# Hongje/OTVM

Hardware: AMD Instinct MI355X
Metric: frames_per_sec (higher is better)
Workload: dtype f16x3 (fp32 operands split into fp16 hi+lo, fp32 accumulate); 1 GPU; synthetic 1920x1080 clip, T=140 frames (untimed lead-in 0 + warmup 5 + timed: the last 135), memory every 5, max 5 slots, trimap propagation + alpha + memorize per frame, one sequence per GPU; weights=synthetic (otvm_amd.synth_weights seed 0), parallelism=sequence-per-gpu x1, batch=1

## Files before the change

include/otvm_hip.h:

```cpp
#ifndef OTVM_HIP_H
#define OTVM_HIP_H

#include <stdint.h>

#ifdef __cplusplus
extern "C" {
#endif

#define OTVM_ACT_NONE 0
#define OTVM_ACT_RELU 1
#define OTVM_ACT_LEAKY 2

#define OTVM_PREC_F32 0
#define OTVM_PREC_F16X3 1
#define OTVM_PREC_F16 2

const char* otvm_last_error(void);
#define OTVM_ABI_VERSION 21
int otvm_abi_version(void);

int otvm_pack_conv_weight(const float* w_oihw, int O, int I, int kh, int kw, int ws, const float* scale,
                          float* w_packed, int O_pad, int I_pad, int K_pad, void* stream);

int64_t otvm_patch_weight_bytes_f16x3(int O, int I_pad);
int otvm_pack_patch_weight_f16x3(const float* w_packed, int O, int K_pad, int I_pad, void* w_frag, float* w_scale,
                                 void* stream);

int64_t otvm_stem_weight_bytes_f16x3(int I_pad);
int otvm_pack_stem_weight_f16x3(const float* w_packed, int O, int K_pad, int I_pad, void* w_frag, float* w_scale,
                                void* stream);

int otvm_fold_bn(const float* gamma, const float* beta, const float* mean, const float* var, float eps, int n,
                 float* scale, float* bias, void* stream);

typedef struct {
    const float* in;  int H, W, Cin, in_ld;
    const float* w;   int K_pad;
    const float* bias;
    const float* residual; int res_ld;
    float* out;       int Ho, Wo, Cout, out_ld;
    int kh, kw, stride, pad, dil;
    int in_relu, act;
    int precision;
    const void* w_hi; const void* w_lo;
    const float* w_scale;
    const void* w_frag;
    double* gn_stats;
    const float* in_scale; const float* in_shift;
    int in_act;
    int tune;
    void* splitk_ws; int64_t splitk_ws_bytes;
    int batch;
    int64_t in_bs, out_bs, res_bs;
    int gn_bs;
    int norm_bs;
    const void* w_wfrag;
    const float* gn_gamma; const float* gn_beta;
    float* gn_scale_out; float* gn_shift_out;
    unsigned* gn_counter;
    int gn_tab_bs;
    int ws_bs;
    const float* res_scale;
    int res_scale_bs;
    const float* in_res; int in_res_ld; int64_t in_res_bs;
} otvm_conv_params;
int otvm_conv2d_accepts_input_residual(const otvm_conv_params* p);

typedef struct otvm_head_params {
    const float* w; const float* b; int n_out;
    const float* img; int img_ld;
    int64_t P;
    float* alpha_out; int alpha_stride;
    float* tri_out;
    float* sm; int sm_ld;
    int64_t img_bs, alpha_bs, tri_bs, sm_bs;
    const void* w16;
} otvm_head_params;
int otvm_conv2d_head(const otvm_conv_params* p, const otvm_head_params* h, void* stream);
int otvm_conv2d_head_fgr(const otvm_conv_params* p, const otvm_head_params* h, float* fgr, int64_t fgr_bs, void* stream);
int64_t otvm_head16_weight_bytes_f16x3(void);
int otvm_pack_head16_weight_f16x3(const float* w_packed, int O, int K_pad, int I_pad, const float* w_scale, void* w16, void* stream);
int otvm_conv2d(const otvm_conv_params* p, void* stream);
int otvm_conv2d_candidates(const otvm_conv_params* p, int* out, int max_n);
int otvm_conv2d_accepts_input_norm(const otvm_conv_params* p);
int otvm_conv2d_input_norm_kind(const otvm_conv_params* p);

int otvm_split_conv_weight_f16x3(const float* w_packed, int O, int O_pad, int K_pad, int taps, int I_pad,
                                 void* w_hi, void* w_lo, float* w_scale, void* stream);

int64_t otvm_wave_weight_bytes_f16x3(int O_pad, int K_pad);
int otvm_pack_wave_weight_f16x3(const void* w_hi, const void* w_lo, int O_pad, int K_pad, void* w_wfrag, void* stream);

typedef struct {
    const float* x; int H, W, Cin, x_ld;
    float* y; int y_ld;
    const void* w1f; const void* w2f; const void* w3f;
    const float* s1; const float* s2; const float* s3;
    const float* b1; const float* b2; const float* b3;
    int batch; int64_t x_bs, y_bs;
    int tile;
} otvm_stm_bottleneck_params;
int otvm_stm_bottleneck_f16x3(const otvm_stm_bottleneck_params* p, void* stream);

int otvm_gn_stats(const float* x, int64_t P, int C, int ld, double* stats, void* stream);
int otvm_gn_table(const double* stats, int64_t P, int C, const float* gamma, const float* beta, float* scale,
                  float* shift, void* stream);
int otvm_gn_apply(const float* x, int64_t P, int C, int ld, const double* stats, const float* gamma,
                  const float* beta, const float* residual, int res_ld, const float* res_scale, const float* res_shift,
                  int res_act, int act, float* out, int out_ld, void* stream);

int otvm_gn_stats_b(const float* x, int64_t P, int C, int ld, double* stats, int batch, int64_t x_bs, int stats_bs, void* stream);
int otvm_gn_table_b(const double* stats, int64_t P, int C, const float* gamma, const float* beta, float* scale, float* shift,
                    int batch, int stats_bs, int norm_bs, void* stream);
typedef struct {
    const float* x; int64_t P; int C, ld; const double* stats; const float* gamma; const float* beta;
    const float* residual; int res_ld; const float* res_scale; const float* res_shift; int res_act, act;
    float* out; int out_ld;
    int batch; int64_t x_bs, res_bs, out_bs; int stats_bs, norm_bs;
} otvm_gn_apply_params;
int otvm_gn_apply_b(const otvm_gn_apply_params* p, void* stream);

typedef struct otvm_gram_params {
    const float* x; int64_t P; int C, ld;
    const float* in_scale; const float* in_shift; int in_act;
    float* gpart; float* spart; int passes;
    int batch; int64_t x_bs; int norm_bs;
    unsigned* diag;
} otvm_gram_params;
int otvm_gram_block(int C);
int64_t otvm_gram_entries(int C);
int otvm_gram_chunks(int64_t P, int C, int* pch_out);
int otvm_gram_f16(const otvm_gram_params* p, void* stream);
typedef struct otvm_gn_predict_params {
    const float* gpart; const float* spart; int64_t P; int C, Cout;
    const float* Mp; const double* v; void* ws; unsigned* counter;
    const float* wscale; const float* gamma; const float* beta; const float* res_shift;
    float* scale_eff; float* bias_eff; float* stat_out;
    int batch, tab_bs, rs_bs;
    unsigned* diag;
} otvm_gn_predict_params;
int64_t otvm_gn_predict_ws_bytes(void);
int otvm_gn_predict(const otvm_gn_predict_params* p, void* stream);

int otvm_maxpool3x3s2(const float* in, int H, int W, int C, int ld, float* out, int out_ld, void* stream);
int otvm_upsample_bilinear(const float* in, int Hi, int Wi, int C, int in_ld, const float* in_scale, const float* in_shift,
                           int in_act, const float* add, int add_ld, float* out, int Ho, int Wo, int out_ld, void* stream);
int otvm_maxpool3x3s2_b(const float* in, int H, int W, int C, int ld, float* out, int out_ld, int batch, int64_t in_bs,
                        int64_t out_bs, void* stream);
int otvm_upsample_bilinear_b(const float* in, int Hi, int Wi, int C, int in_ld, const float* in_scale, const float* in_shift,
                             int in_act, const float* add, int add_ld, float* out, int Ho, int Wo, int out_ld, int batch,
                             int64_t in_bs, int64_t add_bs, int64_t out_bs, int norm_bs, void* stream);
int64_t otvm_ppm_pool_ws_bytes(int H, int C);
int otvm_ppm_pool(const float* in, int H, int W, int C, int ld, float* out, void* ws, void* stream);

typedef struct otvm_ppm_head_params {
    const float* pooled; int C, K_pad, Cout;
    const float* w[4]; const float* bias[4]; const float* gamma[4]; const float* beta[4];
    float* out[4]; int out_ld, act;
} otvm_ppm_head_params;
int otvm_ppm_head(const otvm_ppm_head_params* p, void* stream);

int otvm_ppm_conv_z(const float* const* y, int y_ld, const float* w_ppm, float* Z, void* stream);
int otvm_ppm_conv_add(const float* Z, int H, int W, float* out, int out_ld, double* gn_stats, void* stream);

int64_t otvm_memory_read_ws_bytes(int hw, int T);
int otvm_memory_read(const float* q_key, int q_ld, const float* const* keys, const float* const* vals, int T,
                     int hw, float* out, int out_ld, void* ws, void* stream);

int64_t otvm_bank_slot_bytes_f16x3(int hw);
int otvm_bank_pack_f16x3(const float* key, const float* val, int hw, void* slot, void* stream);
int otvm_memory_read_f16x3(const float* q_key, int q_ld, const void* const* slots, int T, int hw, float* out,
                           int out_ld, void* ws, void* stream);

int otvm_memory_read_f16x3_partial_count(int n_slots, int hw);
int otvm_memory_read_f16x3_partial(const float* q_key, int q_ld, const void* const* slots, int n_slots, int hw, void* ws,
                                   int np_cap, int part0, int* part_end, void* stream);
int otvm_memory_read_f16x3_combine(const void* ws, int np_cap, int n_partials, int hw, float* out, int out_ld, void* stream);

typedef struct {
    const float* fg; const float* bg; const float* a;
    int H, W, Hp, Wp, lh, lw;
    float mean[3], std[3];
    float mean_q[3], std_q[3];
    float mean_m[3], std_m[3];
    float* scaled_imgs;
    float* x11; int x11_ld;
    float* sq;  int sq_ld;
    float* sm;  int sm_ld;
    float* d80; int d80_ld;
    const unsigned char* fg_u8;
    const unsigned char* bg_u8;
    int u8_rgb;
} otvm_preprocess_params;
int otvm_preprocess(const otvm_preprocess_params* p, void* stream);

int otvm_pad_trimap(const float* tri, int H, int W, float* out, int Hp, int Wp, int lh, int lw, void* stream);

int otvm_upsample4_softmax3(const float* logits, int h4, int w4, int ld, float* probs, void* stream);

int otvm_trimap_apply_labels(float* probs, const uint8_t* labels, int H, int W, int Hp, int Wp, int lh, int lw, void* stream);

int64_t otvm_trimap_encode_ws_bytes(int Hp, int Wp);
int otvm_trimap_encode(const float* probs, int Hp, int Wp, const uint8_t* cls_override, uint8_t* cls_out,
                       float* x11, int x11_ld, float* d80, int d80_ld, void* ws, void* stream);

int otvm_fba_head(const float* hid, int hid_ld, const float* w, const float* b, int n_out, const float* img,
                  int img_ld, int64_t P, float* alpha_out, int alpha_stride, float* tri_out, float* sm, int sm_ld,
                  void* stream);
int otvm_fba_head_fgr(const float* hid, int hid_ld, const float* w, const float* b, int n_out, const float* img,
                      int img_ld, int64_t P, float* alpha_out, int alpha_stride, float* tri_out, float* sm, int sm_ld,
                      float* fgr, void* stream);

int otvm_crop_outputs(const float* alpha_p, const float* tri_p, int Hp, int Wp, int H, int W, int lh, int lw,
                      float* alpha, uint8_t* alpha_u8, float* tri, void* stream);

typedef struct otvm_fgr_params {
    const float* alpha_p;
    const float* fgr_p;
    int Hp, Wp, H, W, lh, lw;
    float* fgr;
    unsigned char* rgba_u8;
    unsigned char* comp_u8;
    const unsigned char* bg_u8;
    unsigned char bg_color[3];
    int u8_rgb;
} otvm_fgr_params;
int otvm_fgr_outputs(const otvm_fgr_params* p, void* stream);

int otvm_downsample_u8(const uint8_t* src, int H, int W, int s, uint8_t* dst, void* stream);
int otvm_downsample_trimap(const float* src, int H, int W, int s, float* dst, void* stream);
int otvm_downsample_labels(const uint8_t* src, int H, int W, int s, uint8_t* dst, void* stream);

typedef struct otvm_guided_params {
    int H, W, s, h, w;
    int r, C;
    double eps;
    const uint8_t* guide_full;
    const uint8_t* guide_work;
    const float* target[4];
    float* coef;
    float* alpha;
    uint8_t* alpha_u8;
    float* fgr;
} otvm_guided_params;
int64_t otvm_guided_ws_bytes(int h, int w, int C);
int otvm_guided_coeffs(const otvm_guided_params* p, void* ws, void* stream);
int otvm_guided_apply(const otvm_guided_params* p, void* stream);

int otvm_trimap_from_alpha(const float* a, int H, int W, int r, float* out, void* ws, void* stream);

typedef struct otvm_mask_trimap_params {
    const uint8_t* mask;
    int H, W, lo, hi;
    int t_fg, t_bg;
    float* trimap;
    uint8_t* labels;
    int band_label;
} otvm_mask_trimap_params;
int64_t otvm_trimap_from_mask_ws_bytes(int H, int W);
int otvm_trimap_from_mask(const otvm_mask_trimap_params* p, void* ws, void* stream);

int otvm_onehot_argmax3(const float* tri, int64_t P, float* out, void* stream);

int otvm_matting_metrics(const uint8_t* pred, const uint8_t* target, const uint8_t* mask, const uint8_t* prev_pred,
                         const uint8_t* prev_target, const uint8_t* prev_mask, int64_t n, double* acc, void* stream);
int otvm_matting_grad_conn(const uint8_t* pred, const uint8_t* target, const uint8_t* mask, int H, int W, double* acc,
                           uint8_t* level_map, void* ws, void* stream);
int64_t otvm_matting_grad_conn_ws_bytes(int H, int W);
int otvm_matting_grad_conn_params(int* cutoffs, float* levels, double* taps);
int otvm_optflow_farneback(const uint8_t* prev, const uint8_t* next, int H, int W, float* flow, void* ws, void* stream);
int64_t otvm_optflow_farneback_ws_bytes(int H, int W);
int otvm_optflow_farneback_params(int H, int W, int* levels, float* blur_taps, float* poly_taps, double* poly_inv, float* win_taps);
int otvm_matting_messddt(const uint8_t* p0, const uint8_t* t0, const uint8_t* m0, const uint8_t* p1, const uint8_t* t1,
                         const uint8_t* m1, int H, int W, double* acc, float* flow_out, void* ws, void* stream);

typedef struct otvm_temporal_params {
    int H, W;
    const float* alpha;
    const float* prev;
    const uint8_t* grey;
    const uint8_t* grey_prev;
    const float* flow;
    const float* tri;
    int th, tw, tri_scale;
    float strength;
    float inv_tau_colour, inv_tau_alpha;
    float* out;
    uint8_t* out_u8;
} otvm_temporal_params;
int otvm_luma_u8(const uint8_t* img, int H, int W, int u8_rgb, uint8_t* grey, void* stream);
int otvm_temporal_blend(const otvm_temporal_params* p, void* stream);

int otvm_finite_guard(const float* x, int64_t P, int C, int ld, float limit, int tag, int* flag, void* stream);
int otvm_clear(void* p, int64_t bytes, void* stream);

int otvm_fba_head_train(const float* hid, int hid_ld, const float* w, const float* b, int n_out, const float* img, int img_ld,
                        int64_t P, float* out7, float* logits_out, void* stream);
int otvm_upsample4_logits3(const float* logits, int h4, int w4, int ld, float* logits_out, void* stream);
int otvm_trimap_to_sm(const float* tri, int64_t P, float* sm, int sm_ld, void* stream);
int otvm_scale_flip3(const float* in, int64_t N, int64_t P, float s, float* out, void* stream);
int otvm_trimask(const float* tri, int64_t N, int64_t P, float* mask, unsigned char* cls, const float* gts, float* vis, void* stream);
int otvm_loss_fba_comp(const float* pred7, const float* gt, const float* trimask, const float* fgs, const float* bgs, const float* img,
                       int64_t N, int64_t P, float* cF, float* cB, float* comp, float* alpha_out, double* acc5, void* stream);
int otvm_loss_grad_l1(const float* x, const float* y, int64_t N, int H, int W, float eps, double* acc, void* stream);
int otvm_loss_exclusion_level(const float* img1, const float* img2, int B, int S, int H, int W, float eps, double* acc1, double* acc2,
                              void* stream);
int otvm_avgpool2(const float* x, int64_t N, int H, int W, float* y, void* stream);
int otvm_loss_lap_level(const float* cur_img, const float* cur_tgt, int64_t N, int H, int W, double weight, float* down_img,
                        float* down_tgt, double* acc, void* stream);
int otvm_loss_temporal(const float* x, const float* y, int B, int S, int64_t CP, double* acc, void* stream);
int otvm_loss_ce3(const float* logits, const unsigned char* cls, int64_t N, int64_t P, double* acc, void* stream);

#ifdef __cplusplus
}
#endif
#endif
```

otvm_amd/csrc/conv_patch_f16x3.hip:

```cpp
#pragma clang diagnostic ignored "-Winline-asm"
#include "common.h"
#include "head_math.h"
#include "f16x3_ops.h"
#include <type_traits>
#include <stdlib.h>

#ifndef OTVM_PABL_NOMFMA
#define OTVM_PABL_NOMFMA 0
#endif
#ifndef OTVM_PABL_NOLOAD
#define OTVM_PABL_NOLOAD 0
#endif
#ifndef OTVM_PABL_NOCOMMIT
#define OTVM_PABL_NOCOMMIT 0
#endif
#ifndef OTVM_PABL_NOLDSRD
#define OTVM_PABL_NOLDSRD 0
#endif
#ifndef OTVM_PABL_NOEPI
#define OTVM_PABL_NOEPI 0
#endif
#ifndef OTVM_PABL_MFMA16
#define OTVM_PABL_MFMA16 0
#endif
#ifndef OTVM_PATCH_NO_LEAN
#define OTVM_PATCH_NO_LEAN 0
#endif
#ifndef OTVM_PATCH_SETPRIO
#define OTVM_PATCH_SETPRIO 0
#endif
#ifndef OTVM_PM16_NOKXP
#define OTVM_PM16_NOKXP 0
#endif

namespace {

struct PatchArgs {
    const float* in; const _Float16* wf; const float* wscale; const float* bias; const float* residual; float* out;
    double* gn_stats;
    int H, W, Cin, in_ld, res_ld, Cout, out_ld, n_pad32, in_relu, act;
    int tiles_x, tiles_y, tiles_n;
    OtvmTileWalk walk;
    const float* in_scale; const float* in_shift; int in_act;
    int64_t in_bs, out_bs, res_bs; int gn_bs, norm_bs, batch;
    OtvmGnTail tail;
    const float* in_res; int in_res_ld; int64_t in_res_bs;
    unsigned in_bytes, in_res_bytes;
    OtvmHeadArgs head; int64_t head_img_bs, head_alpha_bs, head_tri_bs, head_sm_bs, head_fgr_bs;
};

constexpr int CB = 16;
constexpr int LDP = 24;

#if OTVM_PABL_MFMA16
__device__ __forceinline__ f32x16 mfma_probe16(const f16x8 a, const f16x8 b, f32x16 c) {
    f32x4 q0 = {c[0], c[1], c[2], c[3]}, q1 = {c[4], c[5], c[6], c[7]};
    q0 = __builtin_amdgcn_mfma_f32_16x16x32_f16(a, b, q0, 0, 0, 0);
    q1 = __builtin_amdgcn_mfma_f32_16x16x32_f16(a, b, q1, 0, 0, 0);
    c[0] = q0.x; c[1] = q0.y; c[2] = q0.z; c[3] = q0.w; c[4] = q1.x; c[5] = q1.y; c[6] = q1.z; c[7] = q1.w;
    return c;
}
#define PATCH_MFMA32(a, b, c) mfma_probe16(a, b, c)
#else
#define PATCH_MFMA32(a, b, c) __builtin_amdgcn_mfma_f32_32x32x16_f16(a, b, c, 0, 0, 0)
#endif

__device__ __forceinline__ int pi16(int r) {
    const int k = (r < 4) ? r : (r < 12 ? r - 4 : r - 8);
    return 4 * (k >> 1) + (k & 1) + ((r >= 4 && r < 12) ? 2 : 0);
}

template <int TH, int BN, int NW, int DIL, int TAPG, bool INRES = false, bool HEAD = false, int NWN = 1, bool GLDS = false, int NPASS = 3,
          bool M16 = false, bool FGR = false>
__global__ __launch_bounds__(NW * 64)
__attribute__((amdgpu_waves_per_eu((TAPG == 3 && BN <= 32 && !INRES) ? 3 : (M16 ? 2 : 1), (TAPG == 3 && BN <= 32 && !INRES) ? 3 : 10)))
void conv_patch_f16x3_kernel(const PatchArgs pa) {
    PatchArgs p = pa;
    {
        const int zb = blockIdx.y;
        p.in += zb * p.in_bs;
        if (INRES) p.in_res += zb * p.in_res_bs;
        if (HEAD) {
            p.head.img += zb * p.head_img_bs;
            if (p.head.alpha_out) p.head.alpha_out += zb * p.head_alpha_bs;
            if (p.head.tri_out) p.head.tri_out += zb * p.head_tri_bs;
            if (p.head.sm) p.head.sm += zb * p.head_sm_bs;
            if constexpr (FGR) { if (p.head.fgr) p.head.fgr += zb * p.head_fgr_bs; }
        }
        p.out += zb * p.out_bs;
        if (p.residual) p.residual += zb * p.res_bs;
        if (p.gn_stats) p.gn_stats += zb * p.gn_bs;
        if (p.in_scale) { p.in_scale += zb * p.norm_bs; p.in_shift += zb * p.norm_bs; }
    }
    constexpr int NT = NW * 64;
    constexpr int NWM = NW / NWN, TNW = BN / 32;
    constexpr int TM = TH / NWM, TN = TNW / NWN;
    static_assert(NW % NWN == 0 && TH % NWM == 0 && TNW % NWN == 0, "bad wave grid");
    constexpr int PW = 32 + 2 * DIL, PH = TH + 2 * DIL, NPIX = PH * PW;
    constexpr int NG = 9 / TAPG;
    static_assert(BN % 32 == 0 && 9 % TAPG == 0, "bad tile");
    static_assert(!FGR || HEAD, "FGR: the HEAD variant that also keeps the head's foreground estimate (head.fgr)");
    static_assert(!M16 || (TAPG == 9 && NPASS == 3 && !HEAD && NWN == 1 && !GLDS), "the 16x16x32 form: nine-tap f16x3 tiles");
    constexpr int PLANE = ((NPIX + 11) / 16) * 16 + 4;
    constexpr int PATCH_HALFS = M16 ? 2 * 2 * PLANE * 8 : 2 * NPIX * LDP;
    constexpr int B_PIECES = TAPG * TNW * 2 * 64;
    constexpr int B_HALFS = B_PIECES * 8;
    constexpr int EPI_HALFS = NW * 32 * 36 * 2 * (HEAD ? 2 : 1);
    static_assert(!GLDS || TAPG == 3, "LDS-DMA weight stages: the 3-tap stages (two buffers fit beside the patch)");
    constexpr int NBUF = GLDS ? 2 : 1;
    constexpr int SM_HALFS = PATCH_HALFS + NBUF * B_HALFS > EPI_HALFS ? PATCH_HALFS + NBUF * B_HALFS : EPI_HALFS;
    __shared__ __attribute__((aligned(16))) _Float16 smem[SM_HALFS];
    _Float16* Ph = smem;
    _Float16* Pl = smem + (M16 ? 2 * PLANE * 8 : NPIX * LDP);
    _Float16* Bs = smem + PATCH_HALFS;

    const int tid = threadIdx.x, lane = tid & 63, wave = tid >> 6;
    const int wave_m = NWN == 1 ? wave : wave % NWM, nt0 = NWN == 1 ? 0 : (wave / NWM) * TN;
#ifdef OTVM_PATCH_STAGGER
    if (blockIdx.x >= 256 && blockIdx.x < 512)
        for (int i = 0; i < OTVM_PATCH_STAGGER; ++i) __builtin_amdgcn_s_sleep(127);
#endif
    int tile_n, tile_x, tile_y;
    otvm_tile_decode(p.walk, blockIdx.x, gridDim.x, p.tiles_n, p.tiles_x, p.tiles_y, tile_n, tile_x, tile_y);
    const int ty0 = tile_y * TH, tx0 = tile_x * 32, n0 = tile_n * BN;

    f32x16 acc[TM][TN];
#pragma unroll
    for (int a = 0; a < TM; ++a)
#pragma unroll
        for (int b = 0; b < TN; ++b)
#pragma unroll
            for (int e = 0; e < 16; ++e) acc[a][b][e] = 0.f;

    const int frow = lane & 31, fh = lane >> 5;
    const int ncb = p.Cin / CB;
    const int nbs = p.n_pad32 >> 5;
    const int nb0 = n0 >> 5;
    constexpr int NP = (NPIX * 4 + NT - 1) / NT;
    constexpr int NB = (B_PIECES + NT - 1) / NT;
    f32x4 rp[NP];
    f32x4 rr[INRES ? NP : 1];
    f16x8 rb[NB];
    f32x4 rsc = {1.f, 1.f, 1.f, 1.f}, rsh = {0.f, 0.f, 0.f, 0.f};
    __amdgpu_buffer_rsrc_t in_rsrc = otvm_buffer_rsrc(p.in, p.in_bytes);
    __amdgpu_buffer_rsrc_t res_rsrc = otvm_buffer_rsrc(INRES ? p.in_res : p.in, INRES ? p.in_res_bytes : 0);
    constexpr bool LEAN = M16 && !INRES && !OTVM_PATCH_NO_LEAN;
    unsigned l_voff[LEAN ? NP : 1];
    unsigned l_woff[LEAN ? NB : 1];
    unsigned l_wok = 0;
    int l_o0 = 0;
    float l_slope = 1.f;
    if constexpr (LEAN) {
        static_assert(NT % 4 == 0 && B_PIECES == NB * NT && TAPG == 9, "lean staging: whole weight pieces per thread, one stage per channel block");
#pragma unroll
        for (int k = 0; k < NP; ++k) {
            const int idx = tid + k * NT;
            const int pix = idx >> 2, c4 = (idx & 3) * 4;
            const int py = pix / PW, px = pix - py * PW;
            const int iy = ty0 - DIL + py, ix = tx0 - DIL + px;
            const bool ok = ((unsigned)iy < (unsigned)p.H) & ((unsigned)ix < (unsigned)p.W) & (idx < NPIX * 4);
            l_voff[k] = ok ? ((unsigned)(iy * p.W + ix) * (unsigned)p.in_ld + (unsigned)c4) << 2 : 0xFFFFFFFFu;
        }
#pragma unroll
        for (int k = 0; k < NB; ++k) {
            const int i = tid + k * NT;
            const int l = i & 63, blk = i >> 6, hl = blk & 1, tb = blk >> 1, b = tb % TNW, tap = tb / TNW;
            const bool ok = nb0 + b < nbs;
            l_woff[k] = (unsigned)((((tap * nbs + nb0 + (ok ? b : 0)) * 2) * 2 + hl) * 512 + l * 8) * 2u;
            l_wok |= ok ? (1u << k) : 0u;
        }
        l_o0 = (((tid >> 1) & 1) * PLANE + (tid >> 2)) * 8 + (tid & 1) * 4;
        l_slope = p.in_relu ? 0.f : (p.in_scale ? (p.in_act == OTVM_ACT_RELU ? 0.f : (p.in_act == OTVM_ACT_LEAKY ? 0.01f : 1.f)) : 1.f);
    }
    auto prefetch = [&](int cb, int g) __attribute__((always_inline)) {
        if constexpr (LEAN) {
            const unsigned soff = (unsigned)(cb * CB * 4);
#pragma unroll
            for (int k = 0; k < NP; ++k)
                rp[k] = __builtin_bit_cast(f32x4, (u32x4)__builtin_amdgcn_raw_buffer_load_b128(in_rsrc, __builtin_elementwise_add_sat(l_voff[k], soff), 0, 0));
            const char* wbase = reinterpret_cast<const char*>(p.wf) + (size_t)(((cb >> 1) * 9 * nbs * 2 + (cb & 1)) * 2) * 1024;
#pragma unroll
            for (int k = 0; k < NB; ++k) rb[k] = *reinterpret_cast<const f16x8*>(wbase + l_woff[k]);
            if (p.in_scale) {
                rsc = *reinterpret_cast<const f32x4*>(p.in_scale + cb * CB + (tid & 3) * 4);
                rsh = *reinterpret_cast<const f32x4*>(p.in_shift + cb * CB + (tid & 3) * 4);
            }
            return;
        }
        const int cb32 = cb >> 1, ks = cb & 1;
        _Float16* bdst = Bs + (GLDS ? ((cb * NG + g) & 1) * B_HALFS : 0);
#pragma unroll
        for (int k = 0; k < NB; ++k) {
            const int i = tid + k * NT;
            if (i < B_PIECES) {
                const int l = i & 63, blk = i >> 6;
                const int hl = blk & 1, tb = blk >> 1, b = tb % TNW, tap = g * TAPG + tb / TNW;
                if (NPASS == 1 && hl) continue;
                const int64_t src = (((((int64_t)cb32 * 9 + tap) * nbs + nb0 + b) * 2 + ks) * 2 + hl) * 512 + l * 8;
                if constexpr (GLDS) {
                    const unsigned m0v = __builtin_amdgcn_readfirstlane((unsigned)(uintptr_t)(__attribute__((address_space(3))) void*)(bdst + (i - l) * 8));
                    asm volatile("s_mov_b32 m0, %0\n\ts_nop 0\n\tglobal_load_lds_dwordx4 %1, off" :: "s"(m0v), "v"(p.wf + src) : "m0", "memory");
                } else {
                    f16x8 wv = {(_Float16)0.f, (_Float16)0.f, (_Float16)0.f, (_Float16)0.f, (_Float16)0.f, (_Float16)0.f, (_Float16)0.f, (_Float16)0.f};
                    if (nb0 + b < nbs) wv = *reinterpret_cast<const f16x8*>(p.wf + src);
                    rb[k] = wv;
                }
            }
        }
        if (g == 0) {
            if (p.in_scale) {
                rsc = *reinterpret_cast<const f32x4*>(p.in_scale + cb * CB + (tid & 3) * 4);
                rsh = *reinterpret_cast<const f32x4*>(p.in_shift + cb * CB + (tid & 3) * 4);
            }
#pragma unroll
            for (int k = 0; k < NP; ++k) {
                const int idx = tid + k * NT;
                const int pix = idx >> 2, c4 = (idx & 3) * 4;
                const int py = pix / PW, px = pix - py * PW;
                const int iy = ty0 - DIL + py, ix = tx0 - DIL + px;
                const unsigned oob = (unsigned)((int)((unsigned)iy < (unsigned)p.H) & (int)((unsigned)ix < (unsigned)p.W) &
                                                (int)(idx < NPIX * 4)) - 1u;
                const unsigned e = (unsigned)(iy * p.W + ix);
                rp[k] = __builtin_bit_cast(f32x4, (u32x4)__builtin_amdgcn_raw_buffer_load_b128(in_rsrc, ((e * (unsigned)p.in_ld + cb * CB + c4) << 2) | oob, 0, 0));
                if (INRES)
                    rr[k] = __builtin_bit_cast(f32x4, (u32x4)__builtin_amdgcn_raw_buffer_load_b128(res_rsrc, ((e * (unsigned)p.in_res_ld + cb * CB + c4) << 2) | oob, 0, 0));
            }
        }
    };
    auto commit = [&](int g) __attribute__((always_inline)) {
        if constexpr (LEAN) {
            const f16x8 zero8 = {(_Float16)0.f, (_Float16)0.f, (_Float16)0.f, (_Float16)0.f, (_Float16)0.f, (_Float16)0.f, (_Float16)0.f, (_Float16)0.f};
#pragma unroll
            for (int k = 0; k < NB; ++k) *reinterpret_cast<f16x8*>(&Bs[(tid + k * NT) * 8]) = ((l_wok >> k) & 1u) ? rb[k] : zero8;
            if (p.in_scale != nullptr || p.in_relu) {
#pragma unroll
                for (int k = 0; k < NP; ++k) {
                    f32x4 v = rp[k] * rsc + rsh;
                    v.x = fmaxf(v.x, 0.f) + l_slope * fminf(v.x, 0.f); v.y = fmaxf(v.y, 0.f) + l_slope * fminf(v.y, 0.f);
                    v.z = fmaxf(v.z, 0.f) + l_slope * fminf(v.z, 0.f); v.w = fmaxf(v.w, 0.f) + l_slope * fminf(v.w, 0.f);
                    const f32x4 z = {0.f, 0.f, 0.f, 0.f};
                    rp[k] = (l_voff[k] == 0xFFFFFFFFu) ? z : v;
                }
            }
#pragma unroll
            for (int k = 0; k < NP; ++k) {
                if (k + 1 < NP || tid + k * NT < NPIX * 4) {
                    f16x4 hi, lo;
                    otvm_split4(rp[k], hi, lo);
                    *reinterpret_cast<f16x4*>(&Ph[l_o0 + 512 * k]) = hi;
                    *reinterpret_cast<f16x4*>(&Pl[l_o0 + 512 * k]) = lo;
                }
            }
            return;
        }
        if constexpr (!GLDS) {
#pragma unroll
            for (int k = 0; k < NB; ++k) {
                const int i = tid + k * NT;
                if (NPASS == 1 && ((i >> 6) & 1)) continue;
                if (i < B_PIECES) *reinterpret_cast<f16x8*>(&Bs[i * 8]) = rb[k];
            }
        }
        if (g == 0) {
#pragma unroll
            for (int k = 0; k < NP; ++k) {
                const int idx = tid + k * NT;
                if (idx < NPIX * 4) {
                    f32x4 v = rp[k];
                    if (p.in_scale) {
                        const int pix = idx >> 2;
                        const int py = pix / PW, px = pix - py * PW;
                        const int iy = ty0 - DIL + py, ix = tx0 - DIL + px;
                        const bool inb = (unsigned)iy < (unsigned)p.H && (unsigned)ix < (unsigned)p.W;
                        v = v * rsc + rsh;
                        if (INRES && inb) v += rr[INRES ? k : 0];
                        v.x = otvm_act(v.x, p.in_act); v.y = otvm_act(v.y, p.in_act);
                        v.z = otvm_act(v.z, p.in_act); v.w = otvm_act(v.w, p.in_act);
                        const f32x4 z = {0.f, 0.f, 0.f, 0.f};
                        v = inb ? v : z;
                    }
                    if (p.in_relu) {
                        v.x = fmaxf(v.x, 0.f); v.y = fmaxf(v.y, 0.f); v.z = fmaxf(v.z, 0.f); v.w = fmaxf(v.w, 0.f);
                    }
                    f16x4 hi, lo;
                    const int pix = idx >> 2, c4 = (idx & 3) * 4;
                    if constexpr (M16) {
                        otvm_split4(v, hi, lo);
                        const int o = (((idx >> 1) & 1) * PLANE + pix) * 8 + (idx & 1) * 4;
                        *reinterpret_cast<f16x4*>(&Ph[o]) = hi;
                        *reinterpret_cast<f16x4*>(&Pl[o]) = lo;
                    } else if constexpr (NPASS == 3) {
                        otvm_split4(v, hi, lo);
                        *reinterpret_cast<f16x4*>(&Ph[pix * LDP + c4]) = hi;
                        *reinterpret_cast<f16x4*>(&Pl[pix * LDP + c4]) = lo;
                    } else {
                        hi = f16x4{(_Float16)v.x, (_Float16)v.y, (_Float16)v.z, (_Float16)v.w};
                        *reinterpret_cast<f16x4*>(&Ph[pix * LDP + c4]) = hi;
                    }
                }
            }
        }
    };
    prefetch(0, 0);
    for (int cb = 0; cb < ncb; ++cb) {
#pragma unroll
        for (int g = 0; g < NG; ++g) {
            const _Float16* Bcur = Bs + (GLDS ? ((cb * NG + g) & 1) * B_HALFS : 0);
            if constexpr (GLDS) {
                asm volatile("s_waitcnt vmcnt(0)" ::: "memory");
                __syncthreads();
                if (g == 0) {
                    commit(0);
                    __syncthreads();
                }
            } else {
                __syncthreads();
                if (!OTVM_PABL_NOCOMMIT || (cb == 0 && g == 0)) commit(g);
                __syncthreads();
            }
            if (!OTVM_PABL_NOLOAD) {
                if (g + 1 < NG) prefetch(cb, g + 1);
                else if (cb + 1 < ncb) prefetch(cb + 1, 0);
            }
            if constexpr (M16) {
                if (OTVM_PATCH_SETPRIO) __builtin_amdgcn_s_setprio(OTVM_PATCH_SETPRIO);
                const int l15 = lane & 15, oct = (lane >> 4) & 1, hs = lane >> 5;
                const int abase = (oct * PLANE + wave_m * TM * PW + pi16(l15)) * 8;
                const int bbase = (l15 + 32 * oct) * 8;
                auto quad = [](const f32x16& c, int q) __attribute__((always_inline)) { return f32x4{c[4 * q], c[4 * q + 1], c[4 * q + 2], c[4 * q + 3]}; };
                auto put = [](f32x16& c, int q, const f32x4 v) __attribute__((always_inline)) { c[4 * q] = v.x; c[4 * q + 1] = v.y; c[4 * q + 2] = v.z; c[4 * q + 3] = v.w; };
                auto pass = [&](const f16x8 (&A)[TM][2], const f16x8 (&B)[TN][2]) __attribute__((always_inline)) {
#pragma unroll
                    for (int a = 0; a < TM; ++a)
#pragma unroll
                        for (int b = 0; b < TN; ++b)
#pragma unroll
                            for (int si = 0; si < 2; ++si)
#pragma unroll
                                for (int sj = 0; sj < 2; ++sj)
                                    put(acc[a][b], 2 * si + sj, __builtin_amdgcn_mfma_f32_16x16x32_f16(A[a][si], B[b][sj], quad(acc[a][b], 2 * si + sj), 0, 0, 0));
                };
                constexpr int TAPB = TNW * 2 * 512;
#pragma unroll
                for (int pr = 0; pr < 4; ++pr) {
                    constexpr bool KXP = DIL == 1 && !OTVM_PM16_NOKXP;
                    const int t1 = !KXP ? 2 * pr : (pr < 3 ? pr : 6), t2 = !KXP ? 2 * pr + 1 : (pr < 3 ? 3 + pr : 7);
                    const int o1 = ((t1 % 3) * DIL * PW + (t1 / 3) * DIL) * 8, o2 = ((t2 % 3) * DIL * PW + (t2 / 3) * DIL) * 8;
                    const int ao = !KXP ? abase + (hs ? o2 : o1)
                                        : (pr < 3 ? abase + hs * (DIL * 8) + pr * DIL * PW * 8 : abase + 2 * DIL * 8 + hs * (DIL * PW * 8));
                    const int bo = bbase + (hs ? t2 : t1) * TAPB;
                    f16x8 ah[TM][2], al[TM][2], bh[TN][2], bl[TN][2];
#pragma unroll
                    for (int a = 0; a < TM; ++a)
#pragma unroll
                        for (int si = 0; si < 2; ++si) {
                            ah[a][si] = *reinterpret_cast<const f16x8*>(&Ph[ao + (a * PW + 16 * si) * 8]);
                            al[a][si] = *reinterpret_cast<const f16x8*>(&Pl[ao + (a * PW + 16 * si) * 8]);
                        }
#pragma unroll
                    for (int b = 0; b < TN; ++b)
#pragma unroll
                        for (int sj = 0; sj < 2; ++sj) {
                            bh[b][sj] = *reinterpret_cast<const f16x8*>(&Bcur[bo + ((nt0 + b) * 2) * 512 + 16 * sj * 8]);
                            bl[b][sj] = *reinterpret_cast<const f16x8*>(&Bcur[bo + ((nt0 + b) * 2 + 1) * 512 + 16 * sj * 8]);
                        }
                    pass(al, bh);
                    pass(ah, bl);
                    pass(ah, bh);
                }
                {
                    constexpr int o8 = (2 * DIL * PW + 2 * DIL) * 8;
                    const _Float16* Ahl = hs ? Pl : Ph;
                    f16x8 ax[TM][2], bhh[TN][2], bl0[TN][2];
#pragma unroll
                    for (int a = 0; a < TM; ++a)
#pragma unroll
                        for (int si = 0; si < 2; ++si) ax[a][si] = *reinterpret_cast<const f16x8*>(&Ahl[abase + o8 + (a * PW + 16 * si) * 8]);
                    const f16x8 zero8 = {(_Float16)0.f, (_Float16)0.f, (_Float16)0.f, (_Float16)0.f, (_Float16)0.f, (_Float16)0.f, (_Float16)0.f, (_Float16)0.f};
#pragma unroll
                    for (int b = 0; b < TN; ++b)
#pragma unroll
                        for (int sj = 0; sj < 2; ++sj) {
                            bhh[b][sj] = *reinterpret_cast<const f16x8*>(&Bcur[bbase + 8 * TAPB + ((nt0 + b) * 2) * 512 + 16 * sj * 8]);
                            const f16x8 l = *reinterpret_cast<const f16x8*>(&Bcur[bbase + 8 * TAPB + ((nt0 + b) * 2 + 1) * 512 + 16 * sj * 8]);
                            bl0[b][sj] = hs ? zero8 : l;
                        }
                    pass(ax, bl0);
                    pass(ax, bhh);
                }
                if (OTVM_PATCH_SETPRIO) __builtin_amdgcn_s_setprio(0);
            } else
#pragma unroll
            for (int tl = 0; tl < TAPG; ++tl) {
                const int tap = g * TAPG + tl;
                const int kx = tap / 3, ky = tap - kx * 3;
                f16x8 ah[TM], al[TM];
#pragma unroll
                for (int a = 0; a < TM; ++a) {
#if OTVM_PABL_NOLDSRD
                    const f16x8 one = {(_Float16)1.f, (_Float16)1.f, (_Float16)1.f, (_Float16)1.f, (_Float16)1.f, (_Float16)1.f, (_Float16)1.f, (_Float16)1.f};
                    ah[a] = one * (_Float16)(float)(lane + tap); al[a] = one;
#else
                    const int o = ((wave_m * TM + a + ky * DIL) * PW + kx * DIL + frow) * LDP + 8 * fh;
                    ah[a] = *reinterpret_cast<const f16x8*>(&Ph[o]);
                    if (NPASS == 3) al[a] = *reinterpret_cast<const f16x8*>(&Pl[o]);
#endif
                }
                constexpr int GB = TN < 4 ? TN : 4;
#pragma unroll
                for (int b0 = 0; b0 < TN; b0 += GB) {
                    f16x8 bh[GB], bl[GB];
#pragma unroll
                    for (int j = 0; j < GB; ++j) {
#if OTVM_PABL_NOLDSRD
                        const f16x8 one = {(_Float16)1.f, (_Float16)1.f, (_Float16)1.f, (_Float16)1.f, (_Float16)1.f, (_Float16)1.f, (_Float16)1.f, (_Float16)1.f};
                        bh[j] = one; bl[j] = one * (_Float16)(float)lane;
#else
                        bh[j] = *reinterpret_cast<const f16x8*>(&Bcur[((tl * TNW + nt0 + b0 + j) * 2) * 512 + lane * 8]);
                        if (NPASS == 3) bl[j] = *reinterpret_cast<const f16x8*>(&Bcur[((tl * TNW + nt0 + b0 + j) * 2 + 1) * 512 + lane * 8]);
#endif
                    }
#if OTVM_PABL_NOMFMA
                    if (ah[0][0] == (_Float16)12345.f) acc[0][0][0] += (float)bh[0][0] + (float)bl[0][0] + (float)al[0][0];
                    continue;
#endif
                    if constexpr (NPASS == 3) {
#pragma unroll
                        for (int j = 0; j < GB; ++j)
#pragma unroll
                            for (int a = 0; a < TM; ++a)
                                acc[a][b0 + j] = PATCH_MFMA32(al[a], bh[j], acc[a][b0 + j]);
#pragma unroll
                        for (int j = 0; j < GB; ++j)
#pragma unroll
                            for (int a = 0; a < TM; ++a)
                                acc[a][b0 + j] = PATCH_MFMA32(ah[a], bl[j], acc[a][b0 + j]);
                    }
#pragma unroll
                    for (int j = 0; j < GB; ++j)
#pragma unroll
                        for (int a = 0; a < TM; ++a)
                            acc[a][b0 + j] = PATCH_MFMA32(ah[a], bh[j], acc[a][b0 + j]);
                }
            }
        }
    }

    const int col = lane & 31, rbase = (lane >> 5) * 4;
    const int pbase16 = pi16(4 * (lane >> 4));
    auto acc_row = [&](int e) __attribute__((always_inline)) -> int {
        return M16 ? 16 * (e >> 3) + pbase16 + (e & 1) + 4 * ((e >> 1) & 1) : (e & 3) + 8 * (e >> 2) + rbase;
    };
    auto acc_col = [&](int e) __attribute__((always_inline)) -> int { return M16 ? 16 * ((e >> 2) & 1) + (lane & 15) : col; };
    __syncthreads();
#if OTVM_PABL_NOEPI
    if (acc[0][0][0] == 12345.678f) p.out[0] = acc[0][0][1];
    if (acc[0][0][0] != 12345.678f) return;
#endif
    if constexpr (HEAD) {
        static_assert(TM == 2 && TN == 1 && NWN == 1, "the head epilogue is written for two pixel rows and one channel tile per wave");
        float* patch = reinterpret_cast<float*>(smem) + wave * (2 * 32 * 36);
#pragma unroll
        for (int a = 0; a < TM; ++a)
#pragma unroll
            for (int e = 0; e < 16; ++e) patch[a * (32 * 36) + ((e & 3) + 8 * (e >> 2) + rbase) * 36 + col] = acc[a][0][e];
        const int a = lane >> 5, px = lane & 31;
        const int y = ty0 + wave_m * TM + a, x = tx0 + px;
        float h[16];
#pragma unroll
        for (int k = 0; k < 4; ++k) {
            f32x4 v = *reinterpret_cast<const f32x4*>(&patch[a * (32 * 36) + px * 36 + 4 * k]);
            f32x4 sc4, bi4 = {0.f, 0.f, 0.f, 0.f};
#pragma unroll
            for (int j = 0; j < 4; ++j) {
                sc4[j] = p.wscale[4 * k + j];
                if (p.bias) bi4[j] = p.bias[4 * k + j];
            }
            v = v * sc4 + bi4;
            h[4 * k] = otvm_act(v.x, p.act); h[4 * k + 1] = otvm_act(v.y, p.act);
            h[4 * k + 2] = otvm_act(v.z, p.act); h[4 * k + 3] = otvm_act(v.w, p.act);
        }
        if (y < p.H && x < p.W) {
            const int64_t m = (int64_t)y * p.W + x;
            if (p.out) {
#pragma unroll
                for (int k = 0; k < 4; ++k)
                    *reinterpret_cast<f32x4*>(p.out + m * p.out_ld + 4 * k) = f32x4{h[4 * k], h[4 * k + 1], h[4 * k + 2], h[4 * k + 3]};
            }
            otvm_head_pixel<FGR>(h, p.head, m);
        }
        return;
    }
    const bool vec_ok = ((p.out_ld & 3) == 0) && ((reinterpret_cast<uintptr_t>(p.out) & 15) == 0) &&
                        (!p.residual || (((p.res_ld & 3) == 0) && ((reinterpret_cast<uintptr_t>(p.residual) & 15) == 0)));
    const bool interior = vec_ok && ty0 + TH <= p.H && tx0 + 32 <= p.W && n0 + BN <= p.Cout;
    auto epilogue_full = [&](auto act_c, auto res_c) __attribute__((always_inline)) {
        constexpr int ACT = decltype(act_c)::value;
        constexpr bool RES = decltype(res_c)::value;
        float* patch = reinterpret_cast<float*>(smem) + wave * (32 * 36);
        const int prow = lane >> 3, pc = (lane & 7) * 4;
        f32x4 sc4[TN], bi4[TN];
#pragma unroll
        for (int b = 0; b < TN; ++b) {
#pragma unroll
            for (int j = 0; j < 4; ++j) sc4[b][j] = p.wscale[n0 + (nt0 + b) * 32 + pc + j];
            bi4[b] = f32x4{0.f, 0.f, 0.f, 0.f};
        }
        if (p.bias) {
#pragma unroll
            for (int b = 0; b < TN; ++b)
#pragma unroll
                for (int j = 0; j < 4; ++j) bi4[b][j] = p.bias[n0 + (nt0 + b) * 32 + pc + j];
        }
        auto load_res = [&](int t, f32x4 (&r)[4]) __attribute__((always_inline)) {
            const int b = t / TM, a = t - b * TM;
            const int64_t m0r = (int64_t)(ty0 + wave_m * TM + a) * p.W + tx0 + prow;
#pragma unroll
            for (int r4 = 0; r4 < 4; ++r4)
                r[r4] = *reinterpret_cast<const f32x4*>(p.residual + (m0r + r4 * 8) * p.res_ld + n0 + (nt0 + b) * 32 + pc);
        };
        f32x4 rnext[4] = {{0.f, 0.f, 0.f, 0.f}, {0.f, 0.f, 0.f, 0.f}, {0.f, 0.f, 0.f, 0.f}, {0.f, 0.f, 0.f, 0.f}};
        if (RES) load_res(0, rnext);
#pragma unroll
        for (int t = 0; t < TM * TN; ++t) {
            const int b = t / TM, a = t - b * TM;
            const int64_t m0r = (int64_t)(ty0 + wave_m * TM + a) * p.W + tx0 + prow;
            f32x4 rres[4];
#pragma unroll
            for (int r4 = 0; r4 < 4; ++r4) rres[r4] = rnext[r4];
#pragma unroll
            for (int e = 0; e < 16; ++e) patch[acc_row(e) * 36 + acc_col(e)] = acc[a][b][e];
            if (RES && t + 1 < TM * TN) load_res(t + 1, rnext);
#pragma unroll
            for (int r4 = 0; r4 < 4; ++r4) {
                f32x4 v = *reinterpret_cast<const f32x4*>(&patch[(r4 * 8 + prow) * 36 + pc]);
                v = v * sc4[b] + bi4[b];
                if (RES) v += rres[r4];
                v.x = otvm_act(v.x, ACT); v.y = otvm_act(v.y, ACT); v.z = otvm_act(v.z, ACT); v.w = otvm_act(v.w, ACT);
                *reinterpret_cast<f32x4*>(p.out + (m0r + r4 * 8) * p.out_ld + n0 + (nt0 + b) * 32 + pc) = v;
            }
        }
    };
    auto epilogue = [&](auto full_c) __attribute__((always_inline)) {
        constexpr bool FULL = decltype(full_c)::value;
        float* patch = reinterpret_cast<float*>(smem) + wave * (32 * 36);
        const int prow = lane >> 3, pc = (lane & 7) * 4;
#pragma unroll
        for (int b = 0; b < TN; ++b) {
            const int n4 = n0 + (nt0 + b) * 32 + pc;
            f32x4 sc4 = {0.f, 0.f, 0.f, 0.f}, bi4 = {0.f, 0.f, 0.f, 0.f};
#pragma unroll
            for (int j = 0; j < 4; ++j) {
                if (FULL || n4 + j < p.Cout) {
                    sc4[j] = p.wscale[n4 + j];
                    bi4[j] = p.bias ? p.bias[n4 + j] : 0.f;
                }
            }
#pragma unroll
            for (int a = 0; a < TM; ++a) {
                const int y = ty0 + wave_m * TM + a;
                f32x4 rres[4];
                const bool res_vec = p.residual && vec_ok && (FULL || n4 + 3 < p.Cout);
#pragma unroll
                for (int r4 = 0; r4 < 4; ++r4) {
                    const int x = tx0 + r4 * 8 + prow;
                    rres[r4] = f32x4{0.f, 0.f, 0.f, 0.f};
                    if (FULL ? (p.residual != nullptr) : (res_vec && y < p.H && x < p.W))
                        rres[r4] = *reinterpret_cast<const f32x4*>(p.residual + ((int64_t)y * p.W + x) * p.res_ld + n4);
                }
#pragma unroll
                for (int e = 0; e < 16; ++e) patch[acc_row(e) * 36 + acc_col(e)] = acc[a][b][e];
#pragma unroll
                for (int r4 = 0; r4 < 4; ++r4) {
                    const int xi = r4 * 8 + prow;
                    const int x = tx0 + xi;
                    f32x4 v = *reinterpret_cast<const f32x4*>(&patch[xi * 36 + pc]);
                    v = v * sc4 + bi4;
                    if (FULL || (y < p.H && x < p.W)) {
                        const int64_t m = (int64_t)y * p.W + x;
                        if (FULL || (vec_ok && n4 + 3 < p.Cout)) {
                            v += rres[r4];
                            v.x = otvm_act(v.x, p.act); v.y = otvm_act(v.y, p.act);
                            v.z = otvm_act(v.z, p.act); v.w = otvm_act(v.w, p.act);
                            *reinterpret_cast<f32x4*>(p.out + m * p.out_ld + n4) = v;
                        } else {
#pragma unroll
                            for (int j = 0; j < 4; ++j) {
                                if (n4 + j < p.Cout) {
                                    float xv = v[j];
                                    if (p.residual) xv += p.residual[m * p.res_ld + n4 + j];
                                    p.out[m * p.out_ld + n4 + j] = otvm_act(xv, p.act);
                                }
                            }
                        }
                    }
                }
            }
        }
    };
    if (interior) {
        using std::integral_constant;
        const bool r = p.residual != nullptr;
        if (p.act == OTVM_ACT_RELU) { if (r) epilogue_full(integral_constant<int, OTVM_ACT_RELU>{}, std::true_type{}); else epilogue_full(integral_constant<int, OTVM_ACT_RELU>{}, std::false_type{}); }
        else if (p.act == OTVM_ACT_LEAKY) { if (r) epilogue_full(integral_constant<int, OTVM_ACT_LEAKY>{}, std::true_type{}); else epilogue_full(integral_constant<int, OTVM_ACT_LEAKY>{}, std::false_type{}); }
        else { if (r) epilogue_full(integral_constant<int, OTVM_ACT_NONE>{}, std::true_type{}); else epilogue_full(integral_constant<int, OTVM_ACT_NONE>{}, std::false_type{}); }
    } else {
        epilogue(std::false_type{});
    }

    if (p.gn_stats) {
        __shared__ double gred[2 * BN];
        const int cg = p.Cout >> 5;
        const int seg = cg < 32 ? cg : 32;
        for (int i = tid; i < 2 * BN; i += NT) gred[i] = 0.0;
        __syncthreads();
        if constexpr (M16) {
#pragma unroll
            for (int b = 0; b < TN; ++b)
#pragma unroll
                for (int sj = 0; sj < 2; ++sj) {
                    const int nl = (nt0 + b) * 32 + 16 * sj + (lane & 15);
                    const int n = n0 + nl;
                    float s = 0.f, ss = 0.f, cnt = 0.f;
                    const float pil = n < p.Cout && p.bias ? p.bias[n / cg * cg] : 0.f;
                    if (n < p.Cout) {
                        const float sc_ = p.wscale[n];
                        const float bias = p.bias ? p.bias[n] : 0.f, bd = bias - pil;
#pragma unroll
                        for (int a = 0; a < TM; ++a) {
                            const int y = ty0 + wave_m * TM + a;
#pragma unroll
                            for (int si = 0; si < 2; ++si)
#pragma unroll
                                for (int j = 0; j < 4; ++j) {
                                    const int e = 4 * (2 * si + sj) + j;
                                    const int x = tx0 + acc_row(e);
                                    if (y < p.H && x < p.W) {
                                        const float d = acc[a][b][e] * sc_ + bd;
                                        s += d;
                                        ss += d * d;
                                        cnt += 1.f;
                                    }
                                }
                        }
                    }
                    s += __shfl_xor(s, 16); ss += __shfl_xor(ss, 16); cnt += __shfl_xor(cnt, 16);
                    s += __shfl_xor(s, 32); ss += __shfl_xor(ss, 32); cnt += __shfl_xor(cnt, 32);
                    const int seg16 = seg < 16 ? seg : 16;
                    for (int off = 1; off < seg16; off <<= 1) {
                        s += __shfl_xor(s, off);
                        ss += __shfl_xor(ss, off);
                        cnt += __shfl_xor(cnt, off);
                    }
                    if (lane < 16 && (lane & (seg16 - 1)) == 0 && n < p.Cout) {
                        const int gl = nl / cg;
                        double S, SS;
                        otvm_gn_unshift(s, ss, (int)cnt, pil, S, SS);
                        atomicAdd(&gred[2 * gl], S);
                        atomicAdd(&gred[2 * gl + 1], SS);
                    }
                }
        } else
#pragma unroll
        for (int b = 0; b < TN; ++b) {
            const int nl = (nt0 + b) * 32 + col;
            const int n = n0 + nl;
            float s = 0.f, ss = 0.f, cnt = 0.f;
            const float pil = n < p.Cout && p.bias ? p.bias[n / cg * cg] : 0.f;
            if (n < p.Cout) {
                const float sc_ = p.wscale[n];
                const float bias = p.bias ? p.bias[n] : 0.f, bd = bias - pil;
#pragma unroll
                for (int a = 0; a < TM; ++a) {
                    const int y = ty0 + wave_m * TM + a;
#pragma unroll
                    for (int e = 0; e < 16; ++e) {
                        const int x = tx0 + (e & 3) + 8 * (e >> 2) + rbase;
                        if (y < p.H && x < p.W) {
                            const float d = acc[a][b][e] * sc_ + bd;
                            s += d;
                            ss += d * d;
                            cnt += 1.f;
                        }
                    }
                }
            }
            s += __shfl_xor(s, 32);
            ss += __shfl_xor(ss, 32);
            cnt += __shfl_xor(cnt, 32);
            for (int off = 1; off < seg; off <<= 1) {
                s += __shfl_xor(s, off);
                ss += __shfl_xor(ss, off);
                cnt += __shfl_xor(cnt, off);
            }
            if (lane < 32 && (lane & (seg - 1)) == 0 && n < p.Cout) {
                const int gl = nl / cg;
                double S, SS;
                otvm_gn_unshift(s, ss, (int)cnt, pil, S, SS);
                atomicAdd(&gred[2 * gl], S);
                atomicAdd(&gred[2 * gl + 1], SS);
            }
        }
        __syncthreads();
        const int ng = (BN + cg - 1) / cg;
        for (int i = tid; i < 2 * ng; i += NT) {
            const int g = n0 / cg + (i >> 1);
            if (g < 32 && gred[i] != 0.0) atomicAdd(&p.gn_stats[2 * g + (i & 1)], gred[i]);
        }
        __syncthreads();
        otvm_gn_table_tail(p.gn_stats, (int64_t)p.H * p.W, p.Cout, p.tail, blockIdx.y, gridDim.x, reinterpret_cast<float*>(gred));
    }
}

__global__ __launch_bounds__(256) void pack_patch_weight_kernel(const float* __restrict__ w, int O, int K_pad, int I_pad, int n_pad32,
                                                                _Float16* __restrict__ wf, float* __restrict__ wscale) {
    const int n = blockIdx.x;
    __shared__ float red[256];
    float mx = 0.f;
    const float* row = w + (int64_t)n * K_pad;
    const bool real = n < O;
    if (real)
        for (int k = threadIdx.x; k < 9 * I_pad; k += 256) mx = fmaxf(mx, fabsf(row[k]));
    red[threadIdx.x] = mx;
    __syncthreads();
    for (int s = 128; s > 0; s >>= 1) {
        if (threadIdx.x < s) red[threadIdx.x] = fmaxf(red[threadIdx.x], red[threadIdx.x + s]);
        __syncthreads();
    }
    int e = 0;
    if (red[0] > 0.f) frexpf(red[0], &e);
    const float inv = ldexpf(1.f, -e);
    if (threadIdx.x == 0 && real) wscale[n] = ldexpf(1.f, e);
    const int nb = n >> 5, nl = n & 31, nbs = n_pad32 >> 5;
    for (int k = threadIdx.x; k < 9 * I_pad; k += 256) {
        const int tap0 = k / I_pad, c = k - tap0 * I_pad;
        const int tap = (tap0 % 3) * 3 + tap0 / 3;
        const float v = real ? row[k] * inv : 0.f;
        const _Float16 hi = (_Float16)v;
        const _Float16 lo = (_Float16)(v - (float)hi);
        const int cb = c >> 5, ks = (c >> 4) & 1, h = (c >> 3) & 1, j = c & 7;
        const int l = nl + 32 * h;
        const int64_t blk = ((((int64_t)cb * 9 + tap) * nbs + nb) * 2 + ks) * 2;
        wf[(blk + 0) * 512 + l * 8 + j] = hi;
        wf[(blk + 1) * 512 + l * 8 + j] = lo;
    }
}

template <int NPASS, int TH, int BN, int NW, int DIL, int TAPG = 9, bool INRES = false, bool HEAD = false, int NWN = 1, bool GLDS = false,
          bool M16 = false, bool FGR = false>
int launch_patch(PatchArgs& a, hipStream_t s) {
    a.tiles_x = otvm_ceil_div(a.W, 32);
    a.tiles_y = otvm_ceil_div(a.H, TH);
    a.tiles_n = otvm_ceil_div(a.Cout, BN);
    a.walk = otvm_tile_walk_of(1);
    hipLaunchKernelGGL((conv_patch_f16x3_kernel<TH, BN, NW, DIL, TAPG, INRES, HEAD, NWN, GLDS, NPASS, M16, FGR>), dim3(a.tiles_x * a.tiles_y * a.tiles_n, a.batch), dim3(NW * 64), 0, s, a);
    OTVM_CHECK_LAUNCH("otvm_conv2d(patch f16x3)");
    return 0;
}

}

extern "C" int64_t otvm_patch_weight_bytes_f16x3(int O, int I_pad) {
    const int64_t n_pad32 = (O + 31) / 32 * 32;
    return (int64_t)((I_pad + 31) / 32) * 9 * n_pad32 * 32 * 2 * sizeof(_Float16);
}

extern "C" int otvm_pack_patch_weight_f16x3(const float* w_packed, int O, int K_pad, int I_pad, void* w_frag, float* w_scale,
                                            void* stream) {
    OTVM_REQUIRE(w_packed && w_frag && w_scale && I_pad % 16 == 0, "otvm_pack_patch_weight_f16x3: needs I_pad %% 16 == 0");
    const int n_pad32 = (O + 31) / 32 * 32;
    hipLaunchKernelGGL(pack_patch_weight_kernel, dim3(n_pad32), dim3(256), 0, (hipStream_t)stream, w_packed, O, K_pad, I_pad, n_pad32,
                       (_Float16*)w_frag, w_scale);
    OTVM_CHECK_LAUNCH("otvm_pack_patch_weight_f16x3");
    return 0;
}

static int patch_choice(const otvm_conv_params* p, bool forced = false) {
    if (!p->w_frag || p->kh != 3 || p->kw != 3 || p->stride != 1 || p->pad != p->dil || p->Cin % 16 != 0) return 0;
    if (p->dil != 1 && p->dil != 2 && p->dil != 4) return 0;
    static const int wide = otvm_probe_int("OTVM_PATCH_WIDE", 1);
    if (p->Cout <= 64) return 1;
    if (!wide || p->Cout % 256 != 0) return 0;
    if (forced) return 2;
    static const int t_patch = otvm_probe_int("OTVM_T_PATCH", 400);
    const int64_t t8 = (int64_t)otvm_ceil_div(p->H, 8) * otvm_ceil_div(p->W, 32) * (p->Cout / 256);
    return t8 >= t_patch ? 2 : 0;
}

int otvm_conv2d_igemm_accepts_input_norm(const otvm_conv_params* p);
extern "C" int otvm_conv2d_accepts_input_norm(const otvm_conv_params* p) {
    return p && otvm_prec_is_split(p->precision) && (patch_choice(p) != 0 || otvm_conv2d_igemm_accepts_input_norm(p)) ? 1 : 0;
}
extern "C" int otvm_conv2d_input_norm_kind(const otvm_conv_params* p) {
    if (!p || !otvm_prec_is_split(p->precision)) return 0;
    if (patch_choice(p) != 0) return 1;
    return otvm_conv2d_igemm_accepts_input_norm(p) ? 2 : 0;
}

extern "C" int otvm_conv2d_accepts_input_residual(const otvm_conv_params* p) {
    return p && otvm_prec_is_split(p->precision) && patch_choice(p) == 1 && p->dil == 1 && p->in_scale && !p->in_relu ? 1 : 0;
}

int otvm_conv2d_patch_eligible(const otvm_conv_params* p) {
    if (p->in_res && !otvm_conv2d_accepts_input_residual(p)) return 0;
    return patch_choice(p, true) != 0 ? 1 : 0;
}

static int patch_run(const otvm_conv_params* p, void* stream, int choice, const otvm_head_params* hd = nullptr, float* fgr = nullptr,
                     int64_t fgr_bs = 0);
int otvm_conv2d_head16_impl(const otvm_conv_params* p, const otvm_head_params* hd, float* fgr, int64_t fgr_bs, void* stream);

static int conv2d_head_any(const otvm_conv_params* p, const otvm_head_params* hd, float* fgr, int64_t fgr_bs, void* stream) {
    OTVM_REQUIRE(p && hd && p->in && hd->w && hd->b && hd->img, "otvm_conv2d_head: null pointer");
    OTVM_REQUIRE(otvm_prec_is_split(p->precision) && p->Cout == 16 && patch_choice(p) == 1 && p->dil == 1 && !p->residual &&
                     !p->gn_stats && !p->in_res && p->w_scale,
                 "otvm_conv2d_head: a 3x3 stride-1 f16x3 layer with 16 output channels, no residual / statistics");
    OTVM_REQUIRE(hd->n_out == 7 || (hd->n_out == 10 && hd->tri_out), "otvm_conv2d_head: n_out must be 7, or 10 with tri_out");
    OTVM_REQUIRE(!p->out || ((p->out_ld & 3) == 0 && ((uintptr_t)p->out & 15) == 0), "otvm_conv2d_head: out must be 16-byte aligned");
    if (hd->w16) return otvm_conv2d_head16_impl(p, hd, fgr, fgr_bs, stream);
    return patch_run(p, stream, 1, hd, fgr, fgr_bs);
}

extern "C" int otvm_conv2d_head(const otvm_conv_params* p, const otvm_head_params* hd, void* stream) {
    return conv2d_head_any(p, hd, nullptr, 0, stream);
}

extern "C" int otvm_conv2d_head_fgr(const otvm_conv_params* p, const otvm_head_params* hd, float* fgr, int64_t fgr_bs, void* stream) {
    OTVM_REQUIRE(fgr && hd && hd->P > 0 && ((p && p->batch > 1) ? fgr_bs >= 3 * hd->P : true),
                 "otvm_conv2d_head_fgr: fgr must be given, [3][P] per image (fgr_bs >= 3 P for a batch)");
    return conv2d_head_any(p, hd, fgr, fgr_bs, stream);
}

int otvm_conv2d_patch_f16x3_forced(const otvm_conv_params* p, void* stream) { return patch_run(p, stream, patch_choice(p, true)); }

int otvm_conv2d_patch_f16x3_impl(const otvm_conv_params* p, void* stream) { return patch_run(p, stream, patch_choice(p)); }

static int patch_m16() {
    static const int m = otvm_probe_int("OTVM_PATCH_M16", 1);
    return m;
}

template <int NPASS>
static int patch_run_t(const otvm_conv_params* p, void* stream, int choice, const otvm_head_params* hd, float* fgr, int64_t fgr_bs) {
    if (choice == 0) return -1;
    const bool is_wide = choice == 2;
    PatchArgs a;
    a.in = p->in; a.wf = (const _Float16*)p->w_frag; a.wscale = p->w_scale; a.bias = p->bias; a.residual = p->residual;
    a.out = p->out; a.gn_stats = p->gn_stats;
    a.H = p->H; a.W = p->W; a.Cin = p->Cin; a.in_ld = p->in_ld; a.res_ld = p->res_ld; a.Cout = p->Cout; a.out_ld = p->out_ld;
    a.n_pad32 = (p->Cout + 31) / 32 * 32; a.in_relu = p->in_relu; a.act = p->act;
    hipStream_t s = (hipStream_t)stream;
    a.in_scale = p->in_scale; a.in_shift = p->in_shift; a.in_act = p->in_act;
    a.tail = otvm_gn_tail_of(p);
    a.batch = p->batch > 1 ? p->batch : 1;
    a.in_bs = a.batch > 1 ? p->in_bs : 0; a.out_bs = a.batch > 1 ? p->out_bs : 0; a.res_bs = a.batch > 1 ? p->res_bs : 0;
    a.gn_bs = a.batch > 1 ? p->gn_bs : 0; a.norm_bs = a.batch > 1 ? p->norm_bs : 0;
    a.in_res = p->in_res; a.in_res_ld = p->in_res_ld; a.in_res_bs = a.batch > 1 ? p->in_res_bs : 0;
    {
        const int64_t ib = (int64_t)p->H * p->W * p->in_ld * 4, rb = p->in_res ? (int64_t)p->H * p->W * p->in_res_ld * 4 : 0;
        OTVM_REQUIRE(ib < 0xFFFFFFF0ll && rb < 0xFFFFFFF0ll, "otvm_conv2d(patch f16x3): input view of %lld bytes is beyond 32-bit offsets", (long long)ib);
        a.in_bytes = (unsigned)ib; a.in_res_bytes = (unsigned)rb;
    }
    if (hd) {
        a.head.w = hd->w; a.head.b = hd->b; a.head.n_out = hd->n_out; a.head.img = hd->img; a.head.img_ld = hd->img_ld;
        a.head.P = hd->P; a.head.alpha_out = hd->alpha_out; a.head.alpha_stride = hd->alpha_stride; a.head.tri_out = hd->tri_out;
        a.head.sm = hd->sm; a.head.sm_ld = hd->sm_ld; a.head.out7 = nullptr; a.head.logits_out = nullptr;
        a.head_img_bs = a.batch > 1 ? hd->img_bs : 0; a.head_alpha_bs = a.batch > 1 ? hd->alpha_bs : 0;
        a.head_tri_bs = a.batch > 1 ? hd->tri_bs : 0; a.head_sm_bs = a.batch > 1 ? hd->sm_bs : 0;
        a.head.fgr = fgr; a.head_fgr_bs = a.batch > 1 ? fgr_bs : 0;
        if (fgr) return launch_patch<3, 8, 32, 4, 1, 3, false, true, 1, false, false, true>(a, s);
        return launch_patch<3, 8, 32, 4, 1, 3, false, true>(a, s);
    }
    if (p->in_res) {
        OTVM_REQUIRE(otvm_conv2d_accepts_input_residual(p) && !is_wide && (p->in_res_ld & 3) == 0 && ((uintptr_t)p->in_res & 15) == 0,
                     "otvm_conv2d: in_res needs in_scale on a 3x3 stride-1 dilation-1 layer with <= 64 output channels");
        if (p->Cout <= 32) return launch_patch<3, 8, 32, 4, 1, 3, true>(a, s);
        return patch_m16() ? launch_patch<3, 8, 64, 4, 1, 9, true, false, 1, false, true>(a, s) : launch_patch<3, 8, 64, 4, 1, 9, true>(a, s);
    }
    if (is_wide) {
        static const int nwn = otvm_probe_int("OTVM_PATCH_WIDE_NWN", 2);
        static const int glds = otvm_probe_int("OTVM_PATCH_WIDE_GLDS", 1);
        if (nwn == 2 && p->dil == 1 && glds) return launch_patch<NPASS, 8, 256, 8, 1, 3, false, false, 2, true>(a, s);
        if (nwn == 2 && p->dil == 1) return launch_patch<NPASS, 8, 256, 8, 1, 3, false, false, 2>(a, s);
        if (p->dil == 1) return launch_patch<NPASS, 8, 256, 8, 1, 3>(a, s);
        if (p->dil == 2) return launch_patch<NPASS, 8, 256, 8, 2, 3>(a, s);
        return launch_patch<NPASS, 8, 256, 8, 4, 3>(a, s);
    }
    static const int th16 = otvm_probe_int("OTVM_PATCH_TH16", 0);
    if (p->dil == 1 && th16 && (int64_t)p->H * p->W >= (1 << 18))
        return p->Cout <= 32 ? launch_patch<NPASS, 16, 32, 8, 1>(a, s) : launch_patch<NPASS, 16, 64, 8, 1>(a, s);
    static const int rows4 = otvm_probe_int("OTVM_PATCH32_ROWS4", 1);
    static const int glds32 = otvm_probe_int("OTVM_PATCH32_GLDS", 0);
    if (p->dil == 1 && p->Cout <= 32 && rows4 && (int64_t)p->H * p->W >= (1 << 20))
        return glds32 ? launch_patch<NPASS, 16, 32, 4, 1, 3, false, false, 1, true>(a, s) : launch_patch<NPASS, 16, 32, 4, 1, 3>(a, s);
    static const int glds64 = otvm_probe_int("OTVM_PATCH64_GLDS", 0);
    if (p->dil == 1 && p->Cout > 32 && glds64) return launch_patch<NPASS, 8, 64, 4, 1, 3, false, false, 1, true>(a, s);
    if (p->dil == 1 && p->Cout <= 32 && glds32) return launch_patch<NPASS, 8, 32, 4, 1, 3, false, false, 1, true>(a, s);
    if constexpr (NPASS == 3) {
        if (patch_m16() && p->Cout > 32) {
            if (p->dil == 1) return launch_patch<3, 8, 64, 4, 1, 9, false, false, 1, false, true>(a, s);
            if (p->dil == 2) return launch_patch<3, 8, 64, 4, 2, 9, false, false, 1, false, true>(a, s);
            return launch_patch<3, 8, 64, 4, 4, 9, false, false, 1, false, true>(a, s);
        }
    }
    if (p->dil == 1) return p->Cout <= 32 ? launch_patch<NPASS, 8, 32, 4, 1, 3>(a, s) : launch_patch<NPASS, 8, 64, 4, 1>(a, s);
    if (p->dil == 2) return launch_patch<NPASS, 8, 64, 4, 2>(a, s);
    return launch_patch<NPASS, 8, 64, 4, 4>(a, s);
}

static int patch_run(const otvm_conv_params* p, void* stream, int choice, const otvm_head_params* hd, float* fgr, int64_t fgr_bs) {
    return p->precision == OTVM_PREC_F16 ? patch_run_t<1>(p, stream, choice, hd, fgr, fgr_bs) : patch_run_t<3>(p, stream, choice, hd, fgr, fgr_bs);
}
```

otvm_amd/engine.py:

```python
import ctypes as C
import os

import torch

from . import lib as L

NONE, RELU, LEAKY = 0, 1, 2
GUARD_CLEAR = 2 ** 31 - 1
F16_LIMIT = 65504.0
FUSE_GN_STATS = True
FUSE_GN_APPLY = os.environ.get("OTVM_FUSE_GN_APPLY", "1") != "0"
_GRAPHS_ENV = os.environ.get("OTVM_GRAPHS")
USE_GRAPHS = None if _GRAPHS_ENV in (None, "", "auto") else (_GRAPHS_ENV != "0")
GRAPH_AUTO_PIXELS = 1 << 22


def graphs_wanted(setting, padded_pixels):
    if setting is not None:
        return bool(setting)
    if int(os.environ.get("WORLD_SIZE", "1")) > 1:
        return True
    return padded_pixels < GRAPH_AUTO_PIXELS
PRE_ON_S2 = os.environ.get("OTVM_PRE_ON_S2", "1") != "0"
EVDEC_LATE = os.environ.get("OTVM_EVDEC_LATE", "1") != "0"
WAVE_TILE = os.environ.get("OTVM_WAVE_TILE", "0") != "0"
FUSE_GN_APPLY_IGEMM = os.environ.get("OTVM_FUSE_GN_APPLY_IGEMM", "1") != "0"
FUSE_GN_APPLY_IGEMM_KXK = os.environ.get("OTVM_FUSE_GN_APPLY_IGEMM_KXK", "0") != "0"
FUSE_GN_TABLE = os.environ.get("OTVM_FUSE_GN_TABLE", "1") != "0"
FUSE_STM_BLOCK = os.environ.get("OTVM_FUSE_STM_BLOCK", "1") != "0"
FUSE_STM_BLOCK128 = int(os.environ.get("OTVM_FUSE_STM_BLOCK128", "1"))
STM128_TILE = int(os.environ.get("OTVM_STM128_TILE", "0"))
FUSE_PPM_HEAD = os.environ.get("OTVM_PPM_HEAD", "1") != "0"
FUSE_GN_PREDICT = os.environ.get("OTVM_GN_PREDICT", "1") != "0"
GN_PREDICT_MIN_PIXELS = int(os.environ.get("OTVM_GN_PREDICT_MIN_PIXELS", "16384"))
GN_PREDICT_PASSES = int(os.environ.get("OTVM_GN_PREDICT_PASSES", "1"))
GN_PREDICT_PLANES = tuple(int(v) for v in os.environ.get("OTVM_GN_PREDICT_PLANES", "64,128,256,512").split(",") if v)
GN_PREDICT_DS = os.environ.get("OTVM_GN_PREDICT_DS", "1") != "0"
GN_PREDICT_KAPPA_P3 = float(os.environ.get("OTVM_GN_PREDICT_KAPPA_P3", "4"))
GN_PREDICT_KAPPA_OFF = float(os.environ.get("OTVM_GN_PREDICT_KAPPA_OFF", "256"))
FUSE_REFINE_TAIL = os.environ.get("OTVM_FUSE_REFINE_TAIL", "0") != "0"
FUSE_HEAD = os.environ.get("OTVM_FUSE_HEAD", "1") != "0"
HEAD16 = os.environ.get("OTVM_HEAD16", "1") != "0"
PPM_ALGEBRA = os.environ.get("OTVM_PPM_ALGEBRA", "1") != "0"


AUTOTUNE = os.environ.get("OTVM_AUTOTUNE", "1") != "0"
_TUNE_CACHE = {}
TUNE_LOG = []
TUNE_FILE = os.environ.get("OTVM_TUNE_FILE")
_TUNE_FILE_LOADED = False


_NON_VARIANT_ENV = ("OTVM_TUNE_FILE", "OTVM_DIST_BACKEND", "OTVM_TEST_FULL_F64", "OTVM_TEST_4K_ORACLE", "OTVM_BENCH_LIVE_PMC",
                    "OTVM_BENCH_FORCE_DIAG", "OTVM_CHECK_FINITE", "OTVM_GRAPHS")


def variant_env():
    return sorted((k, v) for k, v in os.environ.items() if k.startswith("OTVM_") and k not in _NON_VARIANT_ENV)


def kernel_config_digest():
    import hashlib
    return hashlib.sha256(repr((sorted(_TUNE_CACHE.items()), variant_env())).encode()).hexdigest()[:16]


def _tune_file_tag():
    name = "none"
    if torch.cuda.is_available():
        pr = torch.cuda.get_device_properties(torch.cuda.current_device())
        name = "%s/%dcu" % (getattr(pr, "gcnArchName", "?").split(":")[0], pr.multi_processor_count)
    return {"device": name, "abi": L.ABI_VERSION, "variant_env": [list(kv) for kv in variant_env()]}


def _load_tune_file():
    if not (TUNE_FILE and os.path.exists(TUNE_FILE)):
        return
    import json
    import warnings
    try:
        with open(TUNE_FILE) as f:
            doc = json.load(f)
        if not isinstance(doc, dict) or "choices" not in doc:
            raise ValueError("no 'choices' table (file written by an older build)")
        tag = _tune_file_tag()
        if doc.get("abi") != tag["abi"] or (tag["device"] != "none" and doc.get("device") != tag["device"]):
            raise ValueError("tuned for %r / ABI %r, this process runs %r / ABI %r"
                             % (doc.get("device"), doc.get("abi"), tag["device"], tag["abi"]))
        if doc.get("variant_env", []) != tag["variant_env"]:
            raise ValueError("tuned under the switches %r, this process runs under %r" % (doc.get("variant_env", []), tag["variant_env"]))
        for k, v in doc["choices"].items():
            _TUNE_CACHE[tuple(json.loads(k))] = int(v)
    except Exception as e:
        warnings.warn("otvm_amd: ignoring OTVM_TUNE_FILE=%s (%s)" % (TUNE_FILE, e))


def _save_tune_file():
    if not TUNE_FILE:
        return
    import json
    doc = dict(_tune_file_tag())
    doc["choices"] = {json.dumps([int(x) for x in k]): v for k, v in _TUNE_CACHE.items()}
    tmp = "%s.%d.tmp" % (TUNE_FILE, os.getpid())
    with open(tmp, "w") as f:
        json.dump(doc, f, indent=0)
    os.replace(tmp, TUNE_FILE)


def share_tune_cache(src=0):
    import torch.distributed as dist
    if not (dist.is_available() and dist.is_initialized()):
        return
    obj = [dict(_TUNE_CACHE) if dist.get_rank() == src else None]
    dist.broadcast_object_list(obj, src=src)
    if dist.get_rank() != src:
        _TUNE_CACHE.update(obj[0])


def _rup(x, m):
    return (x + m - 1) // m * m


class Act:
    __slots__ = ("t", "H", "W", "C", "ld", "off", "B", "bs")

    def __init__(self, t, H, W, C, ld=None, off=0, B=1, bs=0):
        self.t, self.H, self.W, self.C = t, H, W, C
        self.ld = C if ld is None else ld
        self.off = off
        self.B, self.bs = B, (bs if B > 1 else 0)

    @property
    def ptr(self):
        return self.t.data_ptr() + 4 * self.off

    @property
    def P(self):
        return self.H * self.W

    def ch(self, c0, c):
        return Act(self.t, self.H, self.W, c, self.ld, self.off + c0, self.B, self.bs)

    def img(self, b):
        return Act(self.t, self.H, self.W, self.C, self.ld, self.off + b * self.bs)

    def torch(self, b=0):
        return torch.as_strided(self.t, (self.H, self.W, self.C), (self.W * self.ld, self.ld, 1), self.off + b * self.bs)


class ConvW:
    __slots__ = ("w", "K_pad", "O", "I", "I_pad", "kh", "kw", "bias", "w_hi", "w_lo", "w_scale", "w_frag", "w_wfrag", "w16")


def pad_amounts(h, w, d):
    nh = h + (d - h % d) % d
    nw = w + (d - w % d) % d
    lh, lw = int((nh - h) / 2), int((nw - w) / 2)
    return lw, nw - w - lw, lh, nh - h - lh


def _is_anchor(slot):
    return isinstance(slot, dict) and bool(slot.get("anchor", False))


def bank_update(bank, new, first_frame, memorize, max_memory_num, anchor=False):
    old = list(bank)
    new_anchor = bool(anchor or first_frame)
    if isinstance(new, dict):
        new["anchor"] = new_anchor
    if max_memory_num == 0:
        nb = [new] if first_frame else bank
    elif max_memory_num == 1:
        nb = [new]
    else:
        if first_frame:
            nb = [new]
        elif new_anchor or memorize or len(bank) == 1 or (bank and _is_anchor(bank[-1])):
            nb = bank + [new]
        else:
            nb = bank[:-1] + [new]
        cap = max_memory_num + max(0, sum(1 for s in nb if _is_anchor(s)) - 1)
        while len(nb) > cap:
            i = next(j for j in range(1, len(nb)) if not _is_anchor(nb[j]))
            nb = nb[:i] + nb[i + 1:]
    released = [s for s in old + [new] if not any(s is k for k in nb)]
    return nb, released


PRECISIONS = {"f32": L.PREC_F32, "f16x3": L.PREC_F16X3, "f16": L.PREC_F16X3}
CONV_PRECISIONS = {"f32": L.PREC_F32, "f16x3": L.PREC_F16X3, "f16": L.PREC_F16}


def default_precision():
    import os
    return os.environ.get("OTVM_PRECISION", "f16x3")


def pack_conv_weight(lib, dev, w, ws=False, scale=None, i_pad=None, split=True, stream=0):
    O, I, kh, kw = w.shape
    cw = ConvW()
    cw.O, cw.I, cw.kh, cw.kw = O, I, kh, kw
    cw.I_pad = _rup(I, 4) if i_pad is None else i_pad
    cw.K_pad = _rup(kh * kw * cw.I_pad, 32)
    O_pad = _rup(O, 128)
    cw.w = torch.empty(O_pad * cw.K_pad, dtype=torch.float32, device=dev)
    cw.bias = None
    w = w.contiguous()
    L.check(lib.otvm_pack_conv_weight(w.data_ptr(), O, I, kh, kw, 1 if ws else 0,
                                      0 if scale is None else scale.data_ptr(), cw.w.data_ptr(), O_pad,
                                      cw.I_pad, cw.K_pad, stream), "pack_conv_weight")
    cw.w_hi = cw.w_lo = cw.w_scale = cw.w_frag = cw.w_wfrag = cw.w16 = None
    if split:
        cw.w_hi = torch.empty(O_pad * cw.K_pad, dtype=torch.float16, device=dev)
        cw.w_lo = torch.empty(O_pad * cw.K_pad, dtype=torch.float16, device=dev)
        cw.w_scale = torch.empty(O, dtype=torch.float32, device=dev)
        L.check(lib.otvm_split_conv_weight_f16x3(cw.w.data_ptr(), O, O_pad, cw.K_pad, kh * kw, cw.I_pad, cw.w_hi.data_ptr(),
                                                 cw.w_lo.data_ptr(), cw.w_scale.data_ptr(), stream), "split_conv_weight")
        if cw.I_pad % 32 == 0 and kh * kw <= 32 and (WAVE_TILE or O >= 128):
            cw.w_wfrag = torch.zeros(int(lib.otvm_wave_weight_bytes_f16x3(O_pad, cw.K_pad)), dtype=torch.uint8, device=dev)
            L.check(lib.otvm_pack_wave_weight_f16x3(cw.w_hi.data_ptr(), cw.w_lo.data_ptr(), O_pad, cw.K_pad, cw.w_wfrag.data_ptr(),
                                                    stream), "pack_wave_weight")
        if kh == 7 and kw == 7 and O <= 64 and cw.I_pad <= 64:
            cw.w_frag = torch.zeros(int(lib.otvm_stem_weight_bytes_f16x3(cw.I_pad)), dtype=torch.uint8, device=dev)
            L.check(lib.otvm_pack_stem_weight_f16x3(cw.w.data_ptr(), O, cw.K_pad, cw.I_pad, cw.w_frag.data_ptr(),
                                                    cw.w_scale.data_ptr(), stream), "pack_stem_weight")
        if kh == 3 and kw == 3 and cw.I_pad % 16 == 0:
            cw.w_frag = torch.zeros(int(lib.otvm_patch_weight_bytes_f16x3(O, cw.I_pad)), dtype=torch.uint8, device=dev)
            L.check(lib.otvm_pack_patch_weight_f16x3(cw.w.data_ptr(), O, cw.K_pad, cw.I_pad, cw.w_frag.data_ptr(),
                                                     cw.w_scale.data_ptr(), stream), "pack_patch_weight")
            if O == 16 and cw.I_pad == 32:
                cw.w16 = torch.zeros(int(lib.otvm_head16_weight_bytes_f16x3()), dtype=torch.uint8, device=dev)
                L.check(lib.otvm_pack_head16_weight_f16x3(cw.w.data_ptr(), O, cw.K_pad, cw.I_pad, cw.w_scale.data_ptr(),
                                                          cw.w16.data_ptr(), stream), "pack_head16_weight")
    return cw


def gram_tables(lib, cw):
    O_pad = cw.w.numel() // cw.K_pad
    w = cw.w.view(O_pad, cw.K_pad)[:cw.O, :cw.I].double()
    cg, Cin = cw.O // 32, cw.I
    wg = w.view(32, cg, Cin)
    v = wg.sum(1).contiguous()
    bs = int(lib.otvm_gram_block(Cin))
    nb = Cin // bs
    blocks = []
    for bi in range(nb):
        rows = wg[:, :, bi * bs:(bi + 1) * bs]
        for bj in range(bi, nb):
            m = torch.einsum("gci,gcj->gij", rows, wg[:, :, bj * bs:(bj + 1) * bs])
            blocks.append((m if bi == bj else 2.0 * m).reshape(32, bs * bs))
    mp = torch.cat(blocks, 1).float().contiguous()
    assert mp.shape[1] == int(lib.otvm_gram_entries(Cin))
    return mp, v


def conv_params(x, cw, out, bias=None, stride=1, pad=0, dil=1, act=NONE, in_relu=0, residual=None, precision=L.PREC_F32,
                in_norm=None, splitk_ws=None):
    Ho = (x.H + 2 * pad - dil * (cw.kh - 1) - 1) // stride + 1
    Wo = (x.W + 2 * pad - dil * (cw.kw - 1) - 1) // stride + 1
    if precision in (L.PREC_F16X3, L.PREC_F16) and cw.w_hi is None:
        raise RuntimeError("otvm_amd: f16x3 convolution requested but the weight was packed without a split")
    return L.ConvParams(x.ptr, x.H, x.W, x.C, x.ld, cw.w.data_ptr(), cw.K_pad,
                        0 if bias is None else bias.data_ptr(),
                        0 if residual is None else residual.ptr, 0 if residual is None else residual.ld,
                        out.ptr, Ho, Wo, cw.O, out.ld, cw.kh, cw.kw, stride, pad, dil, in_relu, act, precision,
                        0 if cw.w_hi is None else cw.w_hi.data_ptr(), 0 if cw.w_lo is None else cw.w_lo.data_ptr(),
                        0 if cw.w_scale is None else cw.w_scale.data_ptr(),
                        0 if cw.w_frag is None else cw.w_frag.data_ptr(), 0,
                        0 if in_norm is None else in_norm[0], 0 if in_norm is None else in_norm[1],
                        0 if in_norm is None else in_norm[2], 0,
                        0 if splitk_ws is None else splitk_ws.data_ptr(),
                        0 if splitk_ws is None else splitk_ws.numel() * splitk_ws.element_size(),
                        x.B, x.bs, out.bs, 0 if residual is None else residual.bs, 0,
                        0 if in_norm is None or len(in_norm) < 4 else in_norm[3],
                        0 if cw.w_wfrag is None else cw.w_wfrag.data_ptr())


class HipEngine:
    def __init__(self, state_dict, device, precision=None):
        self.lib = L.load()
        self.precision_name = precision or default_precision()
        if self.precision_name not in PRECISIONS:
            raise ValueError("otvm_amd: unknown precision %r (choose from %s)" % (self.precision_name, sorted(PRECISIONS)))
        self.precision = PRECISIONS[self.precision_name]
        self.conv_precision = CONV_PRECISIONS[self.precision_name]
        self.dev = torch.device(device)
        if self.dev.type != "cuda":
            raise RuntimeError("otvm_amd: the HIP path needs a GPU device (got %s); there is no CPU fallback" % device)
        self.sd = {k: v.detach().to(self.dev, torch.float32).contiguous() for k, v in state_dict.items()
                   if v.is_floating_point()}
        self.W = {}
        self._keep = []
        self.plans = {}
        self.bank = []
        self.free_slots = []
        self.stream = 0
        self.prof = None
        self.pending = None
        self.ev_dec = None
        self.frame_counter = 0
        self.conv_calls = 0
        self.last_T_read = 0
        self.parity = 0
        self.side = None
        self.side2 = None
        import os
        self.use_side_stream = os.environ.get("OTVM_SIDE_STREAM", "1") != "0"
        self.check_level = int(os.environ.get("OTVM_CHECK_FINITE", "1") or 0)
        self.check_finite = self.check_level >= 2
        self.guard_flag = torch.full((1,), GUARD_CLEAR, dtype=torch.int32, device=self.dev)
        self._guard_host = torch.full((1,), GUARD_CLEAR, dtype=torch.int32).pin_memory()
        self._guard_ev = None
        self._guard_what = {}
        self.use_graphs = USE_GRAPHS
        self.gn_predict_off = False
        self.gn_predict_log = []
        self.gn_predict_suspect_from = None
        self._diag_host = None
        self._diag_ev = None
        self.keep_hid_d = False
        self.foreground = False
        self.background = None
        self._fgr_on = False
        self.last_fgr = self.last_rgba_u8 = self.last_comp_u8 = None
        self.last_fgr_b = self.last_rgba_u8_b = self.last_comp_u8_b = None
        global _TUNE_FILE_LOADED
        if not _TUNE_FILE_LOADED:
            _TUNE_FILE_LOADED = True
            with torch.cuda.device(self.dev):
                _load_tune_file()
        self._pack_all()

    def _stream(self):
        return torch.cuda.current_stream(self.dev).cuda_stream

    def _pack(self, name, w, ws=False, scale=None, bias=None, i_pad=None):
        cw = pack_conv_weight(self.lib, self.dev, w, ws, scale, i_pad, split=(self.precision == L.PREC_F16X3),
                              stream=self._stream())
        cw.bias = bias
        self._keep.append((w, scale))
        self.W[name] = cw

    def _wave_frag(self, cw):
        if cw.w_wfrag is None:
            O_pad = cw.w_hi.numel() // cw.K_pad
            cw.w_wfrag = torch.zeros(int(self.lib.otvm_wave_weight_bytes_f16x3(O_pad, cw.K_pad)), dtype=torch.uint8, device=self.dev)
            L.check(self.lib.otvm_pack_wave_weight_f16x3(cw.w_hi.data_ptr(), cw.w_lo.data_ptr(), O_pad, cw.K_pad,
                                                         cw.w_wfrag.data_ptr(), self._stream()), "pack_wave_weight")
        return cw.w_wfrag

    def _gram_tables(self, cw):
        return gram_tables(self.lib, cw)

    def _fold_bn(self, bn):
        sd = self.sd
        n = sd[bn + ".weight"].numel()
        scale = torch.empty(n, dtype=torch.float32, device=self.dev)
        bias = torch.empty(n, dtype=torch.float32, device=self.dev)
        L.check(self.lib.otvm_fold_bn(sd[bn + ".weight"].data_ptr(), sd[bn + ".bias"].data_ptr(),
                                      sd[bn + ".running_mean"].data_ptr(), sd[bn + ".running_var"].data_ptr(), 1e-5, n,
                                      scale.data_ptr(), bias.data_ptr(), self._stream()), "fold_bn " + bn)
        return scale, bias

    def _pack_all(self):
        with torch.cuda.device(self.dev):
            self._pack_all_on_device()

    def _pack_all_on_device(self):
        sd = self.sd
        for k, v in sd.items():
            if not (k.endswith(".weight") and v.dim() == 4):
                continue
            name = k[:-7]
            if k.startswith("NET."):
                ws = not ("conv_up4" in k or ".pred." in k)
                if name in ("NET.decoder.conv_up4.4", "NET.refine.pred.4"):
                    continue
                i_pad = 80 if name in ("NET.decoder.conv_up4.0", "NET.refine.conv1.0") else None
                self._pack(name, v, ws=ws, bias=sd.get(name + ".bias"), i_pad=i_pad)
            elif ".Encoder_" in k:
                if ".conv1_" in k or name.endswith("Encoder_M.conv1"):
                    continue
                bn = name.replace(".conv", ".bn").replace("downsample.0", "downsample.1")
                scale, bias = self._fold_bn(bn)
                self._pack(name, v, scale=scale, bias=bias)
            else:
                self._pack(name, v, bias=sd.get(name + ".bias"))
        if FUSE_STM_BLOCK and self.precision == L.PREC_F16X3:
            for enc in ("trimap.model.Encoder_M.", "trimap.model.Encoder_Q."):
                if enc + "res2.0.conv3.weight" not in sd:
                    continue
                s3, b3 = self._fold_bn(enc + "res2.0.bn3")
                sdn, bdn = self._fold_bn(enc + "res2.0.downsample.1")
                wcat = torch.cat([sd[enc + "res2.0.conv3.weight"] * s3[:, None, None, None],
                                  sd[enc + "res2.0.downsample.0.weight"] * sdn[:, None, None, None]], dim=1)
                self._pack(enc + "res2.0.conv3cat", wcat, bias=b3 + bdn)
                for b in range(3):
                    for cname in ("conv1", "conv2", "conv3cat" if b == 0 else "conv3"):
                        self._wave_frag(self.W[enc + "res2.%d.%s" % (b, cname)])
        self.GP = {}
        if FUSE_GN_PREDICT and self.precision == L.PREC_F16X3:
            for name, cw in list(self.W.items()):
                if (name.startswith("NET.encoder.layer") and name.endswith(".conv3") and cw.kh == 1 and cw.kw == 1 and cw.bias is None
                        and cw.I % 64 == 0 and cw.O % 32 == 0 and cw.I_pad == cw.I):
                    self.GP[name] = self._gram_tables(cw)
        e = "trimap.model.Encoder_M."
        wcat = torch.cat([sd[e + "conv1_h.weight"], sd[e + "conv1.weight"], sd[e + "conv1_m.weight"],
                          sd[e + "conv1_o.weight"], sd[e + "conv1_a.weight"]], dim=1)
        scale, bias = self._fold_bn(e + "bn1")
        self._pack(e + "stem", wcat, scale=scale, bias=bias, i_pad=24)
        up1 = self.W.get("NET.decoder.conv_up1.0")
        self.W_ppm = None
        if PPM_ALGEBRA and FUSE_PPM_HEAD and up1 is not None and (up1.O, up1.I, up1.kh, up1.kw) == (256, 3072, 3, 3):
            O_pad = up1.w.numel() // up1.K_pad
            wk = up1.w.view(O_pad, up1.K_pad)[:256, :9 * up1.I_pad].reshape(256, 3, 3, up1.I_pad)
            w_main = wk[..., :2048].permute(0, 3, 1, 2).contiguous()
            self._pack("NET.decoder.conv_up1.0.main", w_main, ws=False, bias=up1.bias)
            self.W_ppm = wk[..., 2048:3072].reshape(256, 9, 4, 256).permute(2, 1, 3, 0).contiguous()
        torch.cuda.synchronize(self.dev)

    def guard(self, act, what, stream, tag=None):
        if self.check_level <= 0:
            return
        tag = self.frame_counter - 1 if tag is None else tag
        limit = F16_LIMIT if self.precision == L.PREC_F16X3 else float("inf")
        for b in range(act.B):
            v = act.img(b) if act.B > 1 else act
            L.check(self.lib.otvm_finite_guard(v.ptr, v.P, v.C, v.ld, limit, max(int(tag), 0), self.guard_flag.data_ptr(), stream),
                    "finite_guard " + what)

    def scan_now(self, act, what, stream):
        self.guard(act, what, stream)
        v = int(self.guard_flag.item())
        if v != GUARD_CLEAR:
            self.guard_flag.fill_(GUARD_CLEAR)
            raise FloatingPointError("otvm_amd: |x| >= 65504 (or inf / NaN) at the %s, frame %d" % (what, v))

    def _guard_raise(self, frame):
        self.guard_flag.fill_(GUARD_CLEAR)
        self._guard_host.fill_(GUARD_CLEAR)
        self._guard_ev = None
        raise FloatingPointError(
            "otvm_amd: a value outside fp16's range (|x| >= 65504, inf or NaN) reached the recurrent state (memorised key / "
            "value, hidden state or propagated trimap logits) at frame %d of the sequence: the f16x3 path splits fp32 operands "
            "into fp16 halves and cannot represent it.  Everything from that frame on is invalid.  Rerun with "
            "model.precision = 'f32' (exact-fp32 MFMA, no range limit), or OTVM_CHECK_FINITE=3 to find the layer." % frame)

    def guard_check(self, sync):
        if self.check_level <= 0:
            return
        if sync:
            v = int(self.guard_flag.item())
            if v != GUARD_CLEAR:
                self._guard_raise(v)
            return
        if self._guard_ev is not None and self._guard_ev.query():
            self._guard_ev = None
            v = int(self._guard_host[0])
            if v != GUARD_CLEAR:
                self._guard_raise(v)
        if self._guard_ev is None and self.frame_counter % 8 == 0:
            self._guard_host.copy_(self.guard_flag, non_blocking=True)
            self._guard_ev = torch.cuda.Event()
            self._guard_ev.record(torch.cuda.current_stream(self.dev))

    def _predict_verdict(self, pl, words):
        import struct
        import warnings
        verdict = "ok"
        for name, q, slot in pl._predicted:
            kappa = struct.unpack("f", struct.pack("i", int(words[2 * slot])))[0]
            flags = int(words[2 * slot + 1])
            if flags or kappa > GN_PREDICT_KAPPA_OFF:
                why = ("non-finite statistic" if flags & 1 else "fp16 operand saturated") if flags else "kappa %.3g" % kappa
                self.gn_predict_log.append((name, kappa, "off: " + why))
                if not self.gn_predict_off:
                    warnings.warn("otvm_amd: the predicted GroupNorm statistics of %s are ill-conditioned (%s): the prediction is "
                                  "switched off for this model (statistics accumulated from the convolution's output instead; "
                                  "OTVM_GN_PREDICT=0 does the same from the start)" % (name, why))
                self.gn_predict_off = True
                verdict = "off"
            elif kappa > GN_PREDICT_KAPPA_P3 and q.passes == 1:
                q.passes = 3
                self.gn_predict_log.append((name, kappa, "f16x3 Gram matrix"))
                if verdict == "ok":
                    verdict = "p3"
        if verdict == "p3":
            pl.retire_graphs()
        return verdict

    def predict_check(self, pl, sync):
        if not pl._predicted or self.gn_predict_off:
            return "ok"
        if sync:
            words = pl.diag.cpu().tolist()
            pl.diag.zero_()
            self._diag_ev = None
            return self._predict_verdict(pl, words)
        verdict = "ok"
        if self._diag_ev is not None and self._diag_ev[0].query():
            ev, owner = self._diag_ev
            self._diag_ev = None
            if owner is pl:
                verdict = self._predict_verdict(pl, self._diag_host.tolist())
        if self._diag_ev is None and self.frame_counter % 8 == 0:
            if self._diag_host is None:
                self._diag_host = torch.zeros(2 * 64, dtype=torch.int32).pin_memory()
            self._diag_host.copy_(pl.diag, non_blocking=True)
            ev = torch.cuda.Event()
            ev.record(torch.cuda.current_stream(self.dev))
            self._diag_ev = (ev, pl)
        return verdict

    def _drop_plans(self):
        torch.cuda.synchronize(self.dev)
        self.plans.clear()
        self.bank, self.free_slots, self.pending = [], [], None
        self.ev_dec = None
        self.last_plan = None

    def plan(self, H, W, B=1):
        key = (H, W) if B == 1 else (H, W, B)
        if self.keep_hid_d:
            key = key + ("hid_d",)
        if self._fgr_on:
            key = key + ("fgr",)
        if key not in self.plans:
            self.plans[key] = FramePlan(self, H, W, B)
        return self.plans[key]

    def reset(self):
        self.free_slots.extend(self.bank)
        self.bank = []

    def _vec3(self, key):
        return [float(x) for x in self.sd[key].flatten().tolist()]

    def frame(self, *args, **kw):
        with torch.cuda.device(self.dev):
            return self._frame(*args, **kw)

    def frame_batch(self, *args, **kw):
        with torch.cuda.device(self.dev):
            return self._frame_batch(*args, **kw)

    def _frame(self, a, fg, bg, tri_gt=None, first_frame=False, last_frame=False, memorize=False, max_memory_num=2,
               dilate_kernel=None, frame_id=None, cls_override=None, frames_rgb=False, inputs_ready=None, keyframe=False,
               labels=None):
        return self._frame_batch([a], [fg], [bg], [tri_gt], first_frame, last_frame, memorize, max_memory_num, dilate_kernel,
                                 frame_id, None if cls_override is None else [cls_override], frames_rgb, inputs_ready,
                                 keyframe=keyframe, labels=labels)[0]

    def _frame_batch(self, a_l, fg_l, bg_l, tri_gt_l, first_frame=False, last_frame=False, memorize=False, max_memory_num=2,
                     dilate_kernel=None, frame_id=None, cls_override=None, frames_rgb=False, inputs_ready=None, train=None,
                     _recheck=2, keyframe=False, labels=None):
        dev, lib = self.dev, self.lib
        f32 = torch.float32
        B = len(a_l)
        if not (len(fg_l) == len(bg_l) == len(tri_gt_l) == B) or B < 1:
            raise ValueError("otvm_amd: a / fg / bg / tri_gt lists must have the same length")
        keyframe = bool(keyframe)
        if keyframe or labels is not None:
            if B > 1 or train is not None:
                raise NotImplementedError("otvm_amd: keyframe / labels apply to a single sequence (not to lock-step batches)")
            if labels is not None and first_frame:
                raise ValueError("otvm_amd: labels correct a propagated trimap; a first frame takes its trimap as tri_gt")
            if keyframe and labels is None and tri_gt_l[0] is None:
                raise ValueError("otvm_amd: keyframe=True needs the frame's trimap as tri_gt")
            if max_memory_num < 2:
                raise ValueError("otvm_amd: keyframe / labels need max_memory_num >= 2 (a bank of %d slot(s) holds no anchors)"
                                 % max_memory_num)
        kf_full = keyframe and labels is None and not first_frame
        no_segment = first_frame or kf_full
        main = torch.cuda.current_stream(dev)
        if isinstance(inputs_ready, torch.cuda.Event):
            main.wait_event(inputs_ready)
        ins, H, W, converted = [], None, None, False
        u8 = fg_l[0].dtype == torch.uint8
        for a, fg, bg in zip(a_l, fg_l, bg_l):
            a_in, fg_in, bg_in = a, fg, bg
            a = a.to(dev, f32).contiguous()
            if (fg.dtype == torch.uint8) != u8:
                raise ValueError("otvm_amd: the frames of a batch must share one dtype")
            if u8:
                if bg.dtype != torch.uint8 or fg.dim() != 3 or fg.shape[-1] != 3 or bg.shape != fg.shape:
                    raise ValueError("otvm_amd: uint8 frames must be [H,W,3] for both fg and bg, got %s / %s"
                                     % (tuple(fg.shape), tuple(bg.shape)))
                fg, bg = fg.to(dev).contiguous(), bg.to(dev).contiguous()
                h_, w_ = int(fg.shape[0]), int(fg.shape[1])
            else:
                if frames_rgb:
                    raise ValueError("otvm_amd: frames_rgb applies to uint8 [H,W,3] frames only (fp32 input is BGR planar)")
                fg = fg.to(dev, f32).contiguous()
                bg = bg.to(dev, f32).contiguous()
                h_, w_ = int(fg.shape[-2]), int(fg.shape[-1])
            if H is None:
                H, W = h_, w_
            elif (h_, w_) != (H, W):
                raise ValueError("otvm_amd: the sequences of a batch must share one resolution (%dx%d vs %dx%d)" % (w_, h_, W, H))
            converted = converted or a is not a_in or fg is not fg_in or bg is not bg_in
            if a.dim() != 5 or a.shape[0] != 1 or a.shape[1] != 1 or tuple(a.shape[-2:]) != (H, W):
                raise ValueError("otvm_amd: inputs must be [1,1,C,H,W] (batch 1, one frame), got a %s for %dx%d frames"
                                 % (tuple(a.shape), H, W))
            ins.append((a, fg, bg))
        if inputs_ready is not None and converted:
            inputs_ready = None
        if first_frame:
            self._fgr_on = bool(self.foreground) and train is None
        elif bool(self.foreground) != self._fgr_on and train is None:
            raise RuntimeError("otvm_amd: `foreground` may only change at a clip's first frame")
        lab = None
        if labels is not None:
            lab = labels if torch.is_tensor(labels) else torch.as_tensor(labels)
            if lab.dtype != torch.uint8 or tuple(lab.shape) != (H, W):
                raise ValueError("otvm_amd: labels must be a uint8 [%d,%d] map, got %s %s" % (H, W, lab.dtype, tuple(lab.shape)))
            lab = lab.to(dev).contiguous()
        pl = self.plan(H, W, B)
        stream = self._stream()
        outs = [dict(scaled_imgs=torch.empty((1, 1, 3, H, W), dtype=f32, device=dev),
                     alpha=torch.empty((1, 1, 1, H, W), dtype=f32, device=dev),
                     alpha_u8=torch.empty((H, W), dtype=torch.uint8, device=dev),
                     tri_out=torch.empty((1, 1, 3, H, W), dtype=f32, device=dev),
                     tri_gt_out=torch.empty((1, 1, 3, H, W), dtype=f32, device=dev)) for _ in range(B)]
        if first_frame:
            if self.pending is not None:
                self.free_slots.append(self.pending["slot"])
            self.pending = None
            self.reset()
            self.frame_counter = 0
            self.gn_predict_suspect_from = None
        if frame_id is None:
            frame_id = self.frame_counter
        self.frame_counter += 1
        self.guard_check(sync=False)
        pend, self.pending = self.pending, None
        if pend is not None and pend["plan"] is not pl:
            self._memorize(pend, stream)
            pend = None
        par = self.parity
        self.parity ^= 1
        pps = []
        for (a, fg, bg) in ins:
            pp = L.PreprocessParams()
            pp.a = a.data_ptr()
            if u8:
                pp.fg_u8, pp.bg_u8, pp.u8_rgb = fg.data_ptr(), bg.data_ptr(), 1 if frames_rgb else 0
            else:
                pp.fg, pp.bg = fg.data_ptr(), bg.data_ptr()
            pp.H, pp.W, pp.Hp, pp.Wp, pp.lh, pp.lw = H, W, pl.Hp, pl.Wp, pl.lh, pl.lw
            for name, key in (("mean", "IMG_MEAN"), ("std", "IMG_STD"), ("mean_q", "trimap.model.Encoder_Q.mean"),
                              ("std_q", "trimap.model.Encoder_Q.std"), ("mean_m", "trimap.model.Encoder_M.mean"),
                              ("std_m", "trimap.model.Encoder_M.std")):
                setattr(pp, name, (C.c_float * 3)(*self._consts(key)))
            pps.append(pp)
        use_side = self.prof is None and self.use_side_stream and not no_segment
        ev_q = ev_s2 = None
        split = None
        if use_side:
            if self.side is None:
                self.side = torch.cuda.Stream(device=dev)
            side = self.side
            if self.ev_dec is not None:
                side.wait_event(self.ev_dec)
            if isinstance(inputs_ready, torch.cuda.Event):
                side.wait_event(inputs_ready)
            elif inputs_ready is not True:
                ev_in = torch.cuda.Event()
                ev_in.record(main)
                side.wait_event(ev_in)
            for b, (a, fg, bg) in enumerate(ins):
                for t_ in (a, fg, bg):
                    t_.record_stream(side)
                pq = L.PreprocessParams.from_buffer_copy(pps[b])
                sq = pl.SQ.img(b)
                pq.sq, pq.sq_ld = sq.ptr, sq.ld
                L.check(lib.otvm_preprocess(C.byref(pq), side.cuda_stream), "preprocess (query encoder input)")
            pl.run("segment_a", side.cuda_stream, side)
            ev_q = torch.cuda.Event()
            ev_q.record(side)
            if self.side2 is None:
                self.side2 = torch.cuda.Stream(device=dev)
            side2 = self.side2
            ev_m0 = torch.cuda.Event()
            ev_m0.record(main)
            side2.wait_event(ev_q)
            side2.wait_event(ev_m0)
            if PRE_ON_S2:
                for b, (a, fg, bg) in enumerate(ins):
                    for t_ in (a, fg, bg):
                        t_.record_stream(side2)
                    outs[b]["scaled_imgs"].record_stream(side2)
                pl.clear_stats(side2.cuda_stream)
                for b in range(B):
                    self._preprocess_rest(pl, pps[b], par, outs[b]["scaled_imgs"], False, side2.cuda_stream, b)
            if self.precision == L.PREC_F16X3:
                if pend is not None:
                    nb, _ = bank_update(self.bank, pend["slot"], pend["first_frame"], pend["memorize"], pend["max_memory_num"],
                                        pend["anchor"])
                    old = [s_ for s_ in nb if s_ is not pend["slot"]]
                    fresh = [pend["slot"]] if any(s_ is pend["slot"] for s_ in nb) else []
                else:
                    old, fresh = list(self.bank), []
                if old:
                    split = pl.memory_read_begin(old, fresh, side2.cuda_stream)
            pl.run("segment_skip", side2.cuda_stream, side2)
            ev_s2 = torch.cuda.Event()
            ev_s2.record(side2)
        if pend is not None:
            self._memorize(pend, stream)
        if not (use_side and PRE_ON_S2):
            pl.clear_stats(stream)
            for b in range(B):
                self._preprocess_rest(pl, pps[b], par, outs[b]["scaled_imgs"], not use_side, stream, b)

        tri_srcs = []
        for b in range(B):
            tri_gt, tri_gt_out, a = tri_gt_l[b], outs[b]["tri_gt_out"], ins[b][0]
            if tri_gt is not None:
                tri_src = tri_gt.to(dev, f32).contiguous()
                L.check(lib.otvm_onehot_argmax3(tri_src.data_ptr(), H * W, tri_gt_out.data_ptr(), stream), "onehot")
            else:
                if dilate_kernel is None:
                    raise ValueError("otvm_amd: tri_gt=None needs a fixed dilate_kernel (reference eval always sets one)")
                ws = pl.raws("tfa_ws", H * W, torch.uint8)[b]
                L.check(lib.otvm_trimap_from_alpha(a.data_ptr(), H, W, int(dilate_kernel), tri_gt_out.data_ptr(),
                                                   ws.data_ptr(), stream), "trimap_from_alpha")
                tri_src = tri_gt_out
            tri_srcs.append(tri_src)

        self.last_T_read = 0
        if no_segment:
            for b in range(B):
                L.check(lib.otvm_pad_trimap(tri_srcs[b].data_ptr(), H, W, pl.PROBS_B[b].data_ptr(), pl.Hp, pl.Wp, pl.lh, pl.lw,
                                            stream), "pad_trimap")
            self.ev_dec = torch.cuda.Event()
            self.ev_dec.record(main)
        else:
            if ev_q is not None:
                main.wait_event(ev_q)
            else:
                pl.run("segment_a", stream)
                pl.run("segment_skip", stream)
            if not self.bank:
                raise RuntimeError("otvm_amd: non-first frame with an empty memory bank (call with first_frame=True first)")
            self.last_T_read = len(self.bank)
            if self.prof is not None:
                e0, e1 = torch.cuda.Event(enable_timing=True), torch.cuda.Event(enable_timing=True)
                e0.record()
            if split is not None:
                if len(split["old"]) + len(split["fresh"]) != len(self.bank) or not all(
                        any(b_ is s_ for b_ in self.bank) for s_ in split["old"] + split["fresh"]):
                    raise RuntimeError("otvm_amd: the early memory read visited a different bank than the policy produced")
                pl.memory_read_fresh(split, stream)
                main.wait_event(ev_s2)
                pl.memory_read_merge(split, stream)
            else:
                if ev_s2 is not None:
                    main.wait_event(ev_s2)
                pl.memory_read(self.bank, stream)
            if self.prof is not None:
                e1.record()
                self.prof.append(("memory_read", 1280.0 * len(self.bank) * pl.hw * pl.hw * B, e0, e1, len(self.bank)))
            pl.run("segment_b", stream)
            self.guard(pl.L4, "propagated trimap logits", stream, frame_id)
            if lab is not None:
                L.check(lib.otvm_trimap_apply_labels(pl.PROBS_B[0].data_ptr(), lab.data_ptr(), H, W, pl.Hp, pl.Wp, pl.lh, pl.lw,
                                                     stream), "trimap_apply_labels")
            if train is not None and train.get("seg_logits") is not None:
                for b in range(B):
                    l4 = pl.L4.img(b)
                    L.check(lib.otvm_upsample4_logits3(l4.ptr, l4.H, l4.W, l4.ld, train["seg_logits"][b].data_ptr(), stream),
                            "upsample4_logits3")
            if not EVDEC_LATE:
                self.ev_dec = torch.cuda.Event()
                self.ev_dec.record(main)
        pl.encode(stream, cls_override)
        if not no_segment and EVDEC_LATE:
            self.ev_dec = torch.cuda.Event()
            self.ev_dec.record(main)
        pl.run("fba", stream)
        pl.run("fba_tail%d" % par, stream)
        self.guard(pl.SMs[par].ch(0, 16), "hidden state", stream, frame_id)
        if train is not None:
            sd, P_ = self.sd, pl.P
            img = pl.D80.ch(67, 3)
            for b in range(B):
                hd, hr = pl.HID_D.img(b), pl.SMs[par].ch(0, 16).img(b)
                L.check(lib.otvm_fba_head_train(hd.ptr, hd.ld, sd["NET.decoder.conv_up4.4.weight"].data_ptr(),
                                                sd["NET.decoder.conv_up4.4.bias"].data_ptr(), 7, img.img(b).ptr, img.ld, P_,
                                                train["dec7"][b].data_ptr(), 0, stream), "fba_head_train (decoder)")
                L.check(lib.otvm_fba_head_train(hr.ptr, hr.ld, sd["NET.refine.pred.4.weight"].data_ptr(),
                                                sd["NET.refine.pred.4.bias"].data_ptr(), 10, img.img(b).ptr, img.ld, P_,
                                                train["ref7"][b].data_ptr(), train["ref_logits"][b].data_ptr(), stream),
                        "fba_head_train (refinement)")
                if train.get("tri0") is not None:
                    smv = pl.SMs[par].ch(16, 8).img(b)
                    L.check(lib.otvm_trimap_to_sm(train["tri0"][b].data_ptr(), P_, smv.ptr, smv.ld, stream), "trimap_to_sm")
        if not last_frame:
            slot = pl.new_slot()
            slot["frame"] = frame_id
            self.pending = dict(plan=pl, par=par, slot=slot, first_frame=first_frame, memorize=memorize,
                                max_memory_num=max_memory_num, anchor=first_frame or keyframe)
        for b in range(B):
            o = outs[b]
            L.check(lib.otvm_crop_outputs(pl.ALPHA_P_B[b].data_ptr(), pl.TRI_P_B[b].data_ptr(), pl.Hp, pl.Wp, H, W, pl.lh, pl.lw,
                                          o["alpha"].data_ptr(), o["alpha_u8"].data_ptr(), o["tri_out"].data_ptr(), stream), "crop")
        self.last_alpha_u8 = outs[0]["alpha_u8"]
        self.last_alpha_u8_b = [o["alpha_u8"] for o in outs]
        self._fgr_outputs(pl, outs, H, W, u8 and frames_rgb, stream)
        self.last_plan = pl
        if pl._predicted and not self.gn_predict_off:
            verdict = self.predict_check(pl, sync=first_frame)
            if verdict == "off" and not first_frame:
                import warnings
                self.gn_predict_suspect_from = max(0, self.frame_counter - 1 - 16)
                warnings.warn("otvm_amd: predicted GroupNorm statistics went ill-conditioned in the middle of a clip: its frames "
                              "from %d on are suspect (engine.gn_predict_suspect_from); the rest of the clip keeps the current "
                              "plan, the next clip runs on the accumulated route" % self.gn_predict_suspect_from)
            if first_frame and verdict != "ok" and _recheck > 0:
                if verdict == "off":
                    self._drop_plans()
                return self._frame_batch(a_l, fg_l, bg_l, tri_gt_l, first_frame, last_frame, memorize, max_memory_num, dilate_kernel,
                                         frame_id, cls_override, frames_rgb, None, train, _recheck=_recheck - 1, keyframe=keyframe,
                                         labels=labels)
        elif self.gn_predict_off and pl._predicted and first_frame:
            self._drop_plans()
            return self._frame_batch(a_l, fg_l, bg_l, tri_gt_l, first_frame, last_frame, memorize, max_memory_num, dilate_kernel,
                                     frame_id, cls_override, frames_rgb, None, train, _recheck=0, keyframe=keyframe,
                                     labels=labels)
        if self.check_finite and not all(bool(torch.isfinite(o["alpha"]).all()) for o in outs):
            raise FloatingPointError("otvm_amd: non-finite alpha at frame %d -- an activation probably left fp16's range on the "
                                     "f16x3 path; rerun with model.precision = 'f32' (exact-fp32 MFMA)" % frame_id)
        if self.check_finite and pl.fgr and not all(bool(torch.isfinite(f).all()) for f in self.last_fgr_b):
            raise FloatingPointError("otvm_amd: non-finite foreground at frame %d -- an activation probably left fp16's range on "
                                     "the f16x3 path; rerun with model.precision = 'f32' (exact-fp32 MFMA)" % frame_id)
        if last_frame or self.check_finite:
            self.guard_check(sync=True)
        return [(o["scaled_imgs"], o["tri_out"], o["tri_gt_out"], o["alpha"], ins[b][0]) for b, o in enumerate(outs)]

    def _fgr_outputs(self, pl, outs, H, W, rgb, stream):
        if not pl.fgr:
            self.last_fgr = self.last_rgba_u8 = self.last_comp_u8 = None
            self.last_fgr_b = self.last_rgba_u8_b = self.last_comp_u8_b = None
            return
        dev, B = self.dev, len(outs)
        bgs = self.background if isinstance(self.background, list) else [self.background] * B
        if len(bgs) != B:
            raise ValueError("otvm_amd: %d backgrounds for a batch of %d sequences" % (len(bgs), B))
        fl, rl, cl = [], [], []
        for b in range(B):
            q = L.FgrParams()
            q.alpha_p, q.fgr_p = pl.ALPHA_P_B[b].data_ptr(), pl.FGR_P_B[b].data_ptr()
            q.Hp, q.Wp, q.H, q.W, q.lh, q.lw = pl.Hp, pl.Wp, H, W, pl.lh, pl.lw
            q.u8_rgb = int(bool(rgb))
            fgr = torch.empty((3, H, W), dtype=torch.float32, device=dev)
            rgba = torch.empty((H, W, 4), dtype=torch.uint8, device=dev)
            comp, bg = None, bgs[b]
            q.fgr, q.rgba_u8 = fgr.data_ptr(), rgba.data_ptr()
            if bg is not None:
                comp = torch.empty((H, W, 3), dtype=torch.uint8, device=dev)
                q.comp_u8 = comp.data_ptr()
                if torch.is_tensor(bg):
                    if bg.dtype != torch.uint8 or tuple(bg.shape) != (H, W, 3) or bg.device != dev or not bg.is_contiguous():
                        raise ValueError("otvm_amd: the background must be a contiguous uint8 [%d,%d,3] tensor on %s (got %s %s)"
                                         % (H, W, dev, bg.dtype, tuple(bg.shape)))
                    q.bg_u8 = bg.data_ptr()
                else:
                    q.bg_color[:] = [int(c) for c in bg]
            L.check(self.lib.otvm_fgr_outputs(C.byref(q), stream), "fgr_outputs")
            fl.append(fgr), rl.append(rgba), cl.append(comp)
        self.last_fgr, self.last_rgba_u8, self.last_comp_u8 = fl[0], rl[0], cl[0]
        self.last_fgr_b, self.last_rgba_u8_b, self.last_comp_u8_b = fl, rl, cl

    def _preprocess_rest(self, pl, pp, par, scaled_imgs, with_sq, stream, b=0):
        pm = L.PreprocessParams.from_buffer_copy(pp)
        pm.scaled_imgs = scaled_imgs.data_ptr()
        x11 = pl.X11.img(b)
        pm.x11, pm.x11_ld = x11.ptr, x11.ld
        if with_sq:
            sq = pl.SQ.img(b)
            pm.sq, pm.sq_ld = sq.ptr, sq.ld
        smv = pl.SMs[par].ch(16, 8).img(b)
        pm.sm, pm.sm_ld = smv.ptr, smv.ld
        d80 = pl.D80.img(b)
        pm.d80, pm.d80_ld = d80.ptr, d80.ld
        L.check(self.lib.otvm_preprocess(C.byref(pm), stream), "preprocess")

    def _memorize(self, pend, stream, tstream=None):
        pl, slot = pend["plan"], pend["slot"]
        pl.run("mem_stem%d" % pend["par"], stream, tstream)
        pl.run("mem_trunk", stream, tstream)
        pl.kv_into_slot(slot, stream)
        self.bank, released = bank_update(self.bank, slot, pend["first_frame"], pend["memorize"], pend["max_memory_num"],
                                          pend["anchor"])
        self.free_slots.extend(released)

    def _bank_with_pending(self):
        bank = list(self.bank)
        pend = self.pending
        if pend is not None:
            bank, _ = bank_update(bank, pend["slot"], pend["first_frame"], pend["memorize"], pend["max_memory_num"],
                                  pend["anchor"])
        return bank

    def bank_frames(self):
        return [s["frame"] for s in self._bank_with_pending()]

    def bank_anchors(self):
        return [s["frame"] for s in self._bank_with_pending() if _is_anchor(s)]

    def drop_non_anchors(self):
        pend = self.pending
        if pend is not None and (pend["anchor"] or pend["first_frame"]):
            self.flush()
        elif pend is not None:
            self.pending = None
            self.free_slots.append(pend["slot"])
        self.free_slots.extend(s for s in self.bank if not _is_anchor(s))
        self.bank = [s for s in self.bank if _is_anchor(s)]

    def flush(self):
        pend, self.pending = self.pending, None
        if pend is not None:
            with torch.cuda.device(self.dev):
                self._memorize(pend, self._stream())
                self.guard_check(sync=True)

    def _consts(self, key):
        c = getattr(self, "_const_cache", None)
        if c is None:
            c = self._const_cache = {}
        if key not in c:
            c[key] = self._vec3(key)
        return c[key]


class FramePlan:

    def __init__(self, eng, H, W, B=1):
        self.e = eng
        self.lib = eng.lib
        self.dev = eng.dev
        self.H, self.W, self.B = H, W, B
        self.fgr = bool(eng._fgr_on)
        if B > 1 and eng.precision != L.PREC_F16X3:
            raise NotImplementedError("otvm_amd: batched sequences (B > 1) run on the f16x3 path only")
        self.lw, self.uw, self.lh, self.uh = pad_amounts(H, W, 32)
        self.Hp, self.Wp = H + self.lh + self.uh, W + self.lw + self.uw
        self.P = self.Hp * self.Wp
        self._bufs = {}
        self._keep = []
        self.graphs, self._graph_warm = {}, {}
        self._n_conv = {}
        self._retired_graphs = []
        self._stm128 = []
        self._fused_stats = []
        self._convs = []
        self._predicted = []
        self.diag = None
        self.n_gn = 0
        self.steps = {}
        self._build()
        self.stats_bs = max(self.n_gn, 1) * 64
        self.stats = torch.zeros(self.B * self.stats_bs, dtype=torch.float64, device=self.dev)
        self._bind_stats()
        self.autotune()

    @staticmethod
    def _signature(p):
        return (p.H, p.W, p.Cin, p.in_ld, p.Cout, p.out_ld, p.kh, p.kw, p.stride, p.pad, p.dil, p.in_relu, p.act, int(bool(p.bias)),
                int(bool(p.residual)), p.res_ld, int(bool(p.gn_stats)), int(bool(p.in_scale)), int(bool(p.splitk_ws)), p.precision,
                max(1, p.batch), int(bool(p.res_scale)), int(bool(p.in_res)))

    def _time_conv(self, p, code, stream, reps=3):
        p.tune = code
        fn = self.lib.otvm_conv2d
        self.e.conv_calls += 1 + reps
        L.check(fn(C.byref(p), stream), "autotune warm-up")
        e0, e1 = torch.cuda.Event(enable_timing=True), torch.cuda.Event(enable_timing=True)
        e0.record()
        for _ in range(reps):
            fn(C.byref(p), stream)
        e1.record()
        return e0, e1, reps

    def tune_convs(self, convs):
        if not (AUTOTUNE and self.e.precision == L.PREC_F16X3):
            return
        stream = torch.cuda.current_stream(self.dev).cuda_stream
        codes = (C.c_int * 128)()
        timed_any = False
        for p, name in convs:
            sig = self._signature(p)
            if sig not in _TUNE_CACHE:
                n = int(self.lib.otvm_conv2d_candidates(C.byref(p), codes, 128))
                cands = [0] + [int(codes[i]) for i in range(n)]
                if not WAVE_TILE:
                    cands = [c for c in cands if c // 16 - 1 != 9]
                self._time_conv(p, 0, stream, reps=2)
                timed = [(c,) + self._time_conv(p, c, stream) for c in cands + [0]]
                torch.cuda.synchronize(self.dev)
                ms = {}
                for c, e0, e1, r in timed:
                    t = e0.elapsed_time(e1) / r
                    ms[c] = min(ms.get(c, t), t)
                best = min(ms, key=ms.get)
                if ms[best] > 0.97 * ms[0]:
                    best = 0
                _TUNE_CACHE[sig] = best
                TUNE_LOG.append((name, sig, best, ms))
                timed_any = True
            p.tune = _TUNE_CACHE[sig]
        if timed_any:
            _save_tune_file()

    def _resolve_stm128(self, timed):
        stream = torch.cuda.current_stream(self.dev).cuda_stream
        timed_any = False
        for S in self._stm128:
            i = 0
            while i < len(S):
                st = S[i]
                if not (isinstance(st[0], str) and st[0] == "stm128"):
                    i += 1
                    continue
                _, fused, U, q, name = st
                key = (-128, q.H, q.W, max(1, q.batch), q.x_ld, q.y_ld)
                if FUSE_STM_BLOCK128 >= 2 or not timed:
                    choice = _TUNE_CACHE.get(key, -1) if FUSE_STM_BLOCK128 < 2 else (STM128_TILE or -1)
                elif key in _TUNE_CACHE:
                    choice = _TUNE_CACHE[key]
                else:
                    def run(c, reps):
                        e0, e1 = torch.cuda.Event(enable_timing=True), torch.cuda.Event(enable_timing=True)
                        e0.record()
                        for _ in range(reps):
                            if c == 0:
                                for u in U:
                                    u[0](*u[1], stream)
                            else:
                                q.tile = c
                                L.check(fused[0](*fused[1], stream), name)
                        e1.record()
                        return e0, e1, reps
                    self.e.conv_calls += 3 * 7 + 3 * 7
                    run(0, 2)
                    timed_ = [(c,) + run(c, 3) for c in (0, 1, 2, 3, 0, 1, 2, 3)]
                    torch.cuda.synchronize(self.dev)
                    ms = {}
                    for c, e0, e1, r in timed_:
                        t = e0.elapsed_time(e1) / r
                        ms[c] = min(ms.get(c, t), t)
                    choice = min(ms, key=ms.get)
                    _TUNE_CACHE[key] = choice
                    TUNE_LOG.append((name + " (fused bottleneck: 0 = three launches, 1 / 2 / 3 = fused on 8x16 / 8x8 / 4x8 pixels)",
                                     (q.H, q.W, 512, q.x_ld, 512, q.y_ld, 3, 3, 1, 1, 1), choice, ms))
                    timed_any = True
                if choice == 0:
                    S[i:i + 1] = U
                    i += len(U)
                else:
                    q.tile = max(choice, 0)
                    S[i] = fused
                    i += 1
        self._stm128 = []
        if timed_any:
            _save_tune_file()

    def autotune(self):
        if not (AUTOTUNE and self.e.precision == L.PREC_F16X3):
            self._resolve_stm128(timed=False)
            return
        filled = []
        gen = torch.Generator(device=self.dev)
        gen.manual_seed(0x07F3)
        for b in self._bufs.values():
            t = b.t if isinstance(b, Act) else b
            if not t.is_floating_point():
                continue
            if t.dtype == torch.float32:
                t.normal_(generator=gen)
            else:
                continue
            filled.append(t)
        H16, W16 = self.Hp // 16, self.Wp // 16
        tk = Act(torch.empty(self.B * self.hw * 128, dtype=torch.float32, device=self.dev), H16, W16, 128, B=self.B, bs=self.hw * 128)
        tv = Act(torch.empty(self.B * self.hw * 512, dtype=torch.float32, device=self.dev), H16, W16, 512, B=self.B, bs=self.hw * 512)
        n0, k0 = len(self._convs), len(self._keep)
        self.conv([], self.r4m, "trimap.model.KV_M_r4.Key", tk, pad=1)
        self.conv([], self.r4m, "trimap.model.KV_M_r4.Value", tv, pad=1)
        self.tune_convs(self._convs)
        self._resolve_stm128(timed=FUSE_STM_BLOCK128 == 1)
        torch.cuda.synchronize(self.dev)
        del self._convs[n0:], self._keep[k0:]
        for t in filled:
            t.zero_()
        self.stats.zero_()
        torch.cuda.synchronize(self.dev)

    def retire_graphs(self):
        self._retired_graphs.extend(self.graphs.values())
        self.graphs, self._graph_warm = {}, {}

    def clear_stats(self, stream):
        L.check(self.lib.otvm_clear(self.stats.data_ptr(), self.stats.numel() * 8, stream), "clear GroupNorm statistics")

    def buf(self, name, H, W, C):
        key = (name, H, W, C)
        if key not in self._bufs:
            self._bufs[key] = Act(torch.zeros(self.B * H * W * C, dtype=torch.float32, device=self.dev), H, W, C, B=self.B,
                                  bs=H * W * C)
        return self._bufs[key]

    def raw(self, name, n, dtype=torch.float32):
        key = ("raw", name, n, dtype)
        if key not in self._bufs:
            self._bufs[key] = torch.zeros(n, dtype=dtype, device=self.dev)
        return self._bufs[key]

    def raws(self, name, n, dtype=torch.float32):
        t = self.raw(name, n * self.B, dtype)
        return [t[b * n:(b + 1) * n] for b in range(self.B)]

    def conv(self, S, x, wname, out, stride=1, pad=0, dil=1, act=NONE, in_relu=0, residual=None, in_norm=None, in_res=None):
        w = self.e.W[wname]
        assert x.C == w.I_pad, (wname, x.C, w.I_pad)
        Ho = (x.H + 2 * pad - dil * (w.kh - 1) - 1) // stride + 1
        Wo = (x.W + 2 * pad - dil * (w.kw - 1) - 1) // stride + 1
        assert (out.H, out.W) == (Ho, Wo) and out.C >= w.O, (wname, out.H, out.W, Ho, Wo, out.C, w.O)
        p = conv_params(x, w, out, w.bias, stride, pad, dil, act, in_relu, residual, self.e.conv_precision, in_norm, self._ws)
        if in_res is not None:
            assert in_norm is not None and (in_res.H, in_res.W) == (x.H, x.W) and in_res.C >= w.I
            p.in_res, p.in_res_ld, p.in_res_bs = in_res.ptr, in_res.ld, in_res.bs
        self._keep.append(p)
        self._convs.append((p, wname))
        flops = 2 * Ho * Wo * w.O * w.kh * w.kw * w.I * x.B
        abytes = 4 * (x.B * x.H * x.W * w.I * (2 if in_res is not None else 1) + w.O * w.I * w.kh * w.kw
                      + x.B * Ho * Wo * w.O * (2 if residual is not None else 1))
        S.append((self.lib.otvm_conv2d, (C.byref(p),), "conv " + wname, flops, abytes, (x, out.ch(0, _rup(w.O, 4)) if out.C >= _rup(w.O, 4) else out)))
        return p

    def conv_head(self, S, x, wname, hid_out, head_w, head_b, n_out, img, alpha, alpha_stride, alpha_bs, tri=None, sm=None,
                  fgr=None):
        w = self.e.W[wname]
        assert x.C == w.I_pad and w.O == 16 and w.kh == 3
        out = hid_out if hid_out is not None else x
        p = conv_params(x, w, out, w.bias, 1, 1, 1, LEAKY, 0, None, self.e.conv_precision, None, None)
        if hid_out is None:
            p.out, p.out_ld, p.out_bs = 0, 0, 0
        h = L.HeadParams()
        h.w, h.b, h.n_out = head_w.data_ptr(), head_b.data_ptr(), n_out
        h.img, h.img_ld, h.img_bs = img.ptr, img.ld, img.bs
        h.P = x.P
        h.alpha_out, h.alpha_stride, h.alpha_bs = alpha, alpha_stride, alpha_bs
        h.tri_out, h.tri_bs = (0 if tri is None else tri), 3 * x.P
        if sm is not None:
            h.sm, h.sm_ld, h.sm_bs = sm.ptr, sm.ld, sm.bs
        if w.w16 is not None and HEAD16:
            h.w16 = w.w16.data_ptr()
        self._keep += [p, h]
        flops = 2 * x.P * w.O * 9 * w.I * x.B
        abytes = 4 * (x.B * x.P * w.I + w.O * w.I * 9 + x.B * x.P * (16 if hid_out is not None else 0) + x.B * x.P * 4)
        if fgr is not None:
            S.append((self.lib.otvm_conv2d_head_fgr, (C.byref(p), C.byref(h), fgr[0], fgr[1]), "conv " + wname + " (+ head, F)", flops,
                      abytes + 4 * x.B * x.P * 3, (x, hid_out if hid_out is not None else x)))
            return p
        S.append((self.lib.otvm_conv2d_head, (C.byref(p), C.byref(h)), "conv " + wname + " (+ head)", flops, abytes,
                  (x, hid_out if hid_out is not None else x)))
        return p

    def gn(self, S, x, name, act, out=None, residual=None, conv_p=None, res_norm=None):
        out = x if out is None else out
        sd = self.e.sd
        idx = self.n_gn
        self.n_gn += 1
        if conv_p is not None and FUSE_GN_STATS:
            self._fused_stats.append((conv_p, idx))
        else:
            S.append(("gn_stats", (x.ptr, x.P, x.C, x.ld), idx, (self.B, x.bs), "gn_stats " + name))
        q = L.GnApplyParams()
        q.x, q.P, q.C, q.ld = x.ptr, x.P, x.C, x.ld
        q.gamma, q.beta = sd[name + ".weight"].data_ptr(), sd[name + ".bias"].data_ptr()
        if residual is not None:
            q.residual, q.res_ld, q.res_bs = residual.ptr, residual.ld, residual.bs
        if res_norm is not None:
            q.res_scale, q.res_shift, q.res_act = res_norm[0], res_norm[1], res_norm[2]
            q.norm_bs = res_norm[3] if len(res_norm) > 3 else 0
        q.act, q.out, q.out_ld = act, out.ptr, out.ld
        q.batch, q.x_bs, q.out_bs = self.B, x.bs, out.bs
        self._keep.append(q)
        S.append(("gn_apply", q, idx, "gn_apply " + name))

    def gn_table_step(self, S, x, gn_name, producer_p):
        sd = self.e.sd
        idx = self.n_gn
        self.n_gn += 1
        self._fused_stats.append((producer_p, idx))
        tab = self.raw("gntab_" + gn_name, 2 * x.C * self.B)
        if FUSE_GN_TABLE and isinstance(producer_p, L.ConvParams):
            cnt = self.raw("gncnt_" + gn_name, self.B, torch.int32)
            producer_p.gn_gamma, producer_p.gn_beta = sd[gn_name + ".weight"].data_ptr(), sd[gn_name + ".bias"].data_ptr()
            producer_p.gn_scale_out, producer_p.gn_shift_out = tab.data_ptr(), tab.data_ptr() + 4 * x.C
            producer_p.gn_counter, producer_p.gn_tab_bs = cnt.data_ptr(), 2 * x.C
        else:
            S.append(("gn_table", (x.P, x.C, sd[gn_name + ".weight"].data_ptr(), sd[gn_name + ".bias"].data_ptr(),
                                   tab.data_ptr(), tab.data_ptr() + 4 * x.C), idx, 2 * x.C, "gn_table " + gn_name))
        return tab.data_ptr(), tab.data_ptr() + 4 * x.C, 2 * x.C

    def gn_then_conv(self, S, x, gn_name, gn_act, producer_p, wname, out, **kw):
        w = self.e.W[wname]
        sd = self.e.sd
        if FUSE_GN_APPLY and FUSE_GN_STATS and producer_p is not None:
            probe = conv_params(x, w, out, w.bias, kw.get("stride", 1), kw.get("pad", 0), kw.get("dil", 1), kw.get("act", NONE),
                                0, kw.get("residual"), self.e.conv_precision, (1, 1, gn_act))
            kind = self.lib.otvm_conv2d_input_norm_kind(C.byref(probe))
            if kind == 1 or (kind == 2 and (w.kh * w.kw == 1 or FUSE_GN_APPLY_IGEMM_KXK)):
                sc, sh, nbs = self.gn_table_step(S, x, gn_name, producer_p)
                return self.conv(S, x, wname, out, in_norm=(sc, sh, gn_act, nbs), **kw)
        self.gn(S, x, gn_name, gn_act, conv_p=producer_p)
        return self.conv(S, x, wname, out, **kw)

    def _bind_stats(self):
        base, sbs = self.stats.data_ptr(), self.stats_bs
        for conv_p, idx in self._fused_stats:
            conv_p.gn_stats = base + idx * 512
            conv_p.gn_bs = sbs
        for key, S in self.steps.items():
            for i, st in enumerate(S):
                if st[0] == "gn_stats":
                    _, a, idx, (nb, x_bs), label = st
                    S[i] = (self.lib.otvm_gn_stats_b, a + (base + idx * 512, nb, x_bs, sbs), label)
                elif st[0] == "gn_table":
                    _, a, idx, nbs, label = st
                    S[i] = (self.lib.otvm_gn_table_b, (base + idx * 512,) + a + (self.B, sbs, nbs), label)
                elif st[0] == "ppm_add":
                    _, a, b, label = st
                    S[i] = (self.lib.otvm_ppm_conv_add, a + (self._ppm_stats.gn_stats + 8 * b * sbs,), label)
                elif st[0] == "gn_apply":
                    _, q, idx, label = st
                    q.stats, q.stats_bs = base + idx * 512, sbs
                    S[i] = (self.lib.otvm_gn_apply_b, (C.byref(q),), label)

    def upsample(self, S, x, out, add=None, norm=None):
        S.append((self.lib.otvm_upsample_bilinear_b,
                  (x.ptr, x.H, x.W, x.C, x.ld, 0 if norm is None else norm[0], 0 if norm is None else norm[1],
                   0 if norm is None else norm[2], 0 if add is None else add.ptr, 0 if add is None else add.ld,
                   out.ptr, out.H, out.W, out.ld, x.B, x.bs, 0 if add is None else add.bs, out.bs,
                   0 if norm is None else norm[3]), "upsample"))

    def gn_then_upsample(self, S, x, gn_name, gn_act, producer_p, out):
        if FUSE_GN_APPLY and FUSE_GN_STATS and producer_p is not None:
            sc, sh, nbs = self.gn_table_step(S, x, gn_name, producer_p)
            self.upsample(S, x, out, norm=(sc, sh, gn_act, nbs))
        else:
            self.gn(S, x, gn_name, gn_act, conv_p=producer_p)
            self.upsample(S, x, out)

    def maxpool(self, S, x, out):
        S.append((self.lib.otvm_maxpool3x3s2_b, (x.ptr, x.H, x.W, x.C, x.ld, out.ptr, out.ld, x.B, x.bs, out.bs), "maxpool"))

    def gn_bottleneck(self, S, x, p, planes, stride, dil, has_ds, out):
        Ho, Wo = x.H // stride, x.W // stride
        t1 = self.buf("bt1", x.H, x.W, planes)
        cp = self.conv(S, x, p + ".conv1", t1)
        t2 = self.buf("bt2", Ho, Wo, planes)
        cp = self.gn_then_conv(S, t1, p + ".bn1", RELU, cp, p + ".conv2", t2, stride=stride, pad=dil, dil=dil)
        if self._predicted_tail(S, x, p, planes, stride, has_ds, out, t2, cp):
            return
        t3 = self.buf("bt3", Ho, Wo, planes * 4)
        if FUSE_GN_APPLY_IGEMM:
            cp3 = self.gn_then_conv(S, t2, p + ".bn2", RELU, cp, p + ".conv3", t3)
        else:
            self.gn(S, t2, p + ".bn2", RELU, conv_p=cp)
            cp3 = self.conv(S, t2, p + ".conv3", t3)
        res_norm = None
        if has_ds:
            idt = self.buf("btd", Ho, Wo, planes * 4)
            cp = self.conv(S, x, p + ".downsample.0", idt, stride=stride)
            if FUSE_GN_APPLY and FUSE_GN_STATS:
                sc, sh, nbs = self.gn_table_step(S, idt, p + ".downsample.1", cp)
                res_norm = (sc, sh, NONE, nbs)
            else:
                self.gn(S, idt, p + ".downsample.1", NONE, conv_p=cp)
        else:
            idt = x
        self.gn(S, t3, p + ".bn3", RELU, out=out, residual=idt, conv_p=cp3, res_norm=res_norm)

    def _predicted_tail(self, S, x, p, planes, stride, has_ds, out, t2, cp2):
        e, lib, sd = self.e, self.lib, self.e.sd
        wname = p + ".conv3"
        gp = e.GP.get(wname) if hasattr(e, "GP") else None
        if not (FUSE_GN_PREDICT and not e.gn_predict_off and gp is not None and FUSE_GN_APPLY and FUSE_GN_STATS and FUSE_GN_TABLE and FUSE_GN_APPLY_IGEMM
                and cp2 is not None and (GN_PREDICT_DS or not has_ds) and t2.P >= GN_PREDICT_MIN_PIXELS
                and planes in GN_PREDICT_PLANES):
            return False
        w = e.W[wname]
        probe = conv_params(t2, w, out, None, 1, 0, 1, RELU, 0, x, e.conv_precision, (1, 1, RELU))
        if lib.otvm_conv2d_input_norm_kind(C.byref(probe)) != 2:
            return False
        B, C4 = self.B, planes * 4
        Ho, Wo = t2.H, t2.W
        sc, sh, nbs = self.gn_table_step(S, t2, p + ".bn2", cp2)
        rsc = rsh = None
        if has_ds:
            idt = self.buf("btd", Ho, Wo, C4)
            cpd = self.conv(S, x, p + ".downsample.0", idt, stride=stride)
            rsc, rsh, rnbs = self.gn_table_step(S, idt, p + ".downsample.1", cpd)
        else:
            idt = x
        nk = int(lib.otvm_gram_chunks(t2.P, planes, None))
        ent = int(lib.otvm_gram_entries(planes))
        gpart = self.raw("gram_g", B * nk * ent)
        spart = self.raw("gram_s", B * nk * planes)
        q = L.GramParams()
        q.x, q.P, q.C, q.ld = t2.ptr, t2.P, planes, t2.ld
        q.in_scale, q.in_shift, q.in_act = sc, sh, RELU
        q.gpart, q.spart, q.passes = gpart.data_ptr(), spart.data_ptr(), GN_PREDICT_PASSES
        q.batch, q.x_bs, q.norm_bs = B, t2.bs, nbs
        if self.diag is None:
            self.diag = self.raw("gnpred_diag", 2 * 64, torch.int32)
        slot = len(self._predicted)
        assert slot < 64
        q.diag = self.diag.data_ptr() + 8 * slot
        self._predicted.append((p, q, slot))
        self._keep.append(q)
        S.append((lib.otvm_gram_f16, (C.byref(q),), "gram " + p))
        tab = self.raw("gnpred_" + p, 2 * C4 * B)
        cnt = self.raw("gnpredcnt_" + p, B, torch.int32)
        r = L.GnPredictParams()
        r.gpart, r.spart, r.P, r.C, r.Cout = gpart.data_ptr(), spart.data_ptr(), t2.P, planes, C4
        r.Mp, r.v = gp[0].data_ptr(), gp[1].data_ptr()
        r.counter = cnt.data_ptr()
        r.ws = self.raw("gnpred_ws", B * int(lib.otvm_gn_predict_ws_bytes()) // 8, torch.float64).data_ptr()
        r.wscale, r.gamma, r.beta = w.w_scale.data_ptr(), sd[p + ".bn3.weight"].data_ptr(), sd[p + ".bn3.bias"].data_ptr()
        r.res_shift = 0 if rsh is None else rsh
        r.scale_eff, r.bias_eff = tab.data_ptr(), tab.data_ptr() + 4 * C4
        r.batch, r.tab_bs, r.rs_bs = B, 2 * C4, 0 if rsh is None else rnbs
        r.diag = q.diag
        self._keep.append(r)
        S.append((lib.otvm_gn_predict, (C.byref(r),), "gn_predict " + p))
        cp3 = self.conv(S, t2, wname, out, in_norm=(sc, sh, RELU, nbs), residual=idt, act=RELU)
        cp3.w_scale, cp3.bias, cp3.ws_bs = tab.data_ptr(), tab.data_ptr() + 4 * C4, 2 * C4
        if rsc is not None:
            cp3.res_scale, cp3.res_scale_bs = rsc, rnbs
        return True

    def bn_bottleneck(self, S, x, p, planes, stride, has_ds, out, tag):
        Ho, Wo = x.H // stride, x.W // stride
        W = self.e.W
        c3 = W.get(p + (".conv3cat" if has_ds else ".conv3"))
        if (FUSE_STM_BLOCK and self.e.precision == L.PREC_F16X3 and planes == 64 and stride == 1 and c3 is not None
                and c3.w_wfrag is not None and x.C == (64 if has_ds else 256)):
            c1, c2 = W[p + ".conv1"], W[p + ".conv2"]
            q = L.StmBottleneckParams(x.ptr, x.H, x.W, x.C, x.ld, out.ptr, out.ld,
                                      c1.w_wfrag.data_ptr(), c2.w_wfrag.data_ptr(), c3.w_wfrag.data_ptr(),
                                      c1.w_scale.data_ptr(), c2.w_scale.data_ptr(), c3.w_scale.data_ptr(),
                                      c1.bias.data_ptr(), c2.bias.data_ptr(), c3.bias.data_ptr(), x.B, x.bs, out.bs, 0)
            self._keep.append(q)
            P = x.B * x.H * x.W
            flops = 2 * P * (x.C * 64 + 9 * 64 * 64 + 64 * 256 + (x.C * 256 if has_ds else 0))
            abytes = 4 * (P * x.C + P * 256 + x.C * 64 + 9 * 64 * 64 + 64 * 256 + (x.C * 256 if has_ds else 0))
            S.append((self.lib.otvm_stm_bottleneck_f16x3, (C.byref(q),), "conv " + p + " (fused bottleneck)", flops, abytes,
                      (x, out.ch(0, 256) if out.C > 256 else out)))
            return
        c1, c2, c3 = W[p + ".conv1"], W[p + ".conv2"], W.get(p + ".conv3")
        fuse128 = (FUSE_STM_BLOCK128 and self.e.precision == L.PREC_F16X3 and self.e.conv_precision == L.PREC_F16X3 and planes == 128
                   and stride == 1 and not has_ds and x.C == 512 and c3 is not None
                   and all(c.w_wfrag is not None and c.bias is not None for c in (c1, c2, c3))
                   and x.H * x.W * x.ld * 4 < (1 << 31))
        U = [] if fuse128 else S
        t1 = self.buf(tag + "t1", x.H, x.W, planes)
        self.conv(U, x, p + ".conv1", t1, act=RELU)
        t2 = self.buf(tag + "t2", Ho, Wo, planes)
        self.conv(U, t1, p + ".conv2", t2, stride=stride, pad=1, act=RELU)
        if has_ds:
            idt = self.buf(tag + "td", Ho, Wo, planes * 4)
            self.conv(U, x, p + ".downsample.0", idt, stride=stride)
        else:
            idt = x
        self.conv(U, t2, p + ".conv3", out, residual=idt, act=RELU)
        if fuse128:
            q = L.StmBottleneckParams(x.ptr, x.H, x.W, x.C, x.ld, out.ptr, out.ld,
                                      c1.w_wfrag.data_ptr(), c2.w_wfrag.data_ptr(), c3.w_wfrag.data_ptr(),
                                      c1.w_scale.data_ptr(), c2.w_scale.data_ptr(), c3.w_scale.data_ptr(),
                                      c1.bias.data_ptr(), c2.bias.data_ptr(), c3.bias.data_ptr(), x.B, x.bs, out.bs, 0)
            self._keep.append(q)
            P = x.B * x.H * x.W
            flops = 2 * P * (512 * 128 + 9 * 128 * 128 + 128 * 512)
            abytes = 4 * (P * 512 * 2 + 512 * 128 * 2 + 9 * 128 * 128)
            fused = (self.lib.otvm_stm_bottleneck_f16x3, (C.byref(q),), "conv " + p + " (fused bottleneck)", flops, abytes,
                     (x, out.ch(0, 512) if out.C > 512 else out))
            S.append(("stm128", fused, U, q, p))
            self._stm128.append(S)

    def stm_trunk(self, S, stem_out, e, tag):
        H4, W4 = self.Hp // 4, self.Wp // 4
        x = self.buf(tag + "pool", H4, W4, 64)
        self.maxpool(S, stem_out, x)
        outs = {}
        for lname, n, planes, s0 in (("res2", 3, 64, 1), ("res3", 4, 128, 2), ("res4", 6, 256, 2)):
            for b in range(n):
                st = s0 if b == 0 else 1
                o = self.buf(tag + lname + ("a" if b % 2 == 0 else "b"), x.H // st, x.W // st, planes * 4)
                self.bn_bottleneck(S, x, e + "%s.%d" % (lname, b), planes, st, b == 0, o, tag)
                x = o
            outs[lname] = x
        return outs["res4"], outs["res3"], outs["res2"]

    def resblock(self, S, x, p, out, tag):
        r = self.buf(tag + "r", x.H, x.W, 256)
        self.conv(S, x, p + ".conv1", r, pad=1, in_relu=1)
        self.conv(S, r, p + ".conv2", out, pad=1, in_relu=1, residual=x)

    def _build(self):
        e, lib = self.e, self.lib
        Hp, Wp, P = self.Hp, self.Wp, self.P
        H2, W2, H4, W4, H8, W8, H16, W16 = Hp // 2, Wp // 2, Hp // 4, Wp // 4, Hp // 8, Wp // 8, Hp // 16, Wp // 16
        self.hw = H16 * W16

        self.SPLITK_WS = [self.raw("splitk_ws%d" % i, (16 << 20) * self.B) for i in range(4)]
        self._ws = self.SPLITK_WS[2]
        self.X11 = self.buf("X11", Hp, Wp, 12)
        self.SQ = self.buf("SQ", Hp, Wp, 4)
        self.SMs = [self.buf("SM0", Hp, Wp, 24), self.buf("SM1", Hp, Wp, 24)]
        self.D80 = self.buf("D80", Hp, Wp, 80)
        self.PROBS_B = self.raws("probs", 3 * P)
        self.CLS_B = self.raws("cls", P, torch.uint8)
        self.ALPHA_P_B = self.raws("alpha_p", P)
        self.TRI_P_B = self.raws("tri_p", 3 * P)
        self.FGR_P_B = self.raws("fgr_p", 3 * P) if self.fgr else None
        self.enc_ws_B = self.raws("enc_ws", _rup(int(lib.otvm_trimap_encode_ws_bytes(Hp, Wp)), 256), torch.uint8)
        self.PROBS, self.CLS, self.ALPHA_P, self.TRI_P = self.PROBS_B[0], self.CLS_B[0], self.ALPHA_P_B[0], self.TRI_P_B[0]

        S = []
        sd = e.sd
        q = "trimap.model.Encoder_Q."
        stem = self.buf("q_stem", H2, W2, 64)
        self.conv(S, self.SQ, q + "conv1", stem, stride=2, pad=3, act=RELU)
        r4, r3, r2 = self.stm_trunk(S, stem, q, "q_")
        self.QK = self.buf("QK", H16, W16, 128)
        self.M4 = self.buf("M4", H16, W16, 1024)
        self.conv(S, r4, "trimap.model.KV_Q_r4.Key", self.QK, pad=1)
        self.conv(S, r4, "trimap.model.KV_Q_r4.Value", self.M4.ch(512, 512), pad=1)
        self.steps["segment_a"] = S
        self._ws = self.SPLITK_WS[0]
        S = []
        d = "trimap.model.Decoder."
        SK = []
        self._ws = self.SPLITK_WS[3]
        skips = {}
        for rf, feat, (h, w) in (("RF3", r3, (H8, W8)), ("RF2", r2, (H4, W4))):
            s0 = self.buf("d_s0", h, w, 256)
            self.conv(SK, feat, d + rf + ".convFS", s0, pad=1)
            s1 = self.buf("d_s1", h, w, 256)
            self.resblock(SK, s0, d + rf + ".ResFS", s1, "fs%d" % h)
            skips[rf] = s1
        self.steps["segment_skip"] = SK
        self._ws = self.SPLITK_WS[0]
        m = self.buf("d_m4a", H16, W16, 256)
        self.conv(S, self.M4, d + "convFM", m, pad=1)
        m4 = self.buf("d_m4b", H16, W16, 256)
        self.resblock(S, m, d + "ResMM", m4, "d16")
        pm = m4
        for rf, (h, w) in (("RF3", (H8, W8)), ("RF2", (H4, W4))):
            mm = self.buf("d_mm", h, w, 256)
            self.upsample(S, pm, mm, add=skips[rf])
            mo = self.buf("d_mo", h, w, 256)
            self.resblock(S, mm, d + rf + ".ResMM", mo, "d%d" % h)
            pm = mo
        self.L4 = self.buf("L4", H4, W4, 4)
        self.conv(S, pm, d + "pred", self.L4, pad=1, in_relu=1)
        for b in range(self.B):
            S.append((lib.otvm_upsample4_softmax3, (self.L4.img(b).ptr, H4, W4, self.L4.ld, self.PROBS_B[b].data_ptr()), "up4softmax"))
        self.steps["segment_b"] = S

        S = []
        en = "NET.encoder."
        self.U3 = self.buf("U3", H2, W2, 320)
        self.U2 = self.buf("U2", H4, W4, 512)
        ppm_alg = FUSE_PPM_HEAD and self.e.W_ppm is not None
        self.PPMCAT = self.buf("PPMCAT", H8, W8, 2048 if ppm_alg else 3072)
        c1raw = self.buf("c1raw", H2, W2, 64)
        cp = self.conv(S, self.X11, en + "conv1", c1raw, stride=2, pad=3)
        c1 = self.U3.ch(256, 64)
        self.gn(S, c1raw, en + "bn1", RELU, out=c1, conv_p=cp)
        x = self.buf("e_pool", H4, W4, 64)
        self.maxpool(S, c1, x)
        cfg = {"layer1": (64, 3, 1, 1, 1), "layer2": (128, 4, 2, 1, 1), "layer3": (256, 6, 1, 1, 2),
               "layer4": (512, 3, 1, 2, 4)}
        for lname in ("layer1", "layer2", "layer3", "layer4"):
            planes, n, s0, d0, dn = cfg[lname]
            for b in range(n):
                st = s0 if b == 0 else 1
                last = b == n - 1
                if last and lname == "layer1":
                    o = self.U2.ch(256, 256)
                elif last and lname == "layer4":
                    o = self.PPMCAT.ch(0, 2048)
                else:
                    o = self.buf("e_" + lname + ("a" if b % 2 == 0 else "b"), x.H // st, x.W // st, planes * 4)
                self.gn_bottleneck(S, x, en + "%s.%d" % (lname, b), planes, st, d0 if b == 0 else dn, b == 0, o)
                x = o
        de = "NET.decoder."
        conv5 = self.PPMCAT.ch(0, 2048)
        self.POOL_B = self.raws("ppm_pool", 50 * 2048)
        self.POOL_WS_B = self.raws("ppm_ws", int(lib.otvm_ppm_pool_ws_bytes(H8, 2048)) // 4)
        for b in range(self.B):
            S.append((lib.otvm_ppm_pool, (conv5.img(b).ptr, H8, W8, 2048, conv5.ld, self.POOL_B[b].data_ptr(),
                                          self.POOL_WS_B[b].data_ptr()), "ppm_pool"))
        if FUSE_PPM_HEAD and self.e.W[de + "ppm.0.1"].I_pad == 2048 and self.e.W[de + "ppm.0.1"].O == 256:
            sd = self.e.sd
            ys = [self.buf("ppm_y%d" % i, s_, s_, 256) for i, s_ in enumerate((1, 2, 3, 6))]
            for b in range(self.B):
                hp = L.PpmHeadParams()
                hp.pooled, hp.C, hp.Cout, hp.act = self.POOL_B[b].data_ptr(), 2048, 256, LEAKY
                for i in range(4):
                    w = self.e.W[de + "ppm.%d.1" % i]
                    hp.K_pad, hp.out_ld = w.K_pad, ys[i].ld
                    hp.w[i], hp.bias[i] = w.w.data_ptr(), 0 if w.bias is None else w.bias.data_ptr()
                    hp.gamma[i], hp.beta[i] = sd[de + "ppm.%d.2.weight" % i].data_ptr(), sd[de + "ppm.%d.2.bias" % i].data_ptr()
                    hp.out[i] = ys[i].img(b).ptr
                self._keep.append(hp)
                S.append((lib.otvm_ppm_head, (C.byref(hp),), "ppm_head"))
            self._ppm_algebra = ppm_alg
            if not self._ppm_algebra:
                for i, y in enumerate(ys):
                    self.upsample(S, y, self.PPMCAT.ch(2048 + 256 * i, 256))
        else:
            self._ppm_algebra = False
            if self.B > 1:
                raise NotImplementedError("otvm_amd: batched sequences need the fused PPM head (OTVM_PPM_HEAD=1)")
            base = 0
            for i, s_ in enumerate((1, 2, 3, 6)):
                pin = Act(self.POOL_B[0], s_, s_, 2048, 2048, base * 2048)
                y = self.buf("ppm_y%d" % i, s_, s_, 256)
                cp = self.conv(S, pin, de + "ppm.%d.1" % i, y)
                self.gn_then_upsample(S, y, de + "ppm.%d.2" % i, LEAKY, cp, self.PPMCAT.ch(2048 + 256 * i, 256))
                base += s_ * s_
        u1 = self.buf("u1a", H8, W8, 256)
        if self._ppm_algebra:
            self.PPM_Z = self.raws("ppm_z", 9 * 50 * 256)
            for b in range(self.B):
                yp = (C.c_void_p * 4)(*[y.img(b).ptr for y in ys])
                self._keep.append(yp)
                S.append((lib.otvm_ppm_conv_z, (yp, ys[0].ld, self.e.W_ppm.data_ptr(), self.PPM_Z[b].data_ptr()), "ppm_conv_z"))
            self.conv(S, self.PPMCAT.ch(0, 2048), de + "conv_up1.0.main", u1, pad=1)
            for b in range(self.B):
                S.append(("ppm_add", (self.PPM_Z[b].data_ptr(), H8, W8, u1.img(b).ptr, u1.ld), b, "ppm_conv_add"))
            import types
            self._ppm_stats = types.SimpleNamespace(gn_stats=0, gn_bs=0)
            self.gn(S, u1, de + "conv_up1.1", LEAKY, conv_p=self._ppm_stats)
        else:
            cp = self.conv(S, self.PPMCAT, de + "conv_up1.0", u1, pad=1)
            self.gn(S, u1, de + "conv_up1.1", LEAKY, conv_p=cp)
        u1b = self.buf("u1b", H8, W8, 256)
        cp = self.conv(S, u1, de + "conv_up1.3", u1b, pad=1)
        self.gn_then_upsample(S, u1b, de + "conv_up1.4", LEAKY, cp, self.U2.ch(0, 256))
        u2 = self.buf("u2", H4, W4, 256)
        cp = self.conv(S, self.U2, de + "conv_up2.0", u2, pad=1)
        self.gn_then_upsample(S, u2, de + "conv_up2.1", LEAKY, cp, self.U3.ch(0, 256))
        u3 = self.buf("u3", H2, W2, 64)
        cp = self.conv(S, self.U3, de + "conv_up3.0", u3, pad=1)
        self.gn_then_upsample(S, u3, de + "conv_up3.1", LEAKY, cp, self.D80.ch(0, 64))
        h32 = self.buf("h32", Hp, Wp, 32)
        self.conv(S, self.D80, de + "conv_up4.0", h32, pad=1, act=LEAKY)
        img = self.D80.ch(67, 3)
        fuse_head = FUSE_HEAD and e.precision == L.PREC_F16X3 and e.W[de + "conv_up4.2"].w_frag is not None
        if fuse_head:
            hid_d = self.HID_D = self.buf("hid_d", Hp, Wp, 16) if e.keep_hid_d else None
            self.conv_head(S, h32, de + "conv_up4.2", hid_d, sd[de + "conv_up4.4.weight"], sd[de + "conv_up4.4.bias"], 7, img,
                           self.D80.ch(72, 1).ptr, self.D80.ld, self.D80.bs)
        else:
            hid_d = self.HID_D = self.buf("hid_d", Hp, Wp, 16)
            self.conv(S, h32, de + "conv_up4.2", hid_d, pad=1, act=LEAKY)
            for b in range(self.B):
                S.append((lib.otvm_fba_head,
                          (hid_d.img(b).ptr, hid_d.ld, sd[de + "conv_up4.4.weight"].data_ptr(), sd[de + "conv_up4.4.bias"].data_ptr(), 7,
                           img.img(b).ptr, img.ld, P, self.D80.ch(72, 1).img(b).ptr, self.D80.ld, 0, 0, 0), "fba_head7"))
        rf = "NET.refine."
        r0 = self.buf("r0", Hp, Wp, 64)
        cp = self.conv(S, self.D80, rf + "conv1.0", r0, pad=1)
        x, x_norm = r0, None
        w1 = e.W[rf + "layer1.conv1"]
        t1 = self.buf("rt1", Hp, Wp, 64)
        probe = conv_params(r0, w1, t1, w1.bias, 1, 1, 1, NONE, 0, None, e.conv_precision, (1, 1, LEAKY))
        if FUSE_GN_APPLY and FUSE_GN_STATS and lib.otvm_conv2d_accepts_input_norm(C.byref(probe)):
            sc, sh, nbs = self.gn_table_step(S, r0, rf + "conv1.1", cp)
            x_norm = (sc, sh, LEAKY, nbs)
        else:
            self.gn(S, r0, rf + "conv1.1", LEAKY, conv_p=cp)
        tail = None
        for l in ("layer1", "layer2"):
            cp = self.conv(S, x, rf + l + ".conv1", t1, pad=1, in_norm=x_norm)
            t2 = self.buf("rt2", Hp, Wp, 64)
            cp = self.gn_then_conv(S, t1, rf + l + ".bn1", RELU, cp, rf + l + ".conv2", t2, pad=1)
            if l == "layer2" and FUSE_REFINE_TAIL and FUSE_GN_APPLY and FUSE_GN_STATS and x_norm is None:
                w0 = e.W[rf + "pred.0"]
                probe = conv_params(t2, w0, h32, w0.bias, 1, 1, 1, LEAKY, 0, None, e.conv_precision, (1, 1, RELU))
                if lib.otvm_conv2d_accepts_input_residual(C.byref(probe)):
                    sc, sh, nbs = self.gn_table_step(S, t2, rf + l + ".bn2", cp)
                    tail = (t2, (sc, sh, RELU, nbs), x)
                    break
            o = self.buf("r_" + l, Hp, Wp, 64)
            self.gn(S, t2, rf + l + ".bn2", RELU, out=o, residual=x, conv_p=cp, res_norm=x_norm)
            x, x_norm = o, None
        if tail is not None:
            self.conv(S, tail[0], rf + "pred.0", h32, pad=1, act=LEAKY, in_norm=tail[1], in_res=tail[2])
        else:
            self.conv(S, x, rf + "pred.0", h32, pad=1, act=LEAKY)
        self.steps["fba"] = S
        for par in (0, 1):
            S = []
            SM = self.SMs[par]
            hid = SM.ch(0, 16)
            if fuse_head:
                self.conv_head(S, h32, rf + "pred.2", hid, sd[rf + "pred.4.weight"], sd[rf + "pred.4.bias"], 10, img,
                               self.ALPHA_P_B[0].data_ptr(), 1, P, tri=self.TRI_P_B[0].data_ptr(), sm=SM.ch(16, 8),
                               fgr=(self.FGR_P_B[0].data_ptr(), 3 * P) if self.fgr else None)
                self.steps["fba_tail%d" % par] = S
                continue
            self.conv(S, h32, rf + "pred.2", hid, pad=1, act=LEAKY)
            for b in range(self.B):
                args = (hid.img(b).ptr, hid.ld, sd[rf + "pred.4.weight"].data_ptr(), sd[rf + "pred.4.bias"].data_ptr(), 10,
                        img.img(b).ptr, img.ld, P, self.ALPHA_P_B[b].data_ptr(), 1, self.TRI_P_B[b].data_ptr(),
                        SM.ch(16, 8).img(b).ptr, SM.ld)
                if self.fgr:
                    S.append((lib.otvm_fba_head_fgr, args + (self.FGR_P_B[b].data_ptr(),), "fba_head10 (+ F)"))
                else:
                    S.append((lib.otvm_fba_head, args, "fba_head10"))
            self.steps["fba_tail%d" % par] = S

        self._ws = self.SPLITK_WS[1]
        m_ = "trimap.model.Encoder_M."
        stem = self.buf("m_stem", H2, W2, 64)
        for par in (0, 1):
            S = []
            self.conv(S, self.SMs[par], m_ + "stem", stem, stride=2, pad=3, act=RELU)
            self.steps["mem_stem%d" % par] = S
        S = []
        self.r4m, _, _ = self.stm_trunk(S, stem, m_, "m_")
        self.steps["mem_trunk"] = S
        self.mem_ws = None

    def run(self, key, stream, tstream=None):
        prof = self.e.prof
        nc = self._n_conv.get(key)
        if nc is None:
            nc = self._n_conv[key] = sum(1 for st in self.steps[key] if not isinstance(st[0], str) and st[2].startswith("conv "))
        self.e.conv_calls += nc
        if prof is None and self.e.check_level >= 3:
            for st in self.steps[key]:
                if isinstance(st[0], str):
                    continue
                if st[2].startswith("conv "):
                    self.e.guard(st[5][0], "input of " + st[2], stream)
                rc = st[0](*st[1], stream)
                if rc != 0:
                    L.check(rc, st[2])
                if st[2].startswith("conv "):
                    self.e.scan_now(st[5][1], "output of " + st[2], stream)
            return
        if prof is None:
            if graphs_wanted(self.e.use_graphs, self.P):
                g = self.graphs.get(key)
                if g is None and self._graph_warm.get(key):
                    g = torch.cuda.CUDAGraph()
                    with torch.cuda.graph(g, capture_error_mode="thread_local"):
                        self._launch(self.steps[key], torch.cuda.current_stream(self.dev))
                    self.graphs[key] = g
                if g is not None:
                    if tstream is None:
                        g.replay()
                    else:
                        with torch.cuda.stream(tstream):
                            g.replay()
                    return
                self._graph_warm[key] = True
            self._launch(self.steps[key], tstream if tstream is not None else torch.cuda.current_stream(self.dev), stream)
            return
        for st in self.steps[key]:
            if isinstance(st[0], str):
                continue
            if st[2].startswith("conv "):
                e0, e1 = torch.cuda.Event(enable_timing=True), torch.cuda.Event(enable_timing=True)
                e0.record()
                rc = st[0](*st[1], stream)
                e1.record()
                prof.append((st[2], st[3], e0, e1, st[4]))
            else:
                rc = st[0](*st[1], stream)
            if rc != 0:
                L.check(rc, st[2])

    def _launch(self, steps, tmain, handle=None):
        handle = tmain.cuda_stream if handle is None else handle
        for st in steps:
            f = st[0]
            if isinstance(f, str):
                raise RuntimeError("otvm_amd: unbound step %r in a launch list" % (f,))
            rc = f(*st[1], handle)
            if rc != 0:
                L.check(rc, st[2])

    def new_slot(self):
        e = self.e
        for i, s in enumerate(e.free_slots):
            if s["plan"] is self:
                return e.free_slots.pop(i)
        H16, W16, B = self.Hp // 16, self.Wp // 16, self.B
        slot = dict(hw=self.hw, plan=self, frame=-1,
                    k=Act(torch.zeros(B * self.hw * 128, dtype=torch.float32, device=self.dev), H16, W16, 128, B=B, bs=self.hw * 128),
                    v=Act(torch.zeros(B * self.hw * 512, dtype=torch.float32, device=self.dev), H16, W16, 512, B=B, bs=self.hw * 512))
        if e.precision == L.PREC_F16X3:
            nb = int(self.lib.otvm_bank_slot_bytes_f16x3(self.hw))
            slot["packed_b"] = [torch.zeros(nb, dtype=torch.uint8, device=self.dev) for _ in range(B)]
            slot["packed"] = slot["packed_b"][0]
        return slot

    def _mem_ws_for(self, b, need):
        if self.mem_ws is None:
            self.mem_ws = [None] * self.B
        w = self.mem_ws[b]
        if w is None or w.numel() < need:
            torch.cuda.synchronize(self.dev)
            w = self.mem_ws[b] = torch.empty(max(need, 2 * (0 if w is None else w.numel())), dtype=torch.uint8, device=self.dev)
        return w

    def memory_read(self, bank, stream):
        T = len(bank)
        need = int(self.lib.otvm_memory_read_ws_bytes(self.hw, T))
        for b in range(self.B):
            ws = self._mem_ws_for(b, need)
            out, qk = self.M4.ch(0, 512).img(b), self.QK.img(b)
            if self.e.precision == L.PREC_F16X3:
                slots = (C.c_void_p * T)(*[s["packed_b"][b].data_ptr() for s in bank])
                L.check(self.lib.otvm_memory_read_f16x3(qk.ptr, qk.ld, slots, T, self.hw, out.ptr, out.ld, ws.data_ptr(), stream),
                        "memory_read_f16x3")
                continue
            keys = (C.c_void_p * T)(*[s["k"].img(b).ptr for s in bank])
            vals = (C.c_void_p * T)(*[s["v"].img(b).ptr for s in bank])
            L.check(self.lib.otvm_memory_read(qk.ptr, qk.ld, keys, vals, T, self.hw, out.ptr, out.ld, ws.data_ptr(), stream),
                    "memory_read")

    def memory_read_begin(self, old, fresh, stream):
        lib = self.lib
        np_cap = int(lib.otvm_memory_read_f16x3_partial_count(len(old), self.hw))
        if fresh:
            np_cap += int(lib.otvm_memory_read_f16x3_partial_count(len(fresh), self.hw))
        need = np_cap * self.hw * (512 + 2) * 4
        wss, done = [], 0
        for b in range(self.B):
            ws = self._mem_ws_for(b, need)
            qk = self.QK.img(b)
            arr = (C.c_void_p * len(old))(*[s["packed_b"][b].data_ptr() for s in old])
            end = C.c_int(0)
            L.check(lib.otvm_memory_read_f16x3_partial(qk.ptr, qk.ld, arr, len(old), self.hw, ws.data_ptr(), np_cap, 0, C.byref(end),
                                                       stream), "memory_read_f16x3_partial")
            wss.append(ws)
            done = end.value
        return dict(old=old, fresh=fresh, np_cap=np_cap, done=done, ws=wss)

    def memory_read_fresh(self, split, stream):
        lib, n = self.lib, split["done"]
        if split["fresh"]:
            fr = split["fresh"]
            for b in range(self.B):
                qk = self.QK.img(b)
                arr = (C.c_void_p * len(fr))(*[s["packed_b"][b].data_ptr() for s in fr])
                end = C.c_int(0)
                L.check(lib.otvm_memory_read_f16x3_partial(qk.ptr, qk.ld, arr, len(fr), self.hw, split["ws"][b].data_ptr(),
                                                           split["np_cap"], n, C.byref(end), stream), "memory_read_f16x3_partial")
            n = end.value
        split["done"] = n

    def memory_read_merge(self, split, stream):
        for b in range(self.B):
            out = self.M4.ch(0, 512).img(b)
            L.check(self.lib.otvm_memory_read_f16x3_combine(split["ws"][b].data_ptr(), split["np_cap"], split["done"], self.hw,
                                                            out.ptr, out.ld, stream), "memory_read_f16x3_combine")

    def kv_into_slot(self, slot, stream):
        if "kv_steps" not in slot:
            S = []
            n0 = len(self._convs)
            self.conv(S, self.r4m, "trimap.model.KV_M_r4.Key", slot["k"], pad=1)
            self.conv(S, self.r4m, "trimap.model.KV_M_r4.Value", slot["v"], pad=1)
            self.tune_convs(self._convs[n0:])
            slot["kv_steps"] = S
        prof = self.e.prof
        self.e.conv_calls += len(slot["kv_steps"])
        for st in slot["kv_steps"]:
            if prof is not None:
                e0, e1 = torch.cuda.Event(enable_timing=True), torch.cuda.Event(enable_timing=True)
                e0.record()
            L.check(st[0](*st[1], stream), st[2])
            if prof is not None:
                e1.record()
                prof.append((st[2], st[3], e0, e1, st[4]))
            if prof is None and self.e.check_level >= 3:
                self.e.scan_now(st[5][1], "output of " + st[2], stream)
        self.e.guard(slot["k"], "memorised key", stream, slot["frame"])
        self.e.guard(slot["v"], "memorised value", stream, slot["frame"])
        if "packed_b" in slot:
            for b in range(self.B):
                L.check(self.lib.otvm_bank_pack_f16x3(slot["k"].img(b).ptr, slot["v"].img(b).ptr, self.hw,
                                                      slot["packed_b"][b].data_ptr(), stream), "bank_pack")

    def encode(self, stream, cls_override=None):
        for b in range(self.B):
            co = None if cls_override is None else (cls_override[b] if isinstance(cls_override, (list, tuple)) else cls_override)
            x11, d80 = self.X11.img(b), self.D80.img(b)
            L.check(self.lib.otvm_trimap_encode(self.PROBS_B[b].data_ptr(), self.Hp, self.Wp, 0 if co is None else co.data_ptr(),
                                                self.CLS_B[b].data_ptr(), x11.ptr, x11.ld, d80.ptr, d80.ld,
                                                self.enc_ws_B[b].data_ptr(), stream), "trimap_encode")
```

otvm_amd/lib.py:

```python
import ctypes as C
import os

_HERE = os.path.dirname(os.path.abspath(__file__))
LIB_PATH = os.environ.get("OTVM_HIP_LIB") or os.path.join(_HERE, "libotvm_hip.so")

vp, i32, i64, f32 = C.c_void_p, C.c_int, C.c_int64, C.c_float
PREC_F32, PREC_F16X3, PREC_F16 = 0, 1, 2
ABI_VERSION = 21


class ConvParams(C.Structure):
    _fields_ = [("inp", vp), ("H", i32), ("W", i32), ("Cin", i32), ("in_ld", i32),
                ("w", vp), ("K_pad", i32),
                ("bias", vp),
                ("residual", vp), ("res_ld", i32),
                ("out", vp), ("Ho", i32), ("Wo", i32), ("Cout", i32), ("out_ld", i32),
                ("kh", i32), ("kw", i32), ("stride", i32), ("pad", i32), ("dil", i32),
                ("in_relu", i32), ("act", i32),
                ("precision", i32), ("w_hi", vp), ("w_lo", vp), ("w_scale", vp), ("w_frag", vp),
                ("gn_stats", vp),
                ("in_scale", vp), ("in_shift", vp), ("in_act", i32),
                ("tune", i32),
                ("splitk_ws", vp), ("splitk_ws_bytes", i64),
                ("batch", i32), ("in_bs", i64), ("out_bs", i64), ("res_bs", i64), ("gn_bs", i32), ("norm_bs", i32),
                ("w_wfrag", vp),
                ("gn_gamma", vp), ("gn_beta", vp), ("gn_scale_out", vp), ("gn_shift_out", vp), ("gn_counter", vp), ("gn_tab_bs", i32),
                ("ws_bs", i32), ("res_scale", vp), ("res_scale_bs", i32),
                ("in_res", vp), ("in_res_ld", i32), ("in_res_bs", i64)]


class StmBottleneckParams(C.Structure):
    _fields_ = [("x", vp), ("H", i32), ("W", i32), ("Cin", i32), ("x_ld", i32), ("y", vp), ("y_ld", i32),
                ("w1f", vp), ("w2f", vp), ("w3f", vp), ("s1", vp), ("s2", vp), ("s3", vp), ("b1", vp), ("b2", vp), ("b3", vp),
                ("batch", i32), ("x_bs", i64), ("y_bs", i64), ("tile", i32)]


class GnApplyParams(C.Structure):
    _fields_ = [("x", vp), ("P", i64), ("C", i32), ("ld", i32), ("stats", vp), ("gamma", vp), ("beta", vp),
                ("residual", vp), ("res_ld", i32), ("res_scale", vp), ("res_shift", vp), ("res_act", i32), ("act", i32),
                ("out", vp), ("out_ld", i32),
                ("batch", i32), ("x_bs", i64), ("res_bs", i64), ("out_bs", i64), ("stats_bs", i32), ("norm_bs", i32)]


class HeadParams(C.Structure):
    _fields_ = [("w", vp), ("b", vp), ("n_out", i32), ("img", vp), ("img_ld", i32), ("P", i64), ("alpha_out", vp),
                ("alpha_stride", i32), ("tri_out", vp), ("sm", vp), ("sm_ld", i32),
                ("img_bs", i64), ("alpha_bs", i64), ("tri_bs", i64), ("sm_bs", i64), ("w16", vp)]


class GramParams(C.Structure):
    _fields_ = [("x", vp), ("P", i64), ("C", i32), ("ld", i32), ("in_scale", vp), ("in_shift", vp), ("in_act", i32),
                ("gpart", vp), ("spart", vp), ("passes", i32), ("batch", i32), ("x_bs", i64), ("norm_bs", i32), ("diag", vp)]


class GnPredictParams(C.Structure):
    _fields_ = [("gpart", vp), ("spart", vp), ("P", i64), ("C", i32), ("Cout", i32), ("Mp", vp), ("v", vp), ("ws", vp),
                ("counter", vp), ("wscale", vp), ("gamma", vp), ("beta", vp), ("res_shift", vp),
                ("scale_eff", vp), ("bias_eff", vp), ("stat_out", vp),
                ("batch", i32), ("tab_bs", i32), ("rs_bs", i32), ("diag", vp)]


class PreprocessParams(C.Structure):
    _fields_ = [("fg", vp), ("bg", vp), ("a", vp),
                ("H", i32), ("W", i32), ("Hp", i32), ("Wp", i32), ("lh", i32), ("lw", i32),
                ("mean", f32 * 3), ("std", f32 * 3), ("mean_q", f32 * 3), ("std_q", f32 * 3),
                ("mean_m", f32 * 3), ("std_m", f32 * 3),
                ("scaled_imgs", vp),
                ("x11", vp), ("x11_ld", i32), ("sq", vp), ("sq_ld", i32), ("sm", vp), ("sm_ld", i32),
                ("d80", vp), ("d80_ld", i32),
                ("fg_u8", vp), ("bg_u8", vp), ("u8_rgb", i32)]


class FgrParams(C.Structure):
    _fields_ = [("alpha_p", vp), ("fgr_p", vp), ("Hp", i32), ("Wp", i32), ("H", i32), ("W", i32), ("lh", i32), ("lw", i32),
                ("fgr", vp), ("rgba_u8", vp), ("comp_u8", vp), ("bg_u8", vp), ("bg_color", C.c_ubyte * 3), ("u8_rgb", i32)]


class GuidedParams(C.Structure):
    _fields_ = [("H", i32), ("W", i32), ("s", i32), ("h", i32), ("w", i32), ("r", i32), ("C", i32), ("eps", C.c_double),
                ("guide_full", vp), ("guide_work", vp), ("target", vp * 4), ("coef", vp), ("alpha", vp), ("alpha_u8", vp),
                ("fgr", vp)]


class MaskTrimapParams(C.Structure):
    _fields_ = [("mask", vp), ("H", i32), ("W", i32), ("lo", i32), ("hi", i32), ("t_fg", i32), ("t_bg", i32),
                ("trimap", vp), ("labels", vp), ("band_label", i32)]


class TemporalParams(C.Structure):
    _fields_ = [("H", i32), ("W", i32), ("alpha", vp), ("prev", vp), ("grey", vp), ("grey_prev", vp), ("flow", vp), ("tri", vp),
                ("th", i32), ("tw", i32), ("tri_scale", i32), ("strength", f32), ("inv_tau_colour", f32), ("inv_tau_alpha", f32),
                ("out", vp), ("out_u8", vp)]


class PpmHeadParams(C.Structure):
    _fields_ = [("pooled", vp), ("C", i32), ("K_pad", i32), ("Cout", i32),
                ("w", vp * 4), ("bias", vp * 4), ("gamma", vp * 4), ("beta", vp * 4), ("out", vp * 4),
                ("out_ld", i32), ("act", i32)]


_PROTOS = {
    "otvm_abi_version": (i32, []),
    "otvm_patch_weight_bytes_f16x3": (i64, [i32, i32]),
    "otvm_pack_patch_weight_f16x3": (i32, [vp, i32, i32, i32, vp, vp, vp]),
    "otvm_stem_weight_bytes_f16x3": (i64, [i32]),
    "otvm_wave_weight_bytes_f16x3": (i64, [i32, i32]),
    "otvm_pack_wave_weight_f16x3": (i32, [vp, vp, i32, i32, vp, vp]),
    "otvm_pack_stem_weight_f16x3": (i32, [vp, i32, i32, i32, vp, vp, vp]),
    "otvm_fold_bn": (i32, [vp, vp, vp, vp, f32, i32, vp, vp, vp]),
    "otvm_pack_conv_weight": (i32, [vp, i32, i32, i32, i32, i32, vp, vp, i32, i32, i32, vp]),
    "otvm_conv2d": (i32, [C.POINTER(ConvParams), vp]),
    "otvm_split_conv_weight_f16x3": (i32, [vp, i32, i32, i32, i32, i32, vp, vp, vp, vp]),
    "otvm_gn_stats": (i32, [vp, i64, i32, i32, vp, vp]),
    "otvm_gn_table": (i32, [vp, i64, i32, vp, vp, vp, vp, vp]),
    "otvm_conv2d_accepts_input_norm": (i32, [C.POINTER(ConvParams)]),
    "otvm_conv2d_input_norm_kind": (i32, [C.POINTER(ConvParams)]),
    "otvm_conv2d_accepts_input_residual": (i32, [C.POINTER(ConvParams)]),
    "otvm_conv2d_head": (i32, [C.POINTER(ConvParams), C.POINTER(HeadParams), vp]),
    "otvm_conv2d_head_fgr": (i32, [C.POINTER(ConvParams), C.POINTER(HeadParams), vp, i64, vp]),
    "otvm_head16_weight_bytes_f16x3": (i64, []),
    "otvm_pack_head16_weight_f16x3": (i32, [vp, i32, i32, i32, vp, vp, vp]),
    "otvm_conv2d_candidates": (i32, [C.POINTER(ConvParams), C.POINTER(i32), i32]),
    "otvm_gn_apply": (i32, [vp, i64, i32, i32, vp, vp, vp, vp, i32, vp, vp, i32, i32, vp, i32, vp]),
    "otvm_maxpool3x3s2": (i32, [vp, i32, i32, i32, i32, vp, i32, vp]),
    "otvm_upsample_bilinear": (i32, [vp, i32, i32, i32, i32, vp, vp, i32, vp, i32, vp, i32, i32, i32, vp]),
    "otvm_ppm_pool_ws_bytes": (i64, [i32, i32]),
    "otvm_ppm_pool": (i32, [vp, i32, i32, i32, i32, vp, vp, vp]),
    "otvm_ppm_head": (i32, [C.POINTER(PpmHeadParams), vp]),
    "otvm_stm_bottleneck_f16x3": (i32, [C.POINTER(StmBottleneckParams), vp]),
    "otvm_ppm_conv_z": (i32, [C.POINTER(vp), i32, vp, vp, vp]),
    "otvm_ppm_conv_add": (i32, [vp, i32, i32, vp, i32, vp, vp]),
    "otvm_memory_read_ws_bytes": (i64, [i32, i32]),
    "otvm_memory_read": (i32, [vp, i32, C.POINTER(vp), C.POINTER(vp), i32, i32, vp, i32, vp, vp]),
    "otvm_bank_slot_bytes_f16x3": (i64, [i32]),
    "otvm_bank_pack_f16x3": (i32, [vp, vp, i32, vp, vp]),
    "otvm_memory_read_f16x3": (i32, [vp, i32, C.POINTER(vp), i32, i32, vp, i32, vp, vp]),
    "otvm_memory_read_f16x3_partial_count": (i32, [i32, i32]),
    "otvm_memory_read_f16x3_partial": (i32, [vp, i32, C.POINTER(vp), i32, i32, vp, i32, i32, C.POINTER(i32), vp]),
    "otvm_memory_read_f16x3_combine": (i32, [vp, i32, i32, i32, vp, i32, vp]),
    "otvm_preprocess": (i32, [C.POINTER(PreprocessParams), vp]),
    "otvm_pad_trimap": (i32, [vp, i32, i32, vp, i32, i32, i32, i32, vp]),
    "otvm_upsample4_softmax3": (i32, [vp, i32, i32, i32, vp, vp]),
    "otvm_trimap_apply_labels": (i32, [vp, vp, i32, i32, i32, i32, i32, i32, vp]),
    "otvm_trimap_encode_ws_bytes": (i64, [i32, i32]),
    "otvm_trimap_encode": (i32, [vp, i32, i32, vp, vp, vp, i32, vp, i32, vp, vp]),
    "otvm_fba_head": (i32, [vp, i32, vp, vp, i32, vp, i32, i64, vp, i32, vp, vp, i32, vp]),
    "otvm_fba_head_fgr": (i32, [vp, i32, vp, vp, i32, vp, i32, i64, vp, i32, vp, vp, i32, vp, vp]),
    "otvm_fgr_outputs": (i32, [C.POINTER(FgrParams), vp]),
    "otvm_downsample_u8": (i32, [vp, i32, i32, i32, vp, vp]),
    "otvm_downsample_trimap": (i32, [vp, i32, i32, i32, vp, vp]),
    "otvm_downsample_labels": (i32, [vp, i32, i32, i32, vp, vp]),
    "otvm_guided_ws_bytes": (i64, [i32, i32, i32]),
    "otvm_guided_coeffs": (i32, [C.POINTER(GuidedParams), vp, vp]),
    "otvm_guided_apply": (i32, [C.POINTER(GuidedParams), vp]),
    "otvm_crop_outputs": (i32, [vp, vp, i32, i32, i32, i32, i32, i32, vp, vp, vp, vp]),
    "otvm_trimap_from_alpha": (i32, [vp, i32, i32, i32, vp, vp, vp]),
    "otvm_trimap_from_mask_ws_bytes": (i64, [i32, i32]),
    "otvm_trimap_from_mask": (i32, [C.POINTER(MaskTrimapParams), vp, vp]),
    "otvm_onehot_argmax3": (i32, [vp, i64, vp, vp]),
    "otvm_matting_metrics": (i32, [vp, vp, vp, vp, vp, vp, i64, vp, vp]),
    "otvm_matting_grad_conn": (i32, [vp, vp, vp, i32, i32, vp, vp, vp, vp]),
    "otvm_matting_grad_conn_ws_bytes": (i64, [i32, i32]),
    "otvm_matting_grad_conn_params": (i32, [vp, vp, vp]),
    "otvm_optflow_farneback": (i32, [vp, vp, i32, i32, vp, vp, vp]),
    "otvm_optflow_farneback_ws_bytes": (i64, [i32, i32]),
    "otvm_optflow_farneback_params": (i32, [i32, i32, vp, vp, vp, vp, vp]),
    "otvm_matting_messddt": (i32, [vp, vp, vp, vp, vp, vp, i32, i32, vp, vp, vp, vp]),
    "otvm_luma_u8": (i32, [vp, i32, i32, i32, vp, vp]),
    "otvm_temporal_blend": (i32, [C.POINTER(TemporalParams), vp]),
    "otvm_gn_stats_b": (i32, [vp, i64, i32, i32, vp, i32, i64, i32, vp]),
    "otvm_gn_table_b": (i32, [vp, i64, i32, vp, vp, vp, vp, i32, i32, i32, vp]),
    "otvm_gn_apply_b": (i32, [C.POINTER(GnApplyParams), vp]),
    "otvm_maxpool3x3s2_b": (i32, [vp, i32, i32, i32, i32, vp, i32, i32, i64, i64, vp]),
    "otvm_upsample_bilinear_b": (i32, [vp, i32, i32, i32, i32, vp, vp, i32, vp, i32, vp, i32, i32, i32, i32, i64, i64, i64, i32, vp]),
    "otvm_fba_head_train": (i32, [vp, i32, vp, vp, i32, vp, i32, i64, vp, vp, vp]),
    "otvm_upsample4_logits3": (i32, [vp, i32, i32, i32, vp, vp]),
    "otvm_trimap_to_sm": (i32, [vp, i64, vp, i32, vp]),
    "otvm_scale_flip3": (i32, [vp, i64, i64, f32, vp, vp]),
    "otvm_trimask": (i32, [vp, i64, i64, vp, vp, vp, vp, vp]),
    "otvm_loss_fba_comp": (i32, [vp, vp, vp, vp, vp, vp, i64, i64, vp, vp, vp, vp, vp, vp]),
    "otvm_loss_grad_l1": (i32, [vp, vp, i64, i32, i32, f32, vp, vp]),
    "otvm_loss_exclusion_level": (i32, [vp, vp, i32, i32, i32, i32, f32, vp, vp, vp]),
    "otvm_avgpool2": (i32, [vp, i64, i32, i32, vp, vp]),
    "otvm_loss_lap_level": (i32, [vp, vp, i64, i32, i32, C.c_double, vp, vp, vp, vp]),
    "otvm_loss_temporal": (i32, [vp, vp, i32, i32, i64, vp, vp]),
    "otvm_loss_ce3": (i32, [vp, vp, i64, i64, vp, vp]),
    "otvm_finite_guard": (i32, [vp, i64, i32, i32, f32, i32, vp, vp]),
    "otvm_clear": (i32, [vp, i64, vp]),
    "otvm_gram_block": (i32, [i32]),
    "otvm_gram_entries": (i64, [i32]),
    "otvm_gram_chunks": (i32, [i64, i32, C.POINTER(i32)]),
    "otvm_gram_f16": (i32, [C.POINTER(GramParams), vp]),
    "otvm_gn_predict": (i32, [C.POINTER(GnPredictParams), vp]),
    "otvm_gn_predict_ws_bytes": (i64, []),
}

EXPORTED = sorted(list(_PROTOS) + ["otvm_last_error"])

_lib = None


def load():
    global _lib
    if _lib is not None:
        return _lib
    if not os.path.exists(LIB_PATH):
        raise RuntimeError(
            "otvm_amd: %s is missing -- build it with `python otvm_amd/csrc/build.py` "
            "(or __graft_entry__.build()).  There is no CPU/PyTorch fallback." % LIB_PATH)
    import torch
    lib = C.CDLL(LIB_PATH)
    lib.otvm_last_error.restype = C.c_char_p
    lib.otvm_last_error.argtypes = []
    for name, (res, args) in _PROTOS.items():
        fn = getattr(lib, name)
        fn.restype = res
        fn.argtypes = args
    got = lib.otvm_abi_version()
    if got != ABI_VERSION:
        raise RuntimeError("otvm_amd: %s has ABI version %d, this binding expects %d -- rebuild it with "
                           "`python otvm_amd/csrc/build.py`" % (LIB_PATH, got, ABI_VERSION))
    _lib = lib
    return lib


def check(rc, what=""):
    if rc != 0:
        raise RuntimeError("otvm_hip %s failed (%d): %s" % (what, rc, load().otvm_last_error().decode()))
```

Measured before the change: 47.73 frames/s.

## Fold 2x bilinear upsample and GN apply into consuming patch convolutions

Adds an UP variant of the f16x3 patch convolution kernel. For the upsampled channel blocks it loads the low-resolution source tile, applies the group-norm scale/shift and activation, stores it in LDS and bilinearly interpolates into the patch registers. The decoder's conv_up3.0, conv_up4.0 and refine conv1.0 can then read upsampled inputs directly, which removes the separate upsample pass and the write and re-read of the full-resolution tensor. Whether to fold is autotuned per site against the unfused route. The cost is extra LDS, more register pressure and interpolation work repeated in each consuming conv.

```diff
diff --git a/include/otvm_hip.h b/include/otvm_hip.h
--- a/include/otvm_hip.h
+++ b/include/otvm_hip.h
@@ -85,6 +85,17 @@
 int otvm_conv2d_accepts_input_norm(const otvm_conv_params* p);
 int otvm_conv2d_input_norm_kind(const otvm_conv_params* p);
 
+typedef struct otvm_conv_up_params {
+    const float* src; int Hi, Wi, Cu, src_ld;
+    int64_t src_bs;
+    const float* scale; const float* shift;
+    int act;
+    int norm_bs;
+    int tile_rows;
+} otvm_conv_up_params;
+int otvm_conv2d_up(const otvm_conv_params* p, const otvm_conv_up_params* u, void* stream);
+int otvm_conv2d_accepts_upsampled_input(const otvm_conv_params* p, const otvm_conv_up_params* u);
+
 int otvm_split_conv_weight_f16x3(const float* w_packed, int O, int O_pad, int K_pad, int taps, int I_pad,
                                  void* w_hi, void* w_lo, float* w_scale, void* stream);
 
diff --git a/otvm_amd/csrc/conv_patch_f16x3.hip b/otvm_amd/csrc/conv_patch_f16x3.hip
--- a/otvm_amd/csrc/conv_patch_f16x3.hip
+++ b/otvm_amd/csrc/conv_patch_f16x3.hip
@@ -2,6 +2,7 @@
 #include "common.h"
 #include "head_math.h"
 #include "f16x3_ops.h"
+#include "upfold_index.h"
 #include <type_traits>
 #include <stdlib.h>
 
@@ -47,6 +48,8 @@
     const float* in_res; int in_res_ld; int64_t in_res_bs;
     unsigned in_bytes, in_res_bytes;
     OtvmHeadArgs head; int64_t head_img_bs, head_alpha_bs, head_tri_bs, head_sm_bs, head_fgr_bs;
+    const float* up_src; const float* up_scale; const float* up_shift;
+    int up_Hi, up_Wi, up_ld, up_ncb, up_act, up_norm_bs; int64_t up_bs; unsigned up_bytes;
 };
 
 constexpr int CB = 16;
@@ -70,8 +73,24 @@
     return 4 * (k >> 1) + (k & 1) + ((r >= 4 && r < 12) ? 2 : 0);
 }
 
+__device__ __forceinline__ f32x4 otvm_up_norm(const f32x4 x, const f32x4 sc, const f32x4 sh, int act) {
+#pragma clang fp contract(off)
+    f32x4 v = x * sc;
+    v = v + sh;
+    v.x = otvm_act(v.x, act); v.y = otvm_act(v.y, act); v.z = otvm_act(v.z, act); v.w = otvm_act(v.w, act);
+    return v;
+}
+__device__ __forceinline__ f32x4 otvm_up_blend(const f32x4 v00, const f32x4 v01, const f32x4 v10, const f32x4 v11, float lx, float ly) {
+#pragma clang fp contract(off)
+    const float hx = 1.f - lx, hy = 1.f - ly;
+    const f32x4 a0 = hx * v00, a1 = lx * v01, b0 = hx * v10, b1 = lx * v11;
+    const f32x4 a = a0 + a1, b = b0 + b1;
+    const f32x4 ta = hy * a, tb = ly * b;
+    return ta + tb;
+}
+
 template <int TH, int BN, int NW, int DIL, int TAPG, bool INRES = false, bool HEAD = false, int NWN = 1, bool GLDS = false, int NPASS = 3,
-          bool M16 = false, bool FGR = false>
+          bool M16 = false, bool FGR = false, bool UP = false>
 __global__ __launch_bounds__(NW * 64)
 __attribute__((amdgpu_waves_per_eu((TAPG == 3 && BN <= 32 && !INRES) ? 3 : (M16 ? 2 : 1), (TAPG == 3 && BN <= 32 && !INRES) ? 3 : 10)))
 void conv_patch_f16x3_kernel(const PatchArgs pa) {
@@ -91,6 +110,10 @@
         if (p.residual) p.residual += zb * p.res_bs;
         if (p.gn_stats) p.gn_stats += zb * p.gn_bs;
         if (p.in_scale) { p.in_scale += zb * p.norm_bs; p.in_shift += zb * p.norm_bs; }
+        if constexpr (UP) {
+            p.up_src += zb * p.up_bs;
+            if (p.up_scale) { p.up_scale += zb * p.up_norm_bs; p.up_shift += zb * p.up_norm_bs; }
+        }
     }
     constexpr int NT = NW * 64;
     constexpr int NWM = NW / NWN, TNW = BN / 32;
@@ -108,11 +131,15 @@
     constexpr int EPI_HALFS = NW * 32 * 36 * 2 * (HEAD ? 2 : 1);
     static_assert(!GLDS || TAPG == 3, "LDS-DMA weight stages: the 3-tap stages (two buffers fit beside the patch)");
     constexpr int NBUF = GLDS ? 2 : 1;
-    constexpr int SM_HALFS = PATCH_HALFS + NBUF * B_HALFS > EPI_HALFS ? PATCH_HALFS + NBUF * B_HALFS : EPI_HALFS;
+    static_assert(!UP || (DIL == 1 && !INRES && !HEAD && !GLDS && NWN == 1 && TH % 2 == 0), "upsampled source: the plain dilation-1 tiles");
+    constexpr int USH = otvm_upfold_extent(TH), USW = otvm_upfold_extent(32), NSPIX = USH * USW;
+    constexpr int UP_HALFS = UP ? NSPIX * CB * 2 : 0;
+    constexpr int SM_HALFS = PATCH_HALFS + NBUF * B_HALFS + UP_HALFS > EPI_HALFS ? PATCH_HALFS + NBUF * B_HALFS + UP_HALFS : EPI_HALFS;
     __shared__ __attribute__((aligned(16))) _Float16 smem[SM_HALFS];
     _Float16* Ph = smem;
     _Float16* Pl = smem + (M16 ? 2 * PLANE * 8 : NPIX * LDP);
     _Float16* Bs = smem + PATCH_HALFS;
+    float* Us = reinterpret_cast<float*>(smem + PATCH_HALFS + NBUF * B_HALFS);
 
     const int tid = threadIdx.x, lane = tid & 63, wave = tid >> 6;
     const int wave_m = NWN == 1 ? wave : wave % NWM, nt0 = NWN == 1 ? 0 : (wave / NWM) * TN;
@@ -172,12 +199,78 @@
         l_o0 = (((tid >> 1) & 1) * PLANE + (tid >> 2)) * 8 + (tid & 1) * 4;
         l_slope = p.in_relu ? 0.f : (p.in_scale ? (p.in_act == OTVM_ACT_RELU ? 0.f : (p.in_act == OTVM_ACT_LEAKY ? 0.01f : 1.f)) : 1.f);
     }
+    constexpr int NS = (NSPIX * 4 + NT - 1) / NT;
+    static_assert(NS <= NP, "the source patch is loaded into the patch registers");
+    const int up_ncb = UP ? p.up_ncb : 0;
+    __amdgpu_buffer_rsrc_t up_rsrc = otvm_buffer_rsrc(UP ? p.up_src : p.in, UP ? p.up_bytes : 0);
+    unsigned u_voff[UP ? NS : 1];
+    unsigned u_inf[UP ? NP : 1];
+    if constexpr (UP) {
+        const int sy0 = otvm_upfold_origin(ty0), sx0 = otvm_upfold_origin(tx0);
+#pragma unroll
+        for (int k = 0; k < NS; ++k) {
+            const int idx = tid + k * NT;
+            const int spix = idx >> 2, c4 = (idx & 3) * 4;
+            const int sr = spix / USW, sc = spix - sr * USW;
+            const int sy = sy0 + sr, sx = sx0 + sc;
+            const bool ok = ((unsigned)sy < (unsigned)p.up_Hi) & ((unsigned)sx < (unsigned)p.up_Wi) & (idx < NSPIX * 4);
+            u_voff[k] = ok ? ((unsigned)(sy * p.up_Wi + sx) * (unsigned)p.up_ld + (unsigned)c4) << 2 : 0xFFFFFFFFu;
+        }
+#pragma unroll
+        for (int k = 0; k < NP; ++k) {
+            const int idx = tid + k * NT;
+            const int pix = idx >> 2;
+            const int py = pix / PW, px = pix - py * PW;
+            const int iy = ty0 - DIL + py, ix = tx0 - DIL + px;
+            const OtvmUpAxis ay = otvm_upfold_axis(iy, p.up_Hi, sy0, USH), ax = otvm_upfold_axis(ix, p.up_Wi, sx0, USW);
+            const bool inside = ((unsigned)iy < (unsigned)p.H) & ((unsigned)ix < (unsigned)p.W);
+            u_inf[k] = (unsigned)(ay.s0 * USW + ax.s0) | ((unsigned)(ax.s1 - ax.s0) << 8) | ((unsigned)(ay.s1 - ay.s0) << 9) |
+                       ((unsigned)ax.code << 10) | ((unsigned)ay.code << 12) | (inside ? 1u << 14 : 0u);
+        }
+    }
+    auto up_fill = [&]() __attribute__((always_inline)) {
+#pragma unroll
+        for (int k = 0; k < NS; ++k) {
+            const int idx = tid + k * NT;
+            if (k + 1 < NS || idx < NSPIX * 4) {
+                f32x4 v = rp[k];
+                if (p.up_scale) v = otvm_up_norm(v, rsc, rsh, p.up_act);
+                *reinterpret_cast<f32x4*>(&Us[idx * 4]) = v;
+            }
+        }
+        __syncthreads();
+        const int q4 = (tid & 3) * 4;
+#pragma unroll
+        for (int k = 0; k < NP; ++k) {
+            unsigned inf = u_inf[UP ? k : 0];
+            asm volatile("" : "+v"(inf));
+            const int o00 = (int)(inf & 255u) * CB + q4, dx = (int)((inf >> 8) & 1u) * CB, dy = (int)((inf >> 9) & 1u) * (USW * CB);
+            const f32x4 v00 = *reinterpret_cast<const f32x4*>(&Us[o00]), v01 = *reinterpret_cast<const f32x4*>(&Us[o00 + dx]);
+            const f32x4 v10 = *reinterpret_cast<const f32x4*>(&Us[o00 + dy]), v11 = *reinterpret_cast<const f32x4*>(&Us[o00 + dy + dx]);
+            const float lx = 0.25f * (float)((inf >> 10) & 3u), ly = 0.25f * (float)((inf >> 12) & 3u);
+            const f32x4 v = otvm_up_blend(v00, v01, v10, v11, lx, ly);
+            const f32x4 z = {0.f, 0.f, 0.f, 0.f};
+            rp[k] = ((inf >> 14) & 1u) ? v : z;
+        }
+    };
     auto prefetch = [&](int cb, int g) __attribute__((always_inline)) {
+        const bool src_stage = UP && cb < up_ncb;
         if constexpr (LEAN) {
-            const unsigned soff = (unsigned)(cb * CB * 4);
-#pragma unroll
-            for (int k = 0; k < NP; ++k)
-                rp[k] = __builtin_bit_cast(f32x4, (u32x4)__builtin_amdgcn_raw_buffer_load_b128(in_rsrc, __builtin_elementwise_add_sat(l_voff[k], soff), 0, 0));
+            if (src_stage) {
+                const unsigned soff = (unsigned)(cb * CB * 4);
+#pragma unroll
+                for (int k = 0; k < NS; ++k)
+                    rp[k] = __builtin_bit_cast(f32x4, (u32x4)__builtin_amdgcn_raw_buffer_load_b128(up_rsrc, __builtin_elementwise_add_sat(u_voff[UP ? k : 0], soff), 0, 0));
+                if (p.up_scale) {
+                    rsc = *reinterpret_cast<const f32x4*>(p.up_scale + cb * CB + (tid & 3) * 4);
+                    rsh = *reinterpret_cast<const f32x4*>(p.up_shift + cb * CB + (tid & 3) * 4);
+                }
+            } else {
+                const unsigned soff = (unsigned)((cb - up_ncb) * CB * 4);
+#pragma unroll
+                for (int k = 0; k < NP; ++k)
+                    rp[k] = __builtin_bit_cast(f32x4, (u32x4)__builtin_amdgcn_raw_buffer_load_b128(in_rsrc, __builtin_elementwise_add_sat(l_voff[k], soff), 0, 0));
+            }
             const char* wbase = reinterpret_cast<const char*>(p.wf) + (size_t)(((cb >> 1) * 9 * nbs * 2 + (cb & 1)) * 2) * 1024;
 #pragma unroll
             for (int k = 0; k < NB; ++k) rb[k] = *reinterpret_cast<const f16x8*>(wbase + l_woff[k]);
@@ -207,11 +300,20 @@
                 }
             }
         }
-        if (g == 0) {
+        if (g == 0 && src_stage) {
+            if (p.up_scale) {
+                rsc = *reinterpret_cast<const f32x4*>(p.up_scale + cb * CB + (tid & 3) * 4);
+                rsh = *reinterpret_cast<const f32x4*>(p.up_shift + cb * CB + (tid & 3) * 4);
+            }
+#pragma unroll
+            for (int k = 0; k < NS; ++k)
+                rp[k] = __builtin_bit_cast(f32x4, (u32x4)__builtin_amdgcn_raw_buffer_load_b128(up_rsrc, __builtin_elementwise_add_sat(u_voff[UP ? k : 0], (unsigned)(cb * CB * 4)), 0, 0));
+        } else if (g == 0) {
             if (p.in_scale) {
                 rsc = *reinterpret_cast<const f32x4*>(p.in_scale + cb * CB + (tid & 3) * 4);
                 rsh = *reinterpret_cast<const f32x4*>(p.in_shift + cb * CB + (tid & 3) * 4);
             }
+            const int cbv = cb - up_ncb;
 #pragma unroll
             for (int k = 0; k < NP; ++k) {
                 const int idx = tid + k * NT;
@@ -221,18 +323,20 @@
                 const unsigned oob = (unsigned)((int)((unsigned)iy < (unsigned)p.H) & (int)((unsigned)ix < (unsigned)p.W) &
                                                 (int)(idx < NPIX * 4)) - 1u;
                 const unsigned e = (unsigned)(iy * p.W + ix);
-                rp[k] = __builtin_bit_cast(f32x4, (u32x4)__builtin_amdgcn_raw_buffer_load_b128(in_rsrc, ((e * (unsigned)p.in_ld + cb * CB + c4) << 2) | oob, 0, 0));
+                rp[k] = __builtin_bit_cast(f32x4, (u32x4)__builtin_amdgcn_raw_buffer_load_b128(in_rsrc, ((e * (unsigned)p.in_ld + cbv * CB + c4) << 2) | oob, 0, 0));
                 if (INRES)
                     rr[k] = __builtin_bit_cast(f32x4, (u32x4)__builtin_amdgcn_raw_buffer_load_b128(res_rsrc, ((e * (unsigned)p.in_res_ld + cb * CB + c4) << 2) | oob, 0, 0));
             }
         }
     };
-    auto commit = [&](int g) __attribute__((always_inline)) {
+    auto commit = [&](int cb, int g) __attribute__((always_inline)) {
+        const bool src_stage = UP && cb < up_ncb;
         if constexpr (LEAN) {
             const f16x8 zero8 = {(_Float16)0.f, (_Float16)0.f, (_Float16)0.f, (_Float16)0.f, (_Float16)0.f, (_Float16)0.f, (_Float16)0.f, (_Float16)0.f};
 #pragma unroll
             for (int k = 0; k < NB; ++k) *reinterpret_cast<f16x8*>(&Bs[(tid + k * NT) * 8]) = ((l_wok >> k) & 1u) ? rb[k] : zero8;
-            if (p.in_scale != nullptr || p.in_relu) {
+            if (src_stage) up_fill();
+            else if (p.in_scale != nullptr || p.in_relu) {
 #pragma unroll
                 for (int k = 0; k < NP; ++k) {
                     f32x4 v = rp[k] * rsc + rsh;
@@ -262,6 +366,7 @@
             }
         }
         if (g == 0) {
+            if (src_stage) up_fill();
 #pragma unroll
             for (int k = 0; k < NP; ++k) {
                 const int idx = tid + k * NT;
@@ -310,12 +415,12 @@
                 asm volatile("s_waitcnt vmcnt(0)" ::: "memory");
                 __syncthreads();
                 if (g == 0) {
-                    commit(0);
+                    commit(cb, 0);
                     __syncthreads();
                 }
             } else {
                 __syncthreads();
-                if (!OTVM_PABL_NOCOMMIT || (cb == 0 && g == 0)) commit(g);
+                if (!OTVM_PABL_NOCOMMIT || (cb == 0 && g == 0)) commit(cb, g);
                 __syncthreads();
             }
             if (!OTVM_PABL_NOLOAD) {
@@ -747,13 +852,13 @@
 }
 
 template <int NPASS, int TH, int BN, int NW, int DIL, int TAPG = 9, bool INRES = false, bool HEAD = false, int NWN = 1, bool GLDS = false,
-          bool M16 = false, bool FGR = false>
+          bool M16 = false, bool FGR = false, bool UP = false>
 int launch_patch(PatchArgs& a, hipStream_t s) {
     a.tiles_x = otvm_ceil_div(a.W, 32);
     a.tiles_y = otvm_ceil_div(a.H, TH);
     a.tiles_n = otvm_ceil_div(a.Cout, BN);
     a.walk = otvm_tile_walk_of(1);
-    hipLaunchKernelGGL((conv_patch_f16x3_kernel<TH, BN, NW, DIL, TAPG, INRES, HEAD, NWN, GLDS, NPASS, M16, FGR>), dim3(a.tiles_x * a.tiles_y * a.tiles_n, a.batch), dim3(NW * 64), 0, s, a);
+    hipLaunchKernelGGL((conv_patch_f16x3_kernel<TH, BN, NW, DIL, TAPG, INRES, HEAD, NWN, GLDS, NPASS, M16, FGR, UP>), dim3(a.tiles_x * a.tiles_y * a.tiles_n, a.batch), dim3(NW * 64), 0, s, a);
     OTVM_CHECK_LAUNCH("otvm_conv2d(patch f16x3)");
     return 0;
 }
@@ -807,7 +912,7 @@
 }
 
 static int patch_run(const otvm_conv_params* p, void* stream, int choice, const otvm_head_params* hd = nullptr, float* fgr = nullptr,
-                     int64_t fgr_bs = 0);
+                     int64_t fgr_bs = 0, const otvm_conv_up_params* up = nullptr);
 int otvm_conv2d_head16_impl(const otvm_conv_params* p, const otvm_head_params* hd, float* fgr, int64_t fgr_bs, void* stream);
 
 static int conv2d_head_any(const otvm_conv_params* p, const otvm_head_params* hd, float* fgr, int64_t fgr_bs, void* stream) {
@@ -841,7 +946,8 @@
 }
 
 template <int NPASS>
-static int patch_run_t(const otvm_conv_params* p, void* stream, int choice, const otvm_head_params* hd, float* fgr, int64_t fgr_bs) {
+static int patch_run_t(const otvm_conv_params* p, void* stream, int choice, const otvm_head_params* hd, float* fgr, int64_t fgr_bs,
+                       const otvm_conv_up_params* up) {
     if (choice == 0) return -1;
     const bool is_wide = choice == 2;
     PatchArgs a;
@@ -861,6 +967,21 @@
         OTVM_REQUIRE(ib < 0xFFFFFFF0ll && rb < 0xFFFFFFF0ll, "otvm_conv2d(patch f16x3): input view of %lld bytes is beyond 32-bit offsets", (long long)ib);
         a.in_bytes = (unsigned)ib; a.in_res_bytes = (unsigned)rb;
     }
+    a.up_src = nullptr; a.up_scale = a.up_shift = nullptr;
+    a.up_Hi = a.up_Wi = a.up_ld = a.up_ncb = a.up_act = a.up_norm_bs = 0; a.up_bs = 0; a.up_bytes = 0;
+    if (up) {
+        a.up_src = up->src; a.up_scale = up->scale; a.up_shift = up->shift; a.up_act = up->act;
+        a.up_Hi = up->Hi; a.up_Wi = up->Wi; a.up_ld = up->src_ld; a.up_ncb = up->Cu / CB;
+        a.up_bs = a.batch > 1 ? up->src_bs : 0; a.up_norm_bs = a.batch > 1 ? up->norm_bs : 0;
+        a.up_bytes = (unsigned)((int64_t)up->Hi * up->Wi * up->src_ld * 4);
+        if (p->Cout <= 32) {
+            if (up->tile_rows == 16 || (up->tile_rows == 0 && (int64_t)p->H * p->W >= (1 << 20)))
+                return launch_patch<NPASS, 16, 32, 4, 1, 3, false, false, 1, false, false, false, true>(a, s);
+            return launch_patch<NPASS, 8, 32, 4, 1, 3, false, false, 1, false, false, false, true>(a, s);
+        }
+        if constexpr (NPASS == 3) return launch_patch<3, 8, 64, 4, 1, 9, false, false, 1, false, true, false, true>(a, s);
+        else return launch_patch<NPASS, 8, 64, 4, 1, 9, false, false, 1, false, false, false, true>(a, s);
+    }
     if (hd) {
         a.head.w = hd->w; a.head.b = hd->b; a.head.n_out = hd->n_out; a.head.img = hd->img; a.head.img_ld = hd->img_ld;
         a.head.P = hd->P; a.head.alpha_out = hd->alpha_out; a.head.alpha_stride = hd->alpha_stride; a.head.tri_out = hd->tri_out;
@@ -908,6 +1029,38 @@
     return launch_patch<NPASS, 8, 64, 4, 4>(a, s);
 }
 
-static int patch_run(const otvm_conv_params* p, void* stream, int choice, const otvm_head_params* hd, float* fgr, int64_t fgr_bs) {
-    return p->precision == OTVM_PREC_F16 ? patch_run_t<1>(p, stream, choice, hd, fgr, fgr_bs) : patch_run_t<3>(p, stream, choice, hd, fgr, fgr_bs);
-}
+static int patch_run(const otvm_conv_params* p, void* stream, int choice, const otvm_head_params* hd, float* fgr, int64_t fgr_bs,
+                     const otvm_conv_up_params* up) {
+    return p->precision == OTVM_PREC_F16 ? patch_run_t<1>(p, stream, choice, hd, fgr, fgr_bs, up) : patch_run_t<3>(p, stream, choice, hd, fgr, fgr_bs, up);
+}
+
+extern "C" int otvm_conv2d_accepts_upsampled_input(const otvm_conv_params* p, const otvm_conv_up_params* u) {
+    constexpr int T_PATCH_ID = 14;
+    if (!p || !u || !otvm_prec_is_split(p->precision) || !p->w_scale) return 0;
+    if (patch_choice(p) != 1 || p->dil != 1) return 0;
+    if (p->in_res || p->in_scale || p->in_shift || p->in_relu) return 0;
+    if (p->tune && p->tune / 16 - 1 != T_PATCH_ID) return 0;
+    if (p->precision == OTVM_PREC_F16X3 && p->Cout > 32 && !patch_m16()) return 0;
+    if (!u->src || u->Hi < 1 || u->Wi < 1 || u->Cu < CB || u->Cu % CB != 0 || u->Cu > p->Cin) return 0;
+    if (p->H != 2 * u->Hi || p->W != 2 * u->Wi || p->Ho != p->H || p->Wo != p->W) return 0;
+    if (u->src_ld < u->Cu || (u->src_ld & 3) || ((uintptr_t)u->src & 15)) return 0;
+    if (!u->scale != !u->shift || ((uintptr_t)u->scale & 15) || ((uintptr_t)u->shift & 15)) return 0;
+    if (u->act != OTVM_ACT_NONE && u->act != OTVM_ACT_RELU && u->act != OTVM_ACT_LEAKY) return 0;
+    if (u->Cu < p->Cin && (!p->in || (p->in_ld & 3) || ((uintptr_t)p->in & 15) || p->in_ld < p->Cin - u->Cu)) return 0;
+    if (p->batch > 1 && ((u->src_bs & 3) || (u->norm_bs & 3) || (p->in_bs & 3))) return 0;
+    if ((int64_t)u->Hi * u->Wi * u->src_ld * 4 >= 0xFFFFFFF0ll || (int64_t)p->H * p->W * p->in_ld * 4 >= 0xFFFFFFF0ll) return 0;
+    if (u->tile_rows != 0 && !(u->tile_rows == 16 && p->Cout <= 32)) return 0;
+    return 1;
+}
+
+extern "C" int otvm_conv2d_up(const otvm_conv_params* p, const otvm_conv_up_params* u, void* stream) {
+    OTVM_REQUIRE(p && u, "otvm_conv2d_up: null pointer");
+    OTVM_REQUIRE(otvm_conv2d_accepts_upsampled_input(p, u),
+                 "otvm_conv2d_up: not a layer / source the patch kernel takes (otvm_conv2d_accepts_upsampled_input)");
+    OTVM_REQUIRE(p->out && p->w_frag, "otvm_conv2d_up: null pointer");
+    OTVM_REQUIRE(!p->gn_stats || (p->Cout == 64 && p->act == OTVM_ACT_NONE && !p->residual),
+                 "otvm_conv2d_up: fused GroupNorm statistics need Cout = 64, no activation, no residual");
+    OTVM_REQUIRE(!p->gn_scale_out || (p->gn_stats && p->gn_shift_out && p->gn_gamma && p->gn_beta && p->gn_counter),
+                 "otvm_conv2d_up: gn_scale_out needs gn_stats, gn_shift_out, gn_gamma, gn_beta and gn_counter");
+    return patch_run(p, stream, 1, nullptr, nullptr, 0, u);
+}
diff --git a/otvm_amd/csrc/upfold_index.h b/otvm_amd/csrc/upfold_index.h
--- /dev/null
+++ b/otvm_amd/csrc/upfold_index.h
@@ -0,0 +1,33 @@
+#pragma once
+
+#if defined(__HIPCC__)
+#define OTVM_UPFOLD_HD __host__ __device__ inline
+#else
+#define OTVM_UPFOLD_HD inline
+#endif
+
+struct OtvmUpAxis {
+    int i0, i1;
+    float l;
+    int s0, s1;
+    int code;
+};
+
+OTVM_UPFOLD_HD int otvm_upfold_origin(int t0) { return (t0 >> 1) - 1; }
+constexpr int otvm_upfold_extent(int t) { return t / 2 + 2; }
+
+OTVM_UPFOLD_HD OtvmUpAxis otvm_upfold_axis(int o, int n, int org, int ns) {
+#pragma clang fp contract(off)
+    OtvmUpAxis a;
+    float f = ((float)o + 0.5f) * 0.5f - 0.5f;
+    f = f < 0.f ? 0.f : f;
+    const int fi = (int)f;
+    a.l = f - (float)fi;
+    a.i0 = fi > n - 1 ? n - 1 : fi;
+    a.i1 = a.i0 + (a.i0 < n - 1 ? 1 : 0);
+    const int r0 = a.i0 - org, r1 = a.i1 - org;
+    a.s0 = r0 < 0 ? 0 : (r0 > ns - 1 ? ns - 1 : r0);
+    a.s1 = r1 < 0 ? 0 : (r1 > ns - 1 ? ns - 1 : r1);
+    a.code = o <= 0 ? 0 : ((o & 1) ? 1 : 3);
+    return a;
+}
diff --git a/otvm_amd/engine.py b/otvm_amd/engine.py
--- a/otvm_amd/engine.py
+++ b/otvm_amd/engine.py
@@ -30,6 +30,7 @@
 FUSE_STM_BLOCK = os.environ.get("OTVM_FUSE_STM_BLOCK", "1") != "0"
 FUSE_STM_BLOCK128 = int(os.environ.get("OTVM_FUSE_STM_BLOCK128", "1"))
 STM128_TILE = int(os.environ.get("OTVM_STM128_TILE", "0"))
+FOLD_UPSAMPLE = int(os.environ.get("OTVM_FOLD_UPSAMPLE", "1"))
 FUSE_PPM_HEAD = os.environ.get("OTVM_PPM_HEAD", "1") != "0"
 FUSE_GN_PREDICT = os.environ.get("OTVM_GN_PREDICT", "1") != "0"
 GN_PREDICT_MIN_PIXELS = int(os.environ.get("OTVM_GN_PREDICT_MIN_PIXELS", "16384"))
@@ -953,6 +954,8 @@
         self._n_conv = {}
         self._retired_graphs = []
         self._stm128 = []
+        self._upfold = []
+        self.upfold_routes = {}
         self._fused_stats = []
         self._convs = []
         self._predicted = []
@@ -1069,6 +1072,7 @@
     def autotune(self):
         if not (AUTOTUNE and self.e.precision == L.PREC_F16X3):
             self._resolve_stm128(timed=False)
+            self._resolve_upfold(timed=False)
             return
         filled = []
         gen = torch.Generator(device=self.dev)
@@ -1092,6 +1096,8 @@
         self._resolve_stm128(timed=FUSE_STM_BLOCK128 == 1)
         torch.cuda.synchronize(self.dev)
         del self._convs[n0:], self._keep[k0:]
+        self._resolve_upfold(timed=FOLD_UPSAMPLE == 1)
+        torch.cuda.synchronize(self.dev)
         for t in filled:
             t.zero_()
         self.stats.zero_()
@@ -1121,7 +1127,8 @@
         t = self.raw(name, n * self.B, dtype)
         return [t[b * n:(b + 1) * n] for b in range(self.B)]
 
-    def conv(self, S, x, wname, out, stride=1, pad=0, dil=1, act=NONE, in_relu=0, residual=None, in_norm=None, in_res=None):
+    def conv(self, S, x, wname, out, stride=1, pad=0, dil=1, act=NONE, in_relu=0, residual=None, in_norm=None, in_res=None,
+             up_source=None):
         w = self.e.W[wname]
         assert x.C == w.I_pad, (wname, x.C, w.I_pad)
         Ho = (x.H + 2 * pad - dil * (w.kh - 1) - 1) // stride + 1
@@ -1137,6 +1144,9 @@
         abytes = 4 * (x.B * x.H * x.W * w.I * (2 if in_res is not None else 1) + w.O * w.I * w.kh * w.kw
                       + x.B * Ho * Wo * w.O * (2 if residual is not None else 1))
         S.append((self.lib.otvm_conv2d, (C.byref(p),), "conv " + wname, flops, abytes, (x, out.ch(0, _rup(w.O, 4)) if out.C >= _rup(w.O, 4) else out)))
+        if up_source is not None:
+            assert up_source["out"].t is x.t and up_source["out"].off == x.off and stride == 1 and in_norm is None and in_res is None
+            up_source["readers"].append((S, S[-1], p, x, wname))
         return p
 
     def conv_head(self, S, x, wname, hid_out, head_w, head_b, n_out, img, alpha, alpha_stride, alpha_bs, tri=None, sm=None,
@@ -1251,9 +1261,80 @@
         if FUSE_GN_APPLY and FUSE_GN_STATS and producer_p is not None:
             sc, sh, nbs = self.gn_table_step(S, x, gn_name, producer_p)
             self.upsample(S, x, out, norm=(sc, sh, gn_act, nbs))
-        else:
-            self.gn(S, x, gn_name, gn_act, conv_p=producer_p)
-            self.upsample(S, x, out)
+            m = {"name": gn_name, "S": S, "step": S[-1], "src": x, "norm": (sc, sh, gn_act, nbs), "out": out, "readers": []}
+            self._upfold.append(m)
+            return m
+        self.gn(S, x, gn_name, gn_act, conv_p=producer_p)
+        self.upsample(S, x, out)
+        return None
+
+    def _resolve_upfold(self, timed):
+        stream = torch.cuda.current_stream(self.dev).cuda_stream
+        timed_any = False
+        for m in self._upfold:
+            self.upfold_routes[m["name"]] = 0
+            if FOLD_UPSAMPLE <= 0 or self.e.keep_hid_d or not m["readers"]:
+                continue
+            src, (sc, sh, act, nbs) = m["src"], m["norm"]
+            folded = []
+            for S, step, p, x, wname in m["readers"]:
+                pf, u = L.ConvParams(), L.ConvUpParams()
+                C.memmove(C.byref(pf), C.byref(p), C.sizeof(L.ConvParams))
+                pf.inp = x.ch(src.C, x.C - src.C).ptr
+                u.src, u.Hi, u.Wi, u.Cu, u.src_ld, u.src_bs = src.ptr, src.H, src.W, src.C, src.ld, src.bs
+                u.scale, u.shift, u.act, u.norm_bs = sc, sh, act, nbs
+                if not self.lib.otvm_conv2d_accepts_upsampled_input(C.byref(pf), C.byref(u)):
+                    folded = None
+                    break
+                self._keep += [pf, u]
+                w = self.e.W[wname]
+                saved = 4 * x.B * x.P * min(src.C, w.I) * 3 // 4
+                folded.append((self.lib.otvm_conv2d_up, (C.byref(pf), C.byref(u)), step[2] + " (+ up2x)", step[3], step[4] - saved, step[5]))
+            if folded is None:
+                continue
+            key = (-2, src.H, src.W, max(1, src.B), src.C, src.ld) + tuple(v for r in m["readers"] for v in (r[2].Cin, r[2].Cout, r[2].act))
+            if FOLD_UPSAMPLE >= 2:
+                choice = 1
+            elif key in _TUNE_CACHE:
+                choice = _TUNE_CACHE[key]
+            elif not timed:
+                choice = 0
+            else:
+                routes = {0: [m["step"]] + [r[1] for r in m["readers"]], 1: folded}
+
+                def run(c, reps):
+                    e0, e1 = torch.cuda.Event(enable_timing=True), torch.cuda.Event(enable_timing=True)
+                    e0.record()
+                    for _ in range(reps):
+                        for st in routes[c]:
+                            L.check(st[0](*st[1], stream), st[2])
+                    e1.record()
+                    return e0, e1, reps
+                self.e.conv_calls += 2 * (2 + 4 * 3) * len(folded)
+                run(0, 2)
+                run(1, 2)
+                timed_ = [(c,) + run(c, 3) for c in (0, 1, 0, 1, 0, 1, 0, 1)]
+                torch.cuda.synchronize(self.dev)
+                ms = {}
+                for c, e0, e1, r in timed_:
+                    t = e0.elapsed_time(e1) / r
+                    ms[c] = min(ms.get(c, t), t)
+                choice = min(ms, key=ms.get)
+                _TUNE_CACHE[key] = choice
+                TUNE_LOG.append((m["name"] + " (2x upsampling: 0 = pass + reader convs, 1 = read at source resolution by the convs)",
+                                 (2 * src.H, 2 * src.W, src.C, src.ld, src.C, m["out"].ld, 1, 1, 1, 0, 1), choice, ms))
+                timed_any = True
+            if choice:
+                at = lambda S, st: next(i for i, q in enumerate(S) if q is st)
+                del m["S"][at(m["S"], m["step"])]
+                for (S, step, p, x, wname), fs in zip(m["readers"], folded):
+                    S[at(S, step)] = fs
+                self.upfold_routes[m["name"]] = 1
+                for b in range(max(1, m["out"].B)):
+                    m["out"].torch(b).zero_()
+        self._upfold = []
+        if timed_any:
+            _save_tune_file()
 
     def maxpool(self, S, x, out):
         S.append((self.lib.otvm_maxpool3x3s2_b, (x.ptr, x.H, x.W, x.C, x.ld, out.ptr, out.ld, x.B, x.bs, out.bs), "maxpool"))
@@ -1557,12 +1638,12 @@
         self.gn_then_upsample(S, u1b, de + "conv_up1.4", LEAKY, cp, self.U2.ch(0, 256))
         u2 = self.buf("u2", H4, W4, 256)
         cp = self.conv(S, self.U2, de + "conv_up2.0", u2, pad=1)
-        self.gn_then_upsample(S, u2, de + "conv_up2.1", LEAKY, cp, self.U3.ch(0, 256))
+        up2 = self.gn_then_upsample(S, u2, de + "conv_up2.1", LEAKY, cp, self.U3.ch(0, 256))
         u3 = self.buf("u3", H2, W2, 64)
-        cp = self.conv(S, self.U3, de + "conv_up3.0", u3, pad=1)
-        self.gn_then_upsample(S, u3, de + "conv_up3.1", LEAKY, cp, self.D80.ch(0, 64))
+        cp = self.conv(S, self.U3, de + "conv_up3.0", u3, pad=1, up_source=up2)
+        up3 = self.gn_then_upsample(S, u3, de + "conv_up3.1", LEAKY, cp, self.D80.ch(0, 64))
         h32 = self.buf("h32", Hp, Wp, 32)
-        self.conv(S, self.D80, de + "conv_up4.0", h32, pad=1, act=LEAKY)
+        self.conv(S, self.D80, de + "conv_up4.0", h32, pad=1, act=LEAKY, up_source=up3)
         img = self.D80.ch(67, 3)
         fuse_head = FUSE_HEAD and e.precision == L.PREC_F16X3 and e.W[de + "conv_up4.2"].w_frag is not None
         if fuse_head:
@@ -1578,7 +1659,7 @@
                            img.img(b).ptr, img.ld, P, self.D80.ch(72, 1).img(b).ptr, self.D80.ld, 0, 0, 0), "fba_head7"))
         rf = "NET.refine."
         r0 = self.buf("r0", Hp, Wp, 64)
-        cp = self.conv(S, self.D80, rf + "conv1.0", r0, pad=1)
+        cp = self.conv(S, self.D80, rf + "conv1.0", r0, pad=1, up_source=up3)
         x, x_norm = r0, None
         w1 = e.W[rf + "layer1.conv1"]
         t1 = self.buf("rt1", Hp, Wp, 64)
diff --git a/otvm_amd/lib.py b/otvm_amd/lib.py
--- a/otvm_amd/lib.py
+++ b/otvm_amd/lib.py
@@ -29,6 +29,11 @@
                 ("in_res", vp), ("in_res_ld", i32), ("in_res_bs", i64)]
 
 
+class ConvUpParams(C.Structure):
+    _fields_ = [("src", vp), ("Hi", i32), ("Wi", i32), ("Cu", i32), ("src_ld", i32), ("src_bs", i64),
+                ("scale", vp), ("shift", vp), ("act", i32), ("norm_bs", i32), ("tile_rows", i32)]
+
+
 class StmBottleneckParams(C.Structure):
     _fields_ = [("x", vp), ("H", i32), ("W", i32), ("Cin", i32), ("x_ld", i32), ("y", vp), ("y_ld", i32),
                 ("w1f", vp), ("w2f", vp), ("w3f", vp), ("s1", vp), ("s2", vp), ("s3", vp), ("b1", vp), ("b2", vp), ("b3", vp),
@@ -116,6 +121,8 @@
     "otvm_conv2d_accepts_input_norm": (i32, [C.POINTER(ConvParams)]),
     "otvm_conv2d_input_norm_kind": (i32, [C.POINTER(ConvParams)]),
     "otvm_conv2d_accepts_input_residual": (i32, [C.POINTER(ConvParams)]),
+    "otvm_conv2d_up": (i32, [C.POINTER(ConvParams), C.POINTER(ConvUpParams), vp]),
+    "otvm_conv2d_accepts_upsampled_input": (i32, [C.POINTER(ConvParams), C.POINTER(ConvUpParams)]),
     "otvm_conv2d_head": (i32, [C.POINTER(ConvParams), C.POINTER(HeadParams), vp]),
     "otvm_conv2d_head_fgr": (i32, [C.POINTER(ConvParams), C.POINTER(HeadParams), vp, i64, vp]),
     "otvm_head16_weight_bytes_f16x3": (i64, []),
```

After: 48.29 frames/s (median of 6 runs). +1.2%, better.
